# david-knigge/enf-pde

Hardware: AMD Instinct MI355X
Metric: query-points/sec (ENF fit+decode) at 64 latents x 64^2 grid (higher is better)
Workload: dtype bf16; 1 GPU; navier_stokes_64x64_z64_b16_per_gpu; decoded_states=1, latents=64, signals_per_gpu=16, inner_steps=3, sampled_points=512, num_hidden=128, num_heads=2, latent_dim=16, num_out=1, invariant=rel_pos_periodic, hparams=config_navier_stokes.yaml:23-96 with 64 latents, parallelism=dp1 (signals sharded, no data-path collective in fit/decode)

## Files before the change

enf-pde_amd/_lib.py:

```python
import ctypes
import os

_HERE = os.path.dirname(os.path.abspath(__file__))
LIB_PATH = os.environ.get("ENF_HIP_LIB") or os.path.join(_HERE, "libenf_hip.so")
TEST_LIB_PATH = os.environ.get("ENF_HIP_TEST_LIB") or os.path.join(_HERE, "libenf_hip_test.so")

ENF_NUM_TENSORS = 46
PREC = {"f32": 0, "fp32": 0, "float32": 0, "bf16": 1, "bfloat16": 1}
INVARIANT_IDS = {"rel_pos_periodic": 0, "latitude_periodic": 1, "polar_periodic": 2, "ponita": 3,
                 "abs_pos": 4, "rel_pos": 5, "norm_rel_pos": 6, "ball": 7, "ball_lat": 8, "ponita_full": 9}

EXPORTS = ["enf_abi_version", "enf_strerror", "enf_invariant_dim", "enf_invariant_pose_dim", "enf_check_desc",
           "enf_packed_weight_bytes", "enf_pack_weights", "enf_workspace_bytes", "enf_forward",
           "enf_backward_latents", "enf_backward_latents_ex", "enf_forward_stages", "enf_lt_layout", "enf_lt_layout_ext", "enf_pack_pair", "enf_pair_forward",
           "enf_pair_backward", "enf_pair_backward_ex", "enf_pair_scratch_bytes", "enf_pair_variant", "enf_pair_partition", "enf_shared_forward_parts", "enf_shared_backward_applies", "enf_backward_weights", "enf_backward_weights_scratch_bytes",
           "enf_backward_all", "enf_backward_all_scratch_bytes", "enf_fit_step", "enf_fit_inputs",
           "enf_mse_value_grad",
           "enf_workspace_bytes_ex", "enf_fit_step_ex", "enf_mse_value_grad_ex", "enf_mse_scratch_bytes", "enf_pair_backward_ex2",
           "enf_pair_backward_scratch_bytes", "enf_backward_all_scratch_bytes_ex", "enf_backward_weights_ex",
           "enf_backward_weights_scratch_bytes_ex",
           "enf_fit_step_w", "enf_mse_value_grad_w", "enf_fit_inputs_w", "enf_fit_inputs_b",
           "enf_fit_step_cw", "enf_mse_value_grad_cw", "enf_fit_inputs_cw",
           "enf_fit_step_e", "enf_eval_loss", "enf_signal_sum",
           "enf_field_grad_workspace_bytes", "enf_field_grad", "enf_query_vjp",
           "enf_ode_conv_forward", "enf_ode_conv_backward_basis", "enf_ode_conv_backward_weight", "enf_ode_conv_backward_weight_scratch_bytes", "enf_ode_poly_num_features", "enf_ode_poly_forward",
           "enf_ode_poly_backward", "enf_ode_vec_readout_forward", "enf_ode_vec_readout_backward", "enf_ode_block_supported", "enf_ode_block_scratch_bytes", "enf_ode_block_forward", "enf_ode_block_backward",
           "enf_ode_basis_supported", "enf_ode_basis_scratch_bytes", "enf_ode_basis_forward",
           "enf_ode_basis_backward", "enf_relu_mask_bytes", "enf_meta_sgd_update", "enf_table_adam_update"]
ENF_NUM_PAIR_TENSORS = 12
ENF_STAGE_PROLOGUE, ENF_STAGE_PAIR, ENF_STAGE_TAIL, ENF_STAGE_FOLD = 1, 2, 4, 8
ENF_STAGE_TAIL_SAVE = 16
ENF_STAGE_PREPARE_BWD = 32
ENF_STAGE_YBAR_HALF = 64
ENF_STAGES_FORWARD = ENF_STAGE_PROLOGUE | ENF_STAGE_PAIR | ENF_STAGE_TAIL | ENF_STAGE_FOLD
ENF_BWD_REUSE_PROLOGUE, ENF_BWD_REUSE_TAIL, ENF_BWD_REUSE_PREPARED, ENF_BWD_ONLY_PAIR = 1, 2, 4, 8
ENF_BWD_DETERMINISTIC = ENF_FIT_DETERMINISTIC = ENF_MSE_DETERMINISTIC = 16
ENF_FIT_SHARED_LATENTS = ENF_STAGE_SHARED_LATENTS = 128
ENF_BWD_QUERY_GRAD = 32
(ENF_S_EQ, ENF_S_EV, ENF_S_G1, ENF_S_NH, ENF_S_DA1, ENF_S_DA2, ENF_S_DA3, ENF_S_HEAD0) = range(8)


def num_store(H):
    return 7 + 4 * H


class EnfDesc(ctypes.Structure):
    _fields_ = [(n, ctypes.c_int32) for n in
                ("B", "N", "Z", "H", "D", "C", "O", "dx", "invariant_id", "use_window", "precision")] + \
               [("h_true", ctypes.c_int32), ("d_true", ctypes.c_int32),
                ("pair_fwd_variant", ctypes.c_int32), ("pair_bwd_variant", ctypes.c_int32), ("mask_mode", ctypes.c_int32),
                ("mask_signals", ctypes.c_int32), ("embedding", ctypes.c_int32), ("relu_masks", ctypes.c_void_p)]


VARIANT = {"auto": 0, "latent_split": 1, "z_fold": 2, "z_fold_zsplit": 3}
MASK_MODE = {"off": 0, "write": 1, "read": 2}
EMB = {"rff": 0, "ffn": 1}


class EnfSgdSegment(ctypes.Structure):
    _fields_ = [("x", ctypes.c_void_p), ("g", ctypes.c_void_p), ("lr", ctypes.c_void_p), ("out", ctypes.c_void_p),
                ("n", ctypes.c_int64), ("width", ctypes.c_int32), ("g_stride", ctypes.c_int32), ("lr_len", ctypes.c_int32),
                ("reserved", ctypes.c_int32)]


ENF_SGD_MAX_SEGMENTS = 4


ENF_ADAM_MAX_SEGMENTS = 4


class EnfAdamSegment(ctypes.Structure):
    _fields_ = [(n, ctypes.c_void_p) for n in ("x", "mu", "nu", "g", "x_out", "mu_out", "nu_out")] + \
               [("width", ctypes.c_int32), ("g_stride", ctypes.c_int32)]


class EnfFitComponent(ctypes.Structure):
    _fields_ = [("src", ctypes.c_void_p), ("dst", ctypes.c_void_p), ("width", ctypes.c_int32), ("reserved", ctypes.c_int32)]


class EnfError(RuntimeError):
    pass


_lib = None
_test_lib = None


def load():
    global _lib
    if _lib is not None:
        return _lib
    _lib = _bind(LIB_PATH, test_hooks=False)
    return _lib


def load_test():
    global _test_lib
    if _test_lib is None:
        _test_lib = _bind(TEST_LIB_PATH, test_hooks=True)
    return _test_lib


class using:

    def __init__(self, lib):
        self.lib = lib

    def __enter__(self):
        global _lib
        self.prev, _lib = _lib, self.lib
        return self.lib

    def __exit__(self, *exc):
        global _lib
        _lib = self.prev


def _bind(path, test_hooks):
    if not os.path.exists(path):
        raise EnfError(f"{path} not found: build it with `make -C enf-pde_amd/csrc` "
                       "(or python -c 'import __graft_entry__ as g; g.build()'). There is no fallback path.")
    lib = ctypes.CDLL(path)
    vp, i64, sz, ci = ctypes.c_void_p, ctypes.c_int64, ctypes.c_size_t, ctypes.c_int
    dp = ctypes.POINTER(EnfDesc)
    lib.enf_abi_version.restype = ci
    lib.enf_strerror.restype = ctypes.c_char_p
    lib.enf_strerror.argtypes = [ci]
    lib.enf_invariant_dim.argtypes = [ci, ci]
    lib.enf_invariant_pose_dim.argtypes = [ci, ci]
    lib.enf_check_desc.argtypes = [dp]
    lib.enf_packed_weight_bytes.restype = sz
    lib.enf_packed_weight_bytes.argtypes = [dp]
    lib.enf_workspace_bytes.restype = sz
    lib.enf_workspace_bytes.argtypes = [dp]
    lib.enf_pack_weights.argtypes = [dp, ctypes.POINTER(vp), vp, vp]
    lib.enf_forward.argtypes = [dp, vp, i64, vp, vp, vp, vp, vp, vp, vp, vp, sz, vp]
    lib.enf_forward_stages.argtypes = [dp, vp, i64, vp, vp, vp, vp, vp, vp, vp, vp, sz, ctypes.c_uint, vp]
    lib.enf_backward_latents.argtypes = [dp, vp, i64, vp, vp, vp, vp, vp, vp, vp, vp, vp, vp, vp, sz, vp]
    lib.enf_backward_latents_ex.argtypes = [dp, vp, i64, vp, vp, vp, vp, vp, vp, vp, vp, vp, vp, vp, sz, ctypes.c_uint, vp]
    ip = ctypes.POINTER(ci)
    lib.enf_lt_layout.argtypes = [dp, ip, ip, ip, ip, ip, ip]
    lib.enf_pack_pair.argtypes = [dp, ctypes.POINTER(vp), vp, vp]
    lib.enf_mse_value_grad.argtypes = [vp, vp, sz, ctypes.c_float, vp, vp, vp]
    lib.enf_meta_sgd_update.argtypes = [ctypes.c_int, ctypes.POINTER(EnfSgdSegment), ctypes.c_float, vp]
    lib.enf_table_adam_update.argtypes = [ctypes.c_int, ctypes.POINTER(EnfAdamSegment), i64, ctypes.c_int32, vp, ctypes.c_int32] + \
                                         [ctypes.c_float] * 6 + [vp]
    lib.enf_fit_inputs.argtypes = [ctypes.c_int, ctypes.POINTER(EnfFitComponent)] + [ctypes.c_int32] * 7 + [vp] * 7
    lib.enf_ode_conv_forward.argtypes = [ci, ci, ci, ci, vp, vp, i64, i64, vp, vp, vp, vp]
    lib.enf_ode_conv_backward_basis.argtypes = [ci, ci, ci, ci, vp, vp, vp, vp, vp]
    lib.enf_ode_conv_backward_weight_scratch_bytes.restype = sz
    lib.enf_ode_conv_backward_weight_scratch_bytes.argtypes = [ci, ci, ci, ci]
    lib.enf_ode_conv_backward_weight.argtypes = [ci, ci, ci, ci, vp, vp, vp, vp, vp, sz, vp]
    lib.enf_ode_poly_num_features.argtypes = [ci, ci]
    lib.enf_ode_poly_forward.argtypes = [i64, ci, ci, vp, vp, vp]
    lib.enf_ode_poly_backward.argtypes = [i64, ci, ci, vp, vp, vp, vp]
    lib.enf_ode_basis_supported.argtypes = [ci, ci, ci, ci, ci]
    cf = ctypes.c_float
    lib.enf_ode_vec_readout_forward.argtypes = [ci, ci, ci, ci, vp, vp, vp, vp, cf, cf, vp, vp, vp]
    lib.enf_ode_vec_readout_backward.argtypes = [ci, ci, ci, ci, vp, vp, vp, vp, cf, cf, vp, vp, vp, vp, vp, vp, vp, vp]
    lib.enf_ode_block_supported.argtypes = [ci, ci]
    lib.enf_ode_block_scratch_bytes.restype = sz
    lib.enf_ode_block_scratch_bytes.argtypes = [i64, ci, ci]
    lib.enf_ode_block_forward.argtypes = [i64, ci, ci, vp, vp, vp, vp, vp, vp, vp, ctypes.c_float, vp, vp, vp]
    lib.enf_ode_block_backward.argtypes = [i64, ci, ci, vp, vp, vp, vp, vp, vp, vp, ctypes.c_float, vp, vp, vp, sz, vp]
    lib.enf_ode_basis_scratch_bytes.restype = sz
    lib.enf_ode_basis_scratch_bytes.argtypes = [i64, ci, ci, ci, ci]
    lib.enf_ode_basis_forward.argtypes = [i64, ci, ci, ci, ci, vp, vp, vp, vp, vp, vp, vp, sz, vp]
    lib.enf_ode_basis_backward.argtypes = [i64, ci, ci, ci, ci, vp, vp, vp, vp, vp, vp, vp, vp, vp, vp, vp, vp, sz, vp]
    lib.enf_relu_mask_bytes.restype = sz
    lib.enf_relu_mask_bytes.argtypes = [dp]
    lib.enf_pair_variant.argtypes = [dp, ci]
    lib.enf_pair_partition.argtypes = [dp] + [ctypes.POINTER(ctypes.c_int32)] * 3
    lib.enf_shared_forward_parts.argtypes = [dp, ctypes.POINTER(ctypes.c_int32)]
    lib.enf_shared_backward_applies.argtypes = [dp, ctypes.c_uint]
    lib.enf_backward_weights_scratch_bytes.restype = sz
    lib.enf_backward_weights_scratch_bytes.argtypes = [dp, ci]
    lib.enf_backward_weights.argtypes = [dp, vp, i64, vp, vp, vp, vp, vp, vp, ctypes.POINTER(vp), vp, vp, sz, vp]
    lib.enf_fit_step.argtypes = [dp, vp, i64, vp, vp, vp, vp, vp, ctypes.c_float, vp, vp, vp, vp, vp, sz, vp]
    lib.enf_backward_all_scratch_bytes.restype = sz
    lib.enf_backward_all_scratch_bytes.argtypes = [dp, ci]
    lib.enf_backward_all.argtypes = [dp, vp, i64, vp, vp, vp, ctypes.POINTER(vp), vp, vp, vp, vp, vp, vp, vp, ctypes.POINTER(vp), vp,
                                     vp, sz, vp, sz, ctypes.c_uint, vp]
    lib.enf_pair_scratch_bytes.restype = sz
    lib.enf_pair_scratch_bytes.argtypes = [dp]
    lib.enf_pair_forward.argtypes = [dp, vp, i64, vp, vp, vp, vp, vp, sz, vp]
    lib.enf_pair_backward.argtypes = [dp, vp, i64, vp, vp, vp, vp, vp, vp, ctypes.POINTER(vp), vp]
    lib.enf_pair_backward_ex.argtypes = [dp, vp, i64, vp, vp, vp, vp, vp, vp, ctypes.POINTER(vp), vp, vp]
    cu = ctypes.c_uint
    lib.enf_workspace_bytes_ex.restype = sz
    lib.enf_workspace_bytes_ex.argtypes = [dp, cu]
    lib.enf_fit_step_ex.argtypes = [dp, vp, i64, vp, vp, vp, vp, vp, ctypes.c_float, vp, vp, vp, vp, vp, sz, cu, vp]
    lib.enf_mse_scratch_bytes.restype = sz
    lib.enf_mse_scratch_bytes.argtypes = [sz, cu]
    lib.enf_mse_value_grad_ex.argtypes = [vp, vp, sz, ctypes.c_float, vp, vp, vp, sz, cu, vp]
    lib.enf_fit_step_w.argtypes = [dp, vp, i64, vp, vp, vp, vp, vp, ctypes.c_float, vp, vp, vp, vp, vp, sz, vp, cu, vp]
    lib.enf_mse_value_grad_w.argtypes = [vp, vp, vp, sz, ctypes.c_int32, ctypes.c_float, vp, vp, vp, sz, cu, vp]
    lib.enf_fit_inputs_w.argtypes = [ctypes.c_int, ctypes.POINTER(EnfFitComponent)] + [ctypes.c_int32] * 7 + [vp] * 9
    lib.enf_fit_inputs_b.argtypes = [ctypes.c_int, ctypes.POINTER(EnfFitComponent)] + [ctypes.c_int32] * 7 + [vp] * 9
    lib.enf_fit_step_cw.argtypes = [dp, vp, i64, vp, vp, vp, vp, vp, ctypes.c_float, vp, vp, vp, vp, vp, sz, vp, cu, vp]
    lib.enf_mse_value_grad_cw.argtypes = [vp, vp, vp, sz, ctypes.c_float, vp, vp, vp, sz, cu, vp]
    lib.enf_fit_inputs_cw.argtypes = [ctypes.c_int, ctypes.POINTER(EnfFitComponent)] + [ctypes.c_int32] * 7 + [vp] * 8 + [ctypes.c_int32, vp]
    lib.enf_fit_step_e.argtypes = [dp, vp, i64, vp, vp, vp, vp, vp, ctypes.c_float, vp, vp, vp, vp, vp, sz, vp, vp, vp, vp, cu, vp]
    lib.enf_eval_loss.argtypes = [dp, vp, i64] + [vp] * 11 + [sz, cu, vp]
    lib.enf_signal_sum.argtypes = [vp, ctypes.c_int32, ctypes.c_int32, ctypes.c_float, vp, vp]
    lib.enf_field_grad_workspace_bytes.restype = sz
    lib.enf_field_grad_workspace_bytes.argtypes = [dp, cu]
    lib.enf_field_grad.argtypes = [dp, vp, i64] + [vp] * 7 + [sz, cu, vp]
    lib.enf_query_vjp.argtypes = [dp, vp, i64] + [vp] * 8 + [sz, cu, vp]
    lib.enf_pair_backward_scratch_bytes.restype = sz
    lib.enf_pair_backward_scratch_bytes.argtypes = [dp, cu]
    lib.enf_pair_backward_ex2.argtypes = [dp, vp, i64, vp, vp, vp, vp, vp, vp, ctypes.POINTER(vp), vp, vp, sz, cu, vp]
    lib.enf_backward_all_scratch_bytes_ex.restype = sz
    lib.enf_backward_all_scratch_bytes_ex.argtypes = [dp, ci, cu]
    lib.enf_backward_weights_scratch_bytes_ex.restype = sz
    lib.enf_backward_weights_scratch_bytes_ex.argtypes = [dp, ci, cu]
    lib.enf_backward_weights_ex.argtypes = [dp, vp, i64, vp, vp, vp, vp, vp, vp, ctypes.POINTER(vp), vp, vp, sz, cu, vp]
    if test_hooks:
        for name in ("enf_debug_gemm", "enf_debug_pack", "enf_test_read_wave_sums", "enf_test_pair_fwd_streamed"):
            getattr(lib, name).restype = ci
        lib.enf_test_pair_fwd_streamed.argtypes = [ci]
        lib.enf_debug_gemm.argtypes = [vp, vp, vp, ci, ci, ci, vp]
        lib.enf_debug_pack.argtypes = [vp, vp, ci, ci, ci, vp]
        lib.enf_test_read_wave_sums.argtypes = [vp]
    if lib.enf_abi_version() != 2:
        raise EnfError(f"{path}: ABI version mismatch")
    return lib


def check(rc):
    if rc == 0:
        return
    msg = load().enf_strerror(rc).decode()
    if rc == -2:
        raise ValueError(msg)
    if rc == -6:
        raise AssertionError(msg)
    if rc == -3:
        raise NotImplementedError(msg)
    raise EnfError(f"libenf_hip error {rc}: {msg}")


def launch(dev, fn, *args):
    import torch
    idx = dev.index if dev.index is not None else torch.cuda.current_device()
    if idx == torch.cuda.current_device():
        return check(fn(*args))
    with torch.cuda.device(idx):
        return check(fn(*args))


def ptr(t):
    return ctypes.c_void_p(t.data_ptr()) if t is not None else ctypes.c_void_p(0)


def stream(dev):
    import torch
    return ctypes.c_void_p(torch.cuda.current_stream(dev).cuda_stream)


def make_desc(B, N, Z, H, D, C, O, dx, invariant_id, use_window, precision, d_true=0, h_true=0, variants=(0, 0),
              masks=None, embedding=0):
    d = EnfDesc()
    d.B, d.N, d.Z, d.H, d.D, d.C, d.O, d.dx = int(B), int(N), int(Z), int(H), int(D), int(C), int(O), int(dx)
    d.invariant_id, d.use_window, d.precision = int(invariant_id), int(bool(use_window)), int(precision)
    d.d_true, d.h_true = int(d_true), int(h_true)
    d.pair_fwd_variant, d.pair_bwd_variant = int(variants[0]), int(variants[1])
    d.embedding = int(embedding)
    if masks is not None:
        buf, mode, signals = masks
        d.relu_masks, d.mask_mode, d.mask_signals = buf.data_ptr(), MASK_MODE[mode], int(signals)
    return d
```

enf-pde_amd/csrc/enf_api.hip:

```cpp
#include <hip/hip_runtime.h>
#include <mutex>
#include <unordered_map>
#include "enf_launch.h"

extern "C" int enf_abi_version(void) { return ENF_ABI_VERSION; }

extern "C" const char* enf_strerror(int code) {
  switch (code) {
    case ENF_OK: return "ok";
    case ENF_EINVAL: return "invalid argument (null pointer or non-positive size)";
    case ENF_EINVARIANT: return "Unknown invariant type";
    case ENF_EUNSUPPORTED: return "shape not in the compiled kernel set (num_hidden 64 or 128 after padding; num_heads 1, 2, or 4 at num_hidden 64; "
                                  "num_out <= 32; ball / ball_lat at num_hidden 64 only)";
    case ENF_EWORKSPACE: return "workspace too small";
    case ENF_ELAUNCH: return "HIP launch failed";
    case ENF_EDIM: return "coordinate / pose width inconsistent with the invariant";
    default: return "unknown error";
  }
}

extern "C" int enf_invariant_dim(int inv, int dx) {
  const int i = enf_inv_dim(inv, dx);
  return i < 0 ? ENF_EINVARIANT : i;
}
extern "C" int enf_invariant_pose_dim(int inv, int dx) {
  const int i = enf_inv_pose_dim(inv, dx);
  return i < 0 ? ENF_EINVARIANT : i;
}

extern "C" int enf_check_desc(const EnfDesc* d) {
  if (!d) return ENF_EINVAL;
  if (d->B <= 0 || d->N <= 0 || d->Z <= 0 || d->C <= 0 || d->O <= 0 || d->H <= 0 || d->D <= 0) return ENF_EINVAL;
  if (d->invariant_id < 0 || d->invariant_id >= ENF_INV_COUNT) return ENF_EINVARIANT;
  if (d->dx < 1 || d->dx > 3) return ENF_EDIM;
  const bool two_d = d->invariant_id == ENF_INV_REL_POS_PERIODIC || d->invariant_id == ENF_INV_PONITA ||
                     d->invariant_id == ENF_INV_LATITUDE_PERIODIC || d->invariant_id == ENF_INV_POLAR_PERIODIC;
  if (two_d && d->dx != 2) return ENF_EDIM;
  if (d->invariant_id == ENF_INV_PONITA_FULL && d->dx != 3) return ENF_EDIM;
  if (enf_inv_has_phase(d->invariant_id) && d->D != 64) return ENF_EUNSUPPORTED;
  if (enf_inv_has_phase(d->invariant_id) && d->dx != 3) return ENF_EDIM;
  if (!(d->D == 64 || d->D == 128)) return ENF_EUNSUPPORTED;
  if (d->d_true < 0 || d->d_true > d->D || (d->d_true & 1)) return ENF_EINVAL;
  if (!(d->H == 1 || d->H == 2 || (d->H == 4 && d->D == 64))) return ENF_EUNSUPPORTED;
  if (d->h_true < 0 || d->h_true > d->H) return ENF_EINVAL;
  if (d->O > 32) return ENF_EUNSUPPORTED;
  if (d->precision != ENF_PREC_F32 && d->precision != ENF_PREC_BF16) return ENF_EINVAL;
  if (d->pair_fwd_variant < ENF_VARIANT_AUTO || d->pair_fwd_variant > ENF_VARIANT_ZFOLD_ZSPLIT) return ENF_EINVAL;
  if (d->pair_bwd_variant < ENF_VARIANT_AUTO || d->pair_bwd_variant > ENF_VARIANT_ZFOLD) return ENF_EINVAL;
  if (d->mask_mode < ENF_MASK_OFF || d->mask_mode > ENF_MASK_READ || d->mask_signals < 0) return ENF_EINVAL;
  if (d->mask_mode != ENF_MASK_OFF && !d->relu_masks) return ENF_EINVAL;
  if (d->embedding != ENF_EMB_RFF && d->embedding != ENF_EMB_FFN) return ENF_EINVAL;
  if (d->embedding == ENF_EMB_FFN && enf_inv_has_phase(d->invariant_id)) return ENF_EUNSUPPORTED;
  return ENF_OK;
}

extern "C" size_t enf_packed_weight_bytes(const EnfDesc* d) {
  if (enf_check_desc(d) != ENF_OK) return 0;
  return enf_layout(enf_dims(d)).total;
}

extern "C" size_t enf_workspace_bytes(const EnfDesc* d) {
  if (enf_check_desc(d) != ENF_OK) return 0;
  return enf_workspace(enf_dims(d)).total;
}

extern "C" size_t enf_workspace_bytes_ex(const EnfDesc* d, unsigned flags) {
  if (enf_check_desc(d) != ENF_OK || (flags & ~(ENF_BWD_DETERMINISTIC | ENF_BWD_QUERY_GRAD | ENF_FIT_SHARED_LATENTS))) return 0;
  const EnfDims m = enf_dims(d);
  const EnfWorkspace W = enf_workspace(m);
  return (flags & ENF_BWD_DETERMINISTIC) ? enf_det_workspace(m, W).total : W.total;
}

struct SidePending { hipEvent_t join = nullptr; bool pending = false; };
struct SideStream {
  hipStream_t s = nullptr;
  hipEvent_t fork = nullptr;
  std::mutex mu;
  std::unordered_map<const void*, SidePending> ws;
  SidePending* entry(const void* workspace) {
    auto it = ws.find(workspace);
    if (it != ws.end()) return &it->second;
    if (ws.size() >= 64)
      for (auto j = ws.begin(); j != ws.end();) {
        if (!j->second.pending) { (void)hipEventDestroy(j->second.join); j = ws.erase(j); } else ++j;
      }
    SidePending e;
    if (hipEventCreateWithFlags(&e.join, hipEventDisableTiming) != hipSuccess) return nullptr;
    return &ws.emplace(workspace, e).first->second;
  }
};
static constexpr int ENF_MAX_DEVICES = 64;
static SideStream* side_stream() {
  static std::mutex table_mu;
  static SideStream* table[ENF_MAX_DEVICES] = {};
  static bool tried[ENF_MAX_DEVICES] = {};
  int dev = 0;
  if (hipGetDevice(&dev) != hipSuccess || dev < 0 || dev >= ENF_MAX_DEVICES) return nullptr;
  std::lock_guard<std::mutex> lk(table_mu);
  if (!tried[dev]) {
    tried[dev] = true;
    SideStream* t = new SideStream();
    if (hipStreamCreateWithFlags(&t->s, hipStreamNonBlocking) == hipSuccess &&
        hipEventCreateWithFlags(&t->fork, hipEventDisableTiming) == hipSuccess)
      table[dev] = t;
    else
      delete t;
  }
  return table[dev];
}

int enf_side_join_pending(hipStream_t st, const void* workspace) {
  SideStream* side = side_stream();
  if (!side) return 0;
  std::lock_guard<std::mutex> lk(side->mu);
  auto it = side->ws.find(workspace);
  if (it != side->ws.end() && it->second.pending) {
    if (hipStreamWaitEvent(st, it->second.join, 0) != hipSuccess) return ENF_ELAUNCH;
    it->second.pending = false;
  }
  return 0;
}

static int side_prepare_bwd(SideStream* side, const EnfCall& c, bool zero_dlt, int wz_signals = 0) {
  if (!side) return 0;
  EnfDims mw = c.m;
  if (wz_signals > 0) mw.B = wz_signals;
  std::lock_guard<std::mutex> lk(side->mu);
  SidePending* e = side->entry(c.ws);
  if (!e) return 0;
  if (hipEventRecord(side->fork, c.st) != hipSuccess || hipStreamWaitEvent(side->s, side->fork, 0) != hipSuccess) return ENF_ELAUNCH;
  if (int rc = enf_launch_wz(mw, c.L, c.blob, c.F(c.W.lt), nullptr, c.F(c.W.wzb), nullptr, c.ws + c.W.wzt, side->s)) return rc;
  if (zero_dlt && hipMemsetAsync(c.F(c.W.dlt), 0, enf_lt_bytes(c.m), side->s) != hipSuccess) return ENF_ELAUNCH;
  if (hipEventRecord(e->join, side->s) != hipSuccess) return ENF_ELAUNCH;
  e->pending = true;
  return 1;
}

extern "C" int enf_forward_stages(const EnfDesc* d, const float* x, int64_t x_bstride, const float* p, const float* a,
                                  const float* sigma, const void* packed, float* out, float* ybar, float* lse,
                                  void* workspace, size_t workspace_bytes, unsigned stages, void* stream) {
  EnfCall c;
  const bool shared = (stages & ENF_STAGE_SHARED_LATENTS) && d && d->B > 1;
  int rc = enf_call(c, d, x && p && a && out && !(shared && x_bstride != 0), sigma, packed, workspace, workspace_bytes, stream);
  if (rc) return rc;
  const EnfDims& m = c.m;
  const EnfWorkspace& W = c.W;
  float* yb = ybar ? ybar : c.F(W.ybar);
  const bool zf = enf_use_zfold(m);
  float* ls = lse ? lse : c.F(W.lse);
  const bool yhalf = (stages & ENF_STAGE_YBAR_HALF) && m.bf16 && !ybar && (stages & ENF_STAGE_PAIR) && (stages & ENF_STAGE_TAIL) &&
                     !(stages & ENF_STAGE_TAIL_SAVE) && enf_zfold_split(m) <= 1;
  if ((rc = enf_side_join_pending(c.st, workspace))) return rc;
  if ((stages & ENF_STAGE_PROLOGUE) && (rc = enf_launch_prologue(m, c.L, c.blob, p, a, sigma, c.F(W.lt), c.F(W.an), c.F(W.kv), c.st))) return rc;
  if ((stages & (ENF_STAGE_PAIR | ENF_STAGE_FOLD)) &&
      (rc = enf_launch_pair_fwd(m, c.L, c.blob, x, x_bstride, c.F(W.lt), yb, ls, zf ? c.ws + W.wz : nullptr, zf ? c.F(W.wzb) : nullptr,
                                zf ? c.ws + W.wzu : nullptr, enf_zfold_split(m) > 1 ? c.F(W.ysplit) : nullptr, (stages & ENF_STAGE_FOLD) != 0,
                                ((stages & ENF_STAGE_PAIR) != 0 ? 1 : 0) | (yhalf ? 2 : 0), c.st, shared ? c.F(W.dybar) : nullptr)))
    return rc;
  if ((stages & ENF_STAGE_PREPARE_BWD) && enf_use_zfold_bwd(m) && (rc = side_prepare_bwd(side_stream(), c, true)) < 0) return rc;
  const bool tsave = (stages & ENF_STAGE_TAIL_SAVE) != 0;
  if ((stages & ENF_STAGE_TAIL) &&
      (rc = enf_launch_tail(m, c.L, c.blob, yb, out, nullptr, nullptr, nullptr, tsave ? c.F(W.tail_act) : nullptr, 0, (tsave ? 1 : 0) | (yhalf ? 2 : 0), c.st)))
    return rc;
  return ENF_OK;
}

extern "C" int enf_forward(const EnfDesc* d, const float* x, int64_t x_bstride, const float* p, const float* a,
                           const float* sigma, const void* packed, float* out, float* ybar, float* lse, void* workspace,
                           size_t workspace_bytes, void* stream) {
  return enf_forward_stages(d, x, x_bstride, p, a, sigma, packed, out, ybar, lse, workspace, workspace_bytes,
                            ENF_STAGE_PROLOGUE | ENF_STAGE_FOLD | ENF_STAGE_PAIR | ENF_STAGE_TAIL, stream);
}

extern "C" int enf_backward_latents(const EnfDesc* d, const float* x, int64_t x_bstride, const float* p, const float* a,
                                    const float* sigma, const void* packed, const float* ybar, const float* lse,
                                    const float* dout, float* dp, float* da, float* dsigma, void* workspace,
                                    size_t workspace_bytes, void* stream) {
  return enf_backward_latents_ex(d, x, x_bstride, p, a, sigma, packed, ybar, lse, dout, dp, da, dsigma, workspace,
                                 workspace_bytes, 0u, stream);
}

static int pair_bwd_on_workspace(const EnfCall& c, const float* x, int64_t x_bstride, const float* lse, bool det = false) {
  const bool zb = enf_use_zfold_bwd(c.m);
  return enf_launch_pair_bwd(c.m, c.L, c.blob, x, x_bstride, c.F(c.W.lt), lse, c.F(c.W.dybar), c.F(c.W.delta), c.F(c.W.dlt), nullptr,
                             zb ? c.ws + c.W.wzt : nullptr, zb ? c.F(c.W.wzb) : nullptr, nullptr, c.st, det ? c.F(c.X.part) : nullptr);
}

extern "C" int enf_backward_latents_ex(const EnfDesc* d, const float* x, int64_t x_bstride, const float* p, const float* a,
                                       const float* sigma, const void* packed, const float* ybar, const float* lse,
                                       const float* dout, float* dp, float* da, float* dsigma, void* workspace,
                                       size_t workspace_bytes, unsigned flags, void* stream) {
  EnfCall c;
  const bool det = (flags & ENF_BWD_DETERMINISTIC) != 0;
  const bool known = !(flags & ~(ENF_BWD_REUSE_PROLOGUE | ENF_BWD_REUSE_TAIL | ENF_BWD_REUSE_PREPARED | ENF_BWD_ONLY_PAIR | ENF_BWD_DETERMINISTIC));
  int rc = enf_call(c, d, known && x && p && a && ybar && lse && dout && dp && da && dsigma, sigma, packed, workspace, workspace_bytes,
                    stream, det);
  if (rc) return rc;
  const EnfDims& m = c.m;
  const EnfWorkspace& W = c.W;
  hipStream_t st = c.st;
  const bool zb = enf_use_zfold_bwd(m);
  if (flags & ENF_BWD_ONLY_PAIR) {
    if ((rc = enf_side_join_pending(st, workspace))) return rc;
    if (!det && hipMemsetAsync(c.F(W.dlt), 0, enf_lt_bytes(m), st) != hipSuccess) return ENF_ELAUNCH;
    return pair_bwd_on_workspace(c, x, x_bstride, lse, det);
  }
  if (!(flags & ENF_BWD_REUSE_PROLOGUE) && (rc = enf_launch_prologue(m, c.L, c.blob, p, a, sigma, c.F(W.lt), c.F(W.an), c.F(W.kv), st)))
    return rc;
  SideStream* side = zb ? side_stream() : nullptr;
  bool prepared = false;
  if (zb && side && (flags & ENF_BWD_REUSE_PREPARED) && (flags & ENF_BWD_REUSE_PROLOGUE)) {
    std::lock_guard<std::mutex> lk(side->mu);
    auto it = side->ws.find(workspace);
    prepared = it != side->ws.end() && it->second.pending;
  }
  if (!prepared && (rc = enf_side_join_pending(st, workspace))) return rc;
  if (zb && !prepared) {
    if ((rc = side_prepare_bwd(side, c, false)) < 0) return rc;
    if (!rc && (rc = enf_launch_wz(m, c.L, c.blob, c.F(W.lt), nullptr, c.F(W.wzb), nullptr, c.ws + W.wzt, st))) return rc;
  }
  const bool treuse = (flags & ENF_BWD_REUSE_TAIL) && (flags & ENF_BWD_REUSE_PROLOGUE);
  if ((rc = enf_launch_tail(m, c.L, c.blob, ybar, nullptr, dout, c.F(W.dybar), c.F(W.delta), c.F(W.tail_act), 1, treuse ? 1 : 0, st))) return rc;
  if (!prepared && !det && hipMemsetAsync(c.F(W.dlt), 0, enf_lt_bytes(m), st) != hipSuccess) return ENF_ELAUNCH;
  if ((rc = enf_side_join_pending(st, workspace))) return rc;
  if ((rc = pair_bwd_on_workspace(c, x, x_bstride, lse, det))) return rc;
  return enf_launch_prologue_bwd(m, c.L, c.blob, p, sigma, c.F(W.an), c.F(W.kv), c.F(W.dlt), dp, da, dsigma, st);
}


extern "C" int enf_fit_step(const EnfDesc* d, const float* x, int64_t x_bstride, const float* p, const float* a, const float* sigma,
                            const void* packed, const float* target, float grad_scale, float* loss, float* dp, float* da,
                            float* dsigma, void* workspace, size_t workspace_bytes, void* stream) {
  return enf_fit_step_ex(d, x, x_bstride, p, a, sigma, packed, target, grad_scale, loss, dp, da, dsigma, workspace, workspace_bytes, 0u,
                         stream);
}

extern "C" int enf_fit_step_ex(const EnfDesc* d, const float* x, int64_t x_bstride, const float* p, const float* a, const float* sigma,
                               const void* packed, const float* target, float grad_scale, float* loss, float* dp, float* da,
                               float* dsigma, void* workspace, size_t workspace_bytes, unsigned flags, void* stream) {
  return enf_fit_step_w(d, x, x_bstride, p, a, sigma, packed, target, grad_scale, loss, dp, da, dsigma, workspace, workspace_bytes,
                        nullptr, flags, stream);
}

static int fit_step_sequence(const EnfDesc* d, const float* x, int64_t x_bstride, const float* p, const float* a, const float* sigma,
                             const void* packed, const float* target, float grad_scale, float* loss, float* dp, float* da,
                             float* dsigma, void* workspace, size_t workspace_bytes, const float* weight, bool per_value, unsigned flags,
                             void* stream, float* err = nullptr, float* loss_b = nullptr, bool args_ok = true) {
  EnfCall c;
  const bool det = (flags & ENF_FIT_DETERMINISTIC) != 0;
  const bool shared = (flags & ENF_FIT_SHARED_LATENTS) && d && d->B > 1;
  int rc = enf_call(c, d, !(flags & ~(ENF_FIT_DETERMINISTIC | ENF_FIT_SHARED_LATENTS)) && !(shared && x_bstride != 0) && x && p && a && target &&
                    loss && dp && da && dsigma && (!per_value || weight) && args_ok, sigma, packed, workspace, workspace_bytes, stream, det);
  if (rc) return rc;
  const EnfDims& m = c.m;
  const EnfWorkspace& W = c.W;
  hipStream_t st = c.st;
  const bool zf = enf_use_zfold(m), zb = enf_use_zfold_bwd(m);
  if ((rc = enf_side_join_pending(st, workspace))) return rc;
  if ((rc = enf_launch_prologue(m, c.L, c.blob, p, a, sigma, c.F(W.lt), c.F(W.an), c.F(W.kv), st))) return rc;
  if ((rc = enf_launch_pair_fwd(m, c.L, c.blob, x, x_bstride, c.F(W.lt), c.F(W.ybar), c.F(W.lse), zf ? c.ws + W.wz : nullptr,
                                zf ? c.F(W.wzb) : nullptr, zf ? c.ws + W.wzu : nullptr, enf_zfold_split(m) > 1 ? c.F(W.ysplit) : nullptr, 1, 1, st,
                                shared ? c.F(W.dybar) : nullptr)))
    return rc;
  const bool sbwd = enf_shared_backward_rule(m, flags, per_value, err != nullptr) == 1;
  EnfDims m1 = m;
  if (sbwd) m1.B = 1;
  if ((rc = side_prepare_bwd(zb ? side_stream() : nullptr, c, !det, sbwd ? 1 : 0)) < 0) return rc;
  if (!rc) {
    if (zb && (rc = enf_launch_wz(m1, c.L, c.blob, c.F(W.lt), nullptr, c.F(W.wzb), nullptr, c.ws + W.wzt, st))) return rc;
    if (!det && hipMemsetAsync(c.F(W.dlt), 0, enf_lt_bytes(m), st) != hipSuccess) return ENF_ELAUNCH;
  }
  if (sbwd) {
    float* dout = c.F(W.dybar) + (size_t)m.N * m.HD;
    float* out1 = dout + (size_t)m.B * m.N;
    if ((rc = enf_launch_tail(m1, c.L, c.blob, c.F(W.ybar), out1, nullptr, nullptr, nullptr, c.F(W.tail_act), 0, 1, st))) return rc;
    if ((rc = enf_launch_mse_shared(out1, target, weight, m.B, m.N, grad_scale, dout, loss, st))) return rc;
    if ((rc = enf_launch_tail_seed(m1, c.L, c.blob, c.F(W.ybar), 0, c.F(W.dybar), c.F(W.delta), c.F(W.tail_act), st))) return rc;
    if ((rc = enf_side_join_pending(st, workspace))) return rc;
    if ((rc = enf_launch_pair_bwd_shared(m, c.L, c.blob, x, c.F(W.lt), c.F(W.lse), c.F(W.dybar), c.F(W.delta), dout, c.F(W.dlt),
                                         c.ws + W.wzt, c.F(W.wzb), st)))
      return rc;
    return enf_launch_prologue_bwd(m, c.L, c.blob, p, sigma, c.F(W.an), c.F(W.kv), c.F(W.dlt), dp, da, dsigma, st);
  }
  if ((rc = enf_launch_tail_loss(m, c.L, c.blob, c.F(W.ybar), target, weight, grad_scale, loss, c.F(W.dybar), c.F(W.delta), c.F(W.tail_act), st,
                                 det ? c.F(c.X.loss) : nullptr, per_value, err)))
    return rc;
  if ((rc = enf_side_join_pending(st, workspace))) return rc;
  if ((rc = pair_bwd_on_workspace(c, x, x_bstride, c.F(W.lse), det))) return rc;
  if ((rc = enf_launch_prologue_bwd(m, c.L, c.blob, p, sigma, c.F(W.an), c.F(W.kv), c.F(W.dlt), dp, da, dsigma, st))) return rc;
  return err && loss_b ? enf_launch_signal_sum(err, m.B, m.N, 1.0f / ((float)m.N * (float)m.O), loss_b, st) : ENF_OK;
}

extern "C" int enf_fit_step_w(const EnfDesc* d, const float* x, int64_t x_bstride, const float* p, const float* a, const float* sigma,
                              const void* packed, const float* target, float grad_scale, float* loss, float* dp, float* da,
                              float* dsigma, void* workspace, size_t workspace_bytes, const float* weight, unsigned flags,
                              void* stream) {
  return fit_step_sequence(d, x, x_bstride, p, a, sigma, packed, target, grad_scale, loss, dp, da, dsigma, workspace, workspace_bytes, weight,
                           false, flags, stream);
}

extern "C" int enf_fit_step_cw(const EnfDesc* d, const float* x, int64_t x_bstride, const float* p, const float* a, const float* sigma,
                               const void* packed, const float* target, float grad_scale, float* loss, float* dp, float* da,
                               float* dsigma, void* workspace, size_t workspace_bytes, const float* cweight, unsigned flags,
                               void* stream) {
  return fit_step_sequence(d, x, x_bstride, p, a, sigma, packed, target, grad_scale, loss, dp, da, dsigma, workspace, workspace_bytes, cweight,
                           true, flags, stream);
}

extern "C" int enf_fit_step_e(const EnfDesc* d, const float* x, int64_t x_bstride, const float* p, const float* a, const float* sigma,
                              const void* packed, const float* target, float grad_scale, float* loss, float* dp, float* da,
                              float* dsigma, void* workspace, size_t workspace_bytes, const float* weight, const float* cweight,
                              float* err, float* loss_b, unsigned flags, void* stream) {
  return fit_step_sequence(d, x, x_bstride, p, a, sigma, packed, target, grad_scale, loss, dp, da, dsigma, workspace, workspace_bytes,
                           cweight ? cweight : weight, cweight != nullptr, flags, stream, err, loss_b, err && !(weight && cweight));
}

extern "C" int enf_eval_loss(const EnfDesc* d, const float* x, int64_t x_bstride, const float* p, const float* a, const float* sigma,
                             const void* packed, const float* target, const float* weight, const float* cweight, float* loss,
                             float* err, float* loss_b, void* workspace, size_t workspace_bytes, unsigned flags, void* stream) {
  EnfCall c;
  const bool det = (flags & ENF_FIT_DETERMINISTIC) != 0;
  int rc = enf_call(c, d, !(flags & ~ENF_FIT_DETERMINISTIC) && x && p && a && target && !(weight && cweight) && (loss || err || loss_b),
                    sigma, packed, workspace, workspace_bytes, stream, det);
  if (rc) return rc;
  const EnfDims& m = c.m;
  const EnfWorkspace& W = c.W;
  hipStream_t st = c.st;
  const bool zf = enf_use_zfold(m);
  if ((rc = enf_side_join_pending(st, workspace))) return rc;
  if ((rc = enf_launch_prologue(m, c.L, c.blob, p, a, sigma, c.F(W.lt), c.F(W.an), c.F(W.kv), st))) return rc;
  if ((rc = enf_launch_pair_fwd(m, c.L, c.blob, x, x_bstride, c.F(W.lt), c.F(W.ybar), c.F(W.lse), zf ? c.ws + W.wz : nullptr,
                                zf ? c.F(W.wzb) : nullptr, zf ? c.ws + W.wzu : nullptr, enf_zfold_split(m) > 1 ? c.F(W.ysplit) : nullptr, 1, 1, st)))
    return rc;
  float* e = err ? err : (loss_b ? c.F(W.dybar) : nullptr);
  if ((rc = enf_launch_tail_eval(m, c.L, c.blob, c.F(W.ybar), target, cweight ? cweight : weight, cweight != nullptr, loss, e, st,
                                 det ? c.F(c.X.loss) : nullptr)))
    return rc;
  return loss_b ? enf_launch_signal_sum(e, m.B, m.N, 1.0f / ((float)m.N * (float)m.O), loss_b, st) : ENF_OK;
}

extern "C" size_t enf_field_grad_workspace_bytes(const EnfDesc* d, unsigned flags) {
  if (enf_check_desc(d) != ENF_OK || d->mask_mode != ENF_MASK_OFF || (flags & ~ENF_BWD_DETERMINISTIC)) return 0;
  const EnfDims m = enf_dims(d);
  const EnfWorkspace W = enf_workspace(m);
  return (flags & ENF_BWD_DETERMINISTIC) ? enf_det_workspace(m, W).total + enf_det_dx_bytes(m) : W.total;
}

static int field_grad_sequence(const EnfDesc* d, const float* x, int64_t x_bstride, const float* p, const float* a, const float* sigma,
                               const void* packed, const float* dout, float* out, float* grad, bool args_ok, void* workspace,
                               size_t workspace_bytes, unsigned flags, void* stream) {
  int rc = enf_check_desc(d);
  if (rc) return rc;
  if (d->mask_mode != ENF_MASK_OFF) return ENF_EUNSUPPORTED;
  EnfCall c;
  const bool det = (flags & ENF_BWD_DETERMINISTIC) != 0;
  if ((rc = enf_call(c, d, !(flags & ~ENF_BWD_DETERMINISTIC) && x && p && a && grad && args_ok, sigma, packed, workspace, workspace_bytes,
                     stream, det)))
    return rc;
  const EnfDims& m = c.m;
  const EnfWorkspace& W = c.W;
  hipStream_t st = c.st;
  if (det && workspace_bytes < c.X.total + enf_det_dx_bytes(m)) return ENF_EWORKSPACE;
  float* part = det ? c.F(c.X.part) : nullptr;
  float* dxpart = det ? c.F(c.X.total) : nullptr;
  const bool zf = enf_use_zfold(m), zb = enf_use_zfold_bwd(m);
  const size_t per = (size_t)m.B * m.N * m.dx;
  const int passes = dout ? 1 : m.O;
  if ((rc = enf_side_join_pending(st, workspace))) return rc;
  if ((rc = enf_launch_prologue(m, c.L, c.blob, p, a, sigma, c.F(W.lt), c.F(W.an), c.F(W.kv), st))) return rc;
  if (zb && (rc = enf_launch_wz(m, c.L, c.blob, c.F(W.lt), nullptr, c.F(W.wzb), nullptr, c.ws + W.wzt, st))) return rc;
  if ((rc = enf_launch_pair_fwd(m, c.L, c.blob, x, x_bstride, c.F(W.lt), c.F(W.ybar), c.F(W.lse), zf ? c.ws + W.wz : nullptr,
                                zf ? c.F(W.wzb) : nullptr, zf ? c.ws + W.wzu : nullptr, enf_zfold_split(m) > 1 ? c.F(W.ysplit) : nullptr, 1, 1, st)))
    return rc;
  if ((rc = enf_launch_tail(m, c.L, c.blob, c.F(W.ybar), out ? out : c.F(W.dybar), nullptr, nullptr, nullptr, c.F(W.tail_act), 0, 1, st))) return rc;
  if (!det && (hipMemsetAsync(c.F(W.dlt), 0, enf_lt_bytes(m), st) != hipSuccess ||
               hipMemsetAsync(grad, 0, sizeof(float) * per * passes, st) != hipSuccess))
    return ENF_ELAUNCH;
  for (int o = 0; o < passes; ++o) {
    if (dout) rc = enf_launch_tail(m, c.L, c.blob, c.F(W.ybar), nullptr, dout, c.F(W.dybar), c.F(W.delta), c.F(W.tail_act), 1, 1, st);
    else rc = enf_launch_tail_seed(m, c.L, c.blob, c.F(W.ybar), o, c.F(W.dybar), c.F(W.delta), c.F(W.tail_act), st);
    if (rc) return rc;
    if ((rc = enf_launch_pair_bwd(m, c.L, c.blob, x, x_bstride, c.F(W.lt), c.F(W.lse), c.F(W.dybar), c.F(W.delta), c.F(W.dlt), nullptr,
                                  zb ? c.ws + W.wzt : nullptr, zb ? c.F(W.wzb) : nullptr, grad + (size_t)o * per, st, part, dxpart)))
      return rc;
  }
  return ENF_OK;
}

extern "C" int enf_field_grad(const EnfDesc* d, const float* x, int64_t x_bstride, const float* p, const float* a, const float* sigma,
                              const void* packed, float* out, float* jac, void* workspace, size_t workspace_bytes, unsigned flags,
                              void* stream) {
  return field_grad_sequence(d, x, x_bstride, p, a, sigma, packed, nullptr, out, jac, true, workspace, workspace_bytes, flags, stream);
}

extern "C" int enf_query_vjp(const EnfDesc* d, const float* x, int64_t x_bstride, const float* p, const float* a, const float* sigma,
                             const void* packed, const float* dout, float* out, float* dx, void* workspace, size_t workspace_bytes,
                             unsigned flags, void* stream) {
  return field_grad_sequence(d, x, x_bstride, p, a, sigma, packed, dout, out, dx, dout != nullptr, workspace, workspace_bytes, flags, stream);
}

extern "C" int enf_lt_layout(const EnfDesc* d, int* stride, int* off_u, int* off_v0, int* off_pose, int* off_wcoef, int* off_c) {
  int rc = enf_check_desc(d);
  if (rc) return rc;
  if (stride) *stride = enf_lt_stride(d->H, d->D);
  if (off_u) *off_u = enf_lt_off_u(d->H, d->D);
  if (off_v0) *off_v0 = enf_lt_off_v0(d->H, d->D);
  if (off_pose) *off_pose = enf_lt_off_pose(d->H, d->D);
  if (off_wcoef) *off_wcoef = enf_lt_off_wcoef(d->H, d->D);
  if (off_c) *off_c = enf_lt_off_c(d->H, d->D);
  return ENF_OK;
}

extern "C" int enf_lt_layout_ext(const EnfDesc* d, int* off_ext, int* off_phase_q, int* off_phase_v) {
  int rc = enf_check_desc(d);
  if (rc) return rc;
  if (off_ext) *off_ext = enf_lt_off_ext(d->H, d->D);
  if (off_phase_q) *off_phase_q = enf_lt_off_phq(d->H, d->D);
  if (off_phase_v) *off_phase_v = enf_lt_off_phv(d->H, d->D);
  return ENF_OK;
}

extern "C" int enf_pair_variant(const EnfDesc* d, int backward) {
  const int rc = enf_check_desc(d);
  if (rc) return rc;
  const EnfDims m = enf_dims(d);
  if (backward) return enf_use_zfold_bwd(m) ? ENF_VARIANT_ZFOLD : ENF_VARIANT_LATENT_SPLIT;
  const int sp = enf_zfold_split(m);
  return sp > 1 ? ENF_VARIANT_ZFOLD_ZSPLIT : (sp == 1 ? ENF_VARIANT_ZFOLD : ENF_VARIANT_LATENT_SPLIT);
}

extern "C" int enf_shared_forward_parts(const EnfDesc* d, int32_t* parts) {
  const int rc = enf_check_desc(d);
  if (rc) return rc;
  if (!parts) return ENF_EINVAL;
  const EnfDims m = enf_dims(d);
  const int P = enf_use_zfold(m) || (m.mask_mode != ENF_MASK_OFF && !m.ffn) ? 0 : enf_shared_fwd_parts(m);
  *parts = P ? P : 1;
  return P ? 1 : 0;
}

extern "C" int enf_shared_backward_applies(const EnfDesc* d, unsigned flags) {
  const int rc = enf_check_desc(d);
  if (rc) return rc;
  if (flags & ~(ENF_FIT_DETERMINISTIC | ENF_FIT_SHARED_LATENTS)) return ENF_EINVAL;
  return enf_shared_backward_rule(enf_dims(d), flags, false, false);
}

extern "C" int enf_pair_partition(const EnfDesc* d, int32_t* run, int32_t* workgroups, int32_t* parts) {
  const int rc = enf_check_desc(d);
  if (rc) return rc;
  if (!run || !workgroups || !parts) return ENF_EINVAL;
  const EnfDims m = enf_dims(d);
  if (enf_zfold_split(m) < 2) return 0;
  const EnfStreamK k = enf_zfold_streamk(m);
  *run = k.len; *workgroups = k.wgs; *parts = k.parts;
  return 1;
}

struct PairScratch { size_t wz, wzb, wzu, ysplit, total; };
static PairScratch pair_scratch(const EnfDims& m) {
  PairScratch s{0, 0, 0, 0, 0};
  if (!enf_use_zfold(m)) return s;
  const size_t BZ = (size_t)m.B * m.Z, BN = (size_t)m.B * m.N;
  const int split = enf_zfold_split(m);
  s.wzb = s.wz + enf_align(BZ * m.H * enf_panel_bytes(m.D, m.D, m.bf16));
  s.wzu = s.wzb + enf_align(sizeof(float) * BZ * m.HD);
  s.ysplit = s.wzu + enf_align(BZ * enf_wzu_bytes(m.H, m.D));
  s.total = s.ysplit + (split > 1 ? sizeof(float) * split * (BN * m.HD + BN * m.H * 3) : 0);
  return s;
}

extern "C" size_t enf_pair_scratch_bytes(const EnfDesc* d) {
  if (enf_check_desc(d)) return 0;
  return pair_scratch(enf_dims(d)).total;
}

extern "C" int enf_pair_forward(const EnfDesc* d, const float* x, int64_t x_bstride, const float* lt, const void* packed,
                                float* ybar, float* lse, void* scratch, size_t scratch_bytes, void* stream) {
  int rc = enf_check_desc(d);
  if (rc) return rc;
  if (!x || !lt || !packed || !ybar || !lse) return ENF_EINVAL;
  const EnfDims m = enf_dims(d);
  const PairScratch S = pair_scratch(m);
  const bool zf = S.total != 0;
  if (zf && (!scratch || scratch_bytes < S.total)) return ENF_EWORKSPACE;
  char* sc = (char*)scratch;
  return enf_launch_pair_fwd(m, enf_layout(m), (const char*)packed, x, x_bstride, lt, ybar, lse, zf ? sc + S.wz : nullptr,
                             zf ? reinterpret_cast<float*>(sc + S.wzb) : nullptr, zf ? sc + S.wzu : nullptr,
                             zf && enf_zfold_split(m) > 1 ? reinterpret_cast<float*>(sc + S.ysplit) : nullptr, 1, 1, (hipStream_t)stream);
}

extern "C" size_t enf_relu_mask_bytes(const EnfDesc* d) {
  if (enf_check_desc(d) != ENF_OK) return 0;
  const size_t signals = d->mask_signals > 0 ? d->mask_signals : d->B;
  return signals * d->Z * ((d->N + 15) / 16) * 2 * 64 * sizeof(unsigned);
}

extern "C" int enf_pair_backward(const EnfDesc* d, const float* x, int64_t x_bstride, const float* lt, const void* packed,
                                 const float* lse, const float* dybar, const float* delta, float* dlt, void* const* store,
                                 void* stream) {
  return enf_pair_backward_ex(d, x, x_bstride, lt, packed, lse, dybar, delta, dlt, store, nullptr, stream);
}

extern "C" int enf_pair_backward_ex(const EnfDesc* d, const float* x, int64_t x_bstride, const float* lt, const void* packed,
                                    const float* lse, const float* dybar, const float* delta, float* dlt, void* const* store,
                                    float* dx, void* stream) {
  return enf_pair_backward_ex2(d, x, x_bstride, lt, packed, lse, dybar, delta, dlt, store, dx, nullptr, 0, 0u, stream);
}

extern "C" size_t enf_pair_backward_scratch_bytes(const EnfDesc* d, unsigned flags) {
  if (enf_check_desc(d) != ENF_OK || (flags & ~(ENF_BWD_DETERMINISTIC | ENF_BWD_QUERY_GRAD))) return 0;
  if (!(flags & ENF_BWD_DETERMINISTIC)) return 0;
  const EnfDims m = enf_dims(d);
  return enf_det_part_bytes(m, false) + ((flags & ENF_BWD_QUERY_GRAD) ? enf_det_dx_bytes(m) : 0);
}

extern "C" int enf_pair_backward_ex2(const EnfDesc* d, const float* x, int64_t x_bstride, const float* lt, const void* packed,
                                     const float* lse, const float* dybar, const float* delta, float* dlt, void* const* store,
                                     float* dx, void* scratch, size_t scratch_bytes, unsigned flags, void* stream) {
  int rc = enf_check_desc(d);
  if (rc) return rc;
  if ((flags & ~ENF_BWD_DETERMINISTIC) || !x || !lt || !packed || !lse || !dybar || !delta || !dlt) return ENF_EINVAL;
  const bool det = (flags & ENF_BWD_DETERMINISTIC) != 0;
  if (det && !scratch) return ENF_EINVAL;
  const EnfDims m = enf_dims(d);
  if (store)
    for (int i = 0; i < ENF_NUM_STORE(m.H); ++i)
      if (!store[i]) return ENF_EINVAL;
  hipStream_t st = (hipStream_t)stream;
  if (det) {
    const size_t pb = enf_det_part_bytes(m, false);
    if (scratch_bytes < pb + (dx ? enf_det_dx_bytes(m) : 0)) return ENF_EWORKSPACE;
    return enf_launch_pair_bwd(m, enf_layout(m), (const char*)packed, x, x_bstride, lt, lse, dybar, delta, dlt, store, nullptr, nullptr, dx, st,
                               (float*)scratch, dx ? reinterpret_cast<float*>((char*)scratch + pb) : nullptr);
  }
  if (hipMemsetAsync(dlt, 0, enf_lt_bytes(m), st) != hipSuccess) return ENF_ELAUNCH;
  return enf_launch_pair_bwd(m, enf_layout(m), (const char*)packed, x, x_bstride, lt, lse, dybar, delta, dlt, store, nullptr, nullptr, dx, st);
}

extern "C" size_t enf_backward_weights_scratch_bytes(const EnfDesc* d, int chunk_signals) {
  if (enf_check_desc(d) != ENF_OK || chunk_signals < 1 || chunk_signals > d->B) return 0;
  return enf_wgrad_scratch_bytes(enf_dims(d), chunk_signals);
}

extern "C" int enf_backward_weights(const EnfDesc* d, const float* x, int64_t x_bstride, const float* lt, const void* packed,
                                    const float* lse, const float* dybar, const float* delta, float* dlt,
                                    float* const* dpair, float* dx, void* scratch, size_t scratch_bytes, void* stream) {
  return enf_backward_weights_ex(d, x, x_bstride, lt, packed, lse, dybar, delta, dlt, dpair, dx, scratch, scratch_bytes, 0u, stream);
}

static size_t wgrad_scratch_ex(const EnfDims& m, int cb, unsigned flags) {
  size_t n = enf_wgrad_scratch_bytes(m, cb);
  if (flags & ENF_BWD_DETERMINISTIC) {
    n += enf_wgrad_det_part_bytes(m, cb);
    if (flags & ENF_BWD_QUERY_GRAD) n += enf_align(sizeof(float) * (size_t)cb * m.Z * m.N * m.dx);
  }
  return n;
}
extern "C" size_t enf_backward_weights_scratch_bytes_ex(const EnfDesc* d, int chunk_signals, unsigned flags) {
  if (enf_check_desc(d) != ENF_OK || chunk_signals < 1 || chunk_signals > d->B) return 0;
  if (flags & ~(ENF_BWD_DETERMINISTIC | ENF_BWD_QUERY_GRAD)) return 0;
  return wgrad_scratch_ex(enf_dims(d), chunk_signals, flags);
}

extern "C" int enf_backward_weights_ex(const EnfDesc* d, const float* x, int64_t x_bstride, const float* lt, const void* packed,
                                       const float* lse, const float* dybar, const float* delta, float* dlt,
                                       float* const* dpair, float* dx, void* scratch, size_t scratch_bytes, unsigned flags,
                                       void* stream) {
  int rc = enf_check_desc(d);
  if (rc) return rc;
  if (d->embedding == ENF_EMB_FFN) return ENF_EUNSUPPORTED;
  if ((flags & ~ENF_BWD_DETERMINISTIC) || !x || !lt || !packed || !lse || !dybar || !delta || !dlt || !dpair || !scratch) return ENF_EINVAL;
  for (int i = 0; i < ENF_NUM_PAIR_TENSORS; ++i)
    if (i != ENF_P_COEFQ && i != ENF_P_COEFV && !dpair[i]) return ENF_EINVAL;
  const EnfDims m = enf_dims(d);
  const unsigned sflags = flags ? (ENF_BWD_DETERMINISTIC | (dx ? ENF_BWD_QUERY_GRAD : 0u)) : 0u;
  const int cb = enf_wgrad_chunk(m, scratch_bytes, [&](int n) { return wgrad_scratch_ex(m, n, sflags); });
  if (!cb) return ENF_EWORKSPACE;
  char* sc = (char*)scratch;
  float* part = sflags ? reinterpret_cast<float*>(sc + enf_wgrad_scratch_bytes(m, cb)) : nullptr;
  float* dxpart = sflags && dx ? reinterpret_cast<float*>(sc + enf_wgrad_scratch_bytes(m, cb) + enf_wgrad_det_part_bytes(m, cb)) : nullptr;
  return enf_launch_wgrad_chunks(m, enf_layout(m), (const char*)packed, cb, x, x_bstride, lt, lse, dybar, delta, dlt, dx, sc, dpair,
                                 (hipStream_t)stream, part, dxpart);
}
```

enf-pde_amd/csrc/enf_launch.h:

```cpp
#pragma once
#include <hip/hip_runtime.h>
#include <atomic>
#include "enf_layout.h"

typedef std::atomic<unsigned long long> EnfAttrBits;
inline bool enf_lds_attr(const void* kern, int bytes, EnfAttrBits& done) {
  int dev = 0;
  if (hipGetDevice(&dev) != hipSuccess) return false;
  if (dev >= 0 && dev < 64 && ((done.load(std::memory_order_acquire) >> dev) & 1ull)) return true;
  if (hipFuncSetAttribute(kern, hipFuncAttributeMaxDynamicSharedMemorySize, bytes) != hipSuccess) return false;
  if (dev >= 0 && dev < 64) done.fetch_or(1ull << dev, std::memory_order_release);
  return true;
}

inline bool enf_pair_bwd_zfold_fits(const EnfDims& m) { return (size_t)m.H * 2 * enf_panel_bytes(m.D, m.D, m.bf16) < 0x7fffffffu; }
inline int enf_pair_bwd_nsplit(const EnfDims& m, bool zfold) {
  const long long wgs = zfold ? (long long)m.B * m.Z : ((long long)m.B * m.Z + 7) / 8;
  const int ntiles = (m.N + 15) / 16;
  int ns = 1;
  while (wgs * ns < 256 && ns * 2 <= ntiles) ns *= 2;
  return ns;
}
inline int enf_pair_bwd_shared_nsplit(const EnfDims& m) {
  const int ntiles = (m.N + 15) / 16;
  if ((long long)m.Z * ((m.N + 127) / 128) <= 256) return (ntiles + 7) / 8;
  EnfDims m1 = m;
  m1.B = 1;
  return enf_pair_bwd_nsplit(m1, true);
}
inline size_t enf_det_part_bytes(const EnfDims& m, bool zfold) {
  return enf_align(sizeof(float) * (size_t)enf_pair_bwd_nsplit(m, zfold) * m.B * m.Z * enf_lt_stride(m.H, m.D));
}
inline size_t enf_det_dx_bytes(const EnfDims& m) { return enf_align(sizeof(float) * (size_t)m.B * m.Z * m.N * m.dx); }
int enf_tail_loss_parts(const EnfDims& m);
int enf_launch_loss_sum(const float* part, int n, float* loss, hipStream_t st);
struct EnfDetWorkspace { size_t part, loss, total; };
inline EnfDetWorkspace enf_det_workspace(const EnfDims& m, const EnfWorkspace& W) {
  EnfDetWorkspace X;
  X.part = W.total;
  X.loss = X.part + enf_det_part_bytes(m, enf_use_zfold_bwd(m) && enf_pair_bwd_zfold_fits(m));
  X.total = X.loss + enf_align(sizeof(float) * (size_t)enf_tail_loss_parts(m));
  return X;
}

struct EnfCall {
  EnfDims m;
  EnfLayout L;
  EnfWorkspace W;
  EnfDetWorkspace X;
  hipStream_t st;
  char* ws;
  const char* blob;
  float* F(size_t off) const { return reinterpret_cast<float*>(ws + off); }
};
inline int enf_call(EnfCall& c, const EnfDesc* d, bool pointers_ok, const float* sigma, const void* packed, void* workspace,
                    size_t workspace_bytes, void* stream, bool deterministic = false) {
  const int rc = enf_check_desc(d);
  if (rc) return rc;
  if (!pointers_ok || !packed || !workspace) return ENF_EINVAL;
  if (d->use_window && !sigma) return ENF_EINVAL;
  c.m = enf_dims(d);
  c.L = enf_layout(c.m);
  c.W = enf_workspace(c.m);
  c.X = enf_det_workspace(c.m, c.W);
  if (workspace_bytes < (deterministic ? c.X.total : c.W.total)) return ENF_EWORKSPACE;
  c.st = (hipStream_t)stream;
  c.ws = (char*)workspace;
  c.blob = (const char*)packed;
  return ENF_OK;
}

int enf_side_join_pending(hipStream_t st, const void* workspace);

int enf_launch_prologue(const EnfDims& m, const EnfLayout& L, const char* blob, const float* p, const float* a, const float* sigma,
                        float* lt, float* an, float* kv, hipStream_t st);
int enf_launch_prologue_bwd(const EnfDims& m, const EnfLayout& L, const char* blob, const float* p, const float* sigma,
                            const float* an, const float* kv, const float* dlt, float* dp, float* da, float* dsigma, hipStream_t st);
int enf_launch_prologue_bwd_wg(const EnfDims& m, const EnfLayout& L, const char* blob, const float* p, const float* sigma,
                               const float* an, const float* kv, const float* dlt, float* dp, float* da, float* dsigma, float* pg,
                               hipStream_t st);

int enf_launch_wz(const EnfDims& m, const EnfLayout& L, const char* blob, const float* lt, char* wz, float* wzb, char* wzu,
                  char* wzt, hipStream_t st);

int enf_launch_pair_fwd(const EnfDims& m, const EnfLayout& L, const char* blob, const float* x, long long x_bstride, const float* lt,
                        float* ybar, float* lse, char* wz, float* wzb, char* wzu, float* ysplit, int run_fold, int run_pair,
                        hipStream_t st, float* spart = nullptr);

int enf_launch_pair_bwd(const EnfDims& m, const EnfLayout& L, const char* blob, const float* x, long long x_bstride, const float* lt,
                        const float* lse, const float* dybar, const float* delta, float* dlt, void* const* store, const char* wzt,
                        const float* wzb, float* dxq, hipStream_t st, float* part = nullptr, float* dxpart = nullptr);

int enf_launch_pair_bwd_shared(const EnfDims& m, const EnfLayout& L, const char* blob, const float* x, const float* lt, const float* lse,
                               const float* dybar, const float* delta, const float* dout, float* dlt, const char* wzt, const float* wzb,
                               hipStream_t st);

size_t enf_xtd_part_bytes(const EnfDims& m, long long P);
int enf_launch_xtd(const EnfDims& m, void* const* store, long long P, float* const* dpair, float* part, int accumulate,
                   hipStream_t st);

size_t enf_wgrad_scratch_bytes(const EnfDims& m, int cb);
size_t enf_wgrad_det_part_bytes(const EnfDims& m, int cb);
int enf_launch_wgrad_chunks(const EnfDims& m, const EnfLayout& L, const char* blob, int cb, const float* x, long long x_bstride,
                            const float* lt, const float* lse, const float* dybar, const float* delta, float* dlt, float* dx,
                            char* scratch, float* const* dpair, hipStream_t st, float* part = nullptr, float* dxpart = nullptr);
template <class Bytes>
inline int enf_wgrad_chunk(const EnfDims& m, size_t avail, Bytes bytes) {
  const int step = m.mask_mode == ENF_MASK_READ && m.mask_B < m.B ? m.mask_B : 1;
  int cb = m.B;
  while (cb > step && bytes(cb) > avail) cb = (cb - 1) / step * step;
  return cb >= 1 && bytes(cb) <= avail ? cb : 0;
}

int enf_launch_tail(const EnfDims& m, const EnfLayout& L, const char* blob, const float* ybar, float* out, const float* dout,
                    float* dybar, float* delta, float* act, int bwd, int opt, hipStream_t st);
int enf_launch_tail_wg(const EnfDims& m, const EnfLayout& L, const char* blob, const float* ybar, float* out, const float* dout,
                       float* dybar, float* delta, float* act, float* tdel, int bwd, int opt, hipStream_t st);
int enf_launch_tail_seed(const EnfDims& m, const EnfLayout& L, const char* blob, const float* ybar, int seed, float* dybar, float* delta,
                         float* act, hipStream_t st);
int enf_launch_tail_loss(const EnfDims& m, const EnfLayout& L, const char* blob, const float* ybar, const float* target,
                         const float* weight, float gscale, float* loss, float* dybar, float* delta, float* act, hipStream_t st,
                         float* loss_part = nullptr, bool per_value = false, float* err = nullptr);
int enf_launch_tail_eval(const EnfDims& m, const EnfLayout& L, const char* blob, const float* ybar, const float* target,
                         const float* weight, bool per_value, float* loss, float* err, hipStream_t st, float* loss_part = nullptr);
int enf_launch_mse_shared(const float* out1, const float* target, const float* weight, int B, int N, float gscale, float* dout,
                          float* loss, hipStream_t st);
int enf_launch_signal_sum(const float* err, int B, int N, float scale, float* loss_b, hipStream_t st);
```

enf-pde_amd/csrc/enf_pair_bwd.hip:

```cpp
#include <hip/hip_runtime.h>
#include "enf_launch.h"
#include "enf_device.h"
#include "enf_pair_common.h"

#define K3_SCHED_FENCE() __builtin_amdgcn_sched_barrier(0)
#define K3_OPAQUE(x) asm volatile("" : "+v"(x))
#define K3_LSE(h) A.lse[qrow * H + (h)]
#define K3_DELTA(h) A.delta[qrow * H + (h)]

struct PairBwdArgs {
  const float* x; long long x_bstride;
  const float* lt; const char* blob; EnfLayout L;
  const float* lse; const float* dybar; const float* delta;
  float* dlt;
  void* store[ENF_NUM_STORE(4)];
  float inv_d;
  const char* wzt; const float* wzb;
  float* dxq;
  const unsigned* masks; int mask_B;
  int mask_b0;
  int B, N, Z, dx, inv, use_window, nsplit;
  int xcd_remap;
  float* part; float* dxpart;
  const float* dout; int SB;
};

DEV void* k3_store_ptr(const PairBwdArgs& A, int i) {
  void* p;
  const unsigned off = (unsigned)(offsetof(PairBwdArgs, store) + 8 * i);
  asm volatile("s_load_dwordx2 %0, %1, %2\n\ts_waitcnt lgkmcnt(0)" : "=s"(p) : "s"(__builtin_amdgcn_kernarg_segment_ptr()), "s"(off));
  return p;
}

#ifdef ENF_STAMPS
__device__ unsigned long long enf_stamps_bwd[8 * 4 * 24];
#define BSTAMP(k)                                                                                             \
  do {                                                                                                        \
    if (blockIdx.x == 7 && blockIdx.y == 0 && lane == 0 && ti < 4)                                            \
      enf_stamps_bwd[(wave * 4 + ti) * 24 + (k)] = __builtin_amdgcn_s_memtime();                              \
  } while (0)
extern "C" int enf_debug_read_stamps_bwd(unsigned long long* dst) {
  return hipMemcpyFromSymbol(dst, HIP_SYMBOL(enf_stamps_bwd), sizeof(enf_stamps_bwd)) == hipSuccess ? 0 : -1;
}
__device__ unsigned long long enf_stamps_bwd_wg[4 * 8 * 4];
#define WSTAMP(k)                                                                                             \
  do {                                                                                                        \
    if ((blockIdx.x & 255) == 7 && blockIdx.x < 1024 && blockIdx.y == 0 && lane == 0)                         \
      enf_stamps_bwd_wg[((blockIdx.x >> 8) * 8 + wave) * 4 + (k)] = __builtin_amdgcn_s_memtime();             \
  } while (0)
extern "C" int enf_debug_read_stamps_bwd_wg(unsigned long long* dst) {
  return hipMemcpyFromSymbol(dst, HIP_SYMBOL(enf_stamps_bwd_wg), sizeof(enf_stamps_bwd_wg)) == hipSuccess ? 0 : -1;
}
#else
#define BSTAMP(k) do {} while (0)
#define WSTAMP(k) do {} while (0)
#endif

#ifdef ENF_TEST_HOOKS
constexpr int ENF_HOOK_WGS = 64, ENF_HOOK_ROW = 16 * 64 + 16;
__device__ float enf_hook_wave_sums[ENF_HOOK_WGS * NWAVES * ENF_HOOK_ROW];
extern "C" int enf_test_read_wave_sums(float* dst) {
  return hipMemcpyFromSymbol(dst, HIP_SYMBOL(enf_hook_wave_sums), sizeof(enf_hook_wave_sums)) == hipSuccess ? 0 : -1;
}
#endif

template <bool BF16, int KB>
DEV void store_frags(void* base, size_t row, int D, const Frags<BF16, KB>& F, int quad) {
  if constexpr (BF16) {
    __bf16* p = reinterpret_cast<__bf16*>(base) + row * D;
#pragma unroll
    for (int blk = 0; blk < KB; ++blk) {
      *reinterpret_cast<bf16x8*>(p + 32 * blk + 8 * quad) = F.f[blk];
    }
  } else {
    float* p = reinterpret_cast<float*>(base) + row * D;
#pragma unroll
    for (int t = 0; t < 2 * KB; ++t) *reinterpret_cast<f32x4*>(p + 16 * t + 4 * quad) = F.f[t];
  }
}

template <int D, int H, bool BF16, bool FFN = false> struct PairBwdSmem {
  static constexpr int RING = 0;
  static constexpr int CONSTS = RING + 2 * STAGE_MAX;
  static constexpr int EW = FFN ? 4 * D : 2 * D;
  static constexpr int N_CONST = 4 * D + 2 * H * D + 2 * EW;
  static constexpr int GC = CONSTS + 4 * N_CONST;
  static constexpr int GC_BYTES = FFN ? 0 : PanelCfg<D / 64, 1, BF16>::BYTES;
  static constexpr int ZVEC = GC + 2 * GC_BYTES;
  static constexpr int LACC = ZVEC + 4 * NWAVES * 2 * H * D;
  static constexpr int EXTACC = LACC + 4 * NWAVES * 2 * H * (D / 16) * 64;
  static constexpr bool EXT_OK = D == 64;
  static constexpr int TOTAL = EXTACC + (EXT_OK ? 4 * NWAVES * 11 * 16 : 0);
  static_assert(TOTAL <= 160 * 1024, "K3 LDS budget");
};

template <int D> DEV void rff_embed_bwd(f32x4 (&dT)[D / 32], const f32x4 (&dE)[D / 16], const f32x4 (&E)[D / 16]) {
  constexpr int TT = D / 32;
#pragma unroll
  for (int m = 0; m < TT; ++m)
#pragma unroll
    for (int i = 0; i < 4; ++i) dT[m][i] = dE[m][i] * E[TT + m][i] - dE[TT + m][i] * E[m][i];
}

template <bool BF16, int KB> DEV void ffn_inv_frags(Frags<BF16, KB>& F, const float (&inv)[4], int quad) {
  f32x4 X[2 * KB];
#pragma unroll
  for (int t = 0; t < 2 * KB; ++t) X[t] = f32x4{0.f, 0.f, 0.f, 0.f};
  if (quad == 0) X[0] = f32x4{inv[0], inv[1], inv[2], inv[3]};
  make_frags<BF16, KB>(F, X);
}

template <int NT> DEV void ffn_dinv(float (&dinv)[4], const f32x4 (&dP)[NT], const float* w0, int quad) {
#pragma unroll
  for (int c = 0; c < 4; ++c)
    dinv[c] += xquad_sum(tiles_dot<NT>([&](int t) { return dP[t]; }, [&](int t) { return rowvec(w0 + c * 16 * NT, t, quad); }));
}

template <int D, bool BF16, int NEXT_BYTES>
DEV void gb_panel_flip(f32x4 (&v)[D / 16], f32x4 (&opgf)[D / 16], const Frags<BF16, D / 32>& F, Pipe& P, char* ring,
                       unsigned panel, unsigned next, const float* bias, const float* v0vec, int lane, int col, int quad) {
  using C = typename PairCfg<D, BF16>::GB;
  constexpr int KB = D / 32, MTS = C::MTS;
#pragma unroll
  for (int sp = 0; sp < C::SPP; ++sp) {
    if (sp + 1 < C::SPP) stage_issue<C::STAGE>(P.rs, panel + (sp + 1) * C::STAGE, ring + (P.cur ^ 1) * STAGE_MAX, P.wave, lane);
    else if (next != NO_STAGE) stage_issue<NEXT_BYTES>(P.rs, next, ring + (P.cur ^ 1) * STAGE_MAX, P.wave, lane);
    const char* slot = ring + P.cur * STAGE_MAX;
    f32x4 t[MTS];
    constexpr bool ASM = BF16 && GemmStageAsm<KB, MTS>::available && MTS == 8;
    if constexpr (ASM) {
      f32x4 af[4];
#pragma unroll
      for (int j = 0; j < 4; ++j) {
        const float bc = 1.0f + bias[16 * (sp * MTS + 4 * (j >> 1) + (j & 1)) + col];
        af[j] = f32x4{bc, bc, bc, bc};
      }
      GemmStageAsm<KB, MTS>::run_gb_bias(t, af, F.f, (unsigned)(uintptr_t)(lds_ptr_t)(const_cast<char*>(slot) + (lane << 4)),
                                                            (unsigned)(uintptr_t)(lds_ptr_t)(const_cast<float*>(bias) + 16 * sp * MTS + 4 * quad));
#pragma unroll
      for (int j = 0; j < 4; ++j) opgf[2 * (sp * (MTS / 4) + (j >> 1)) + (j & 1)] = af[j];
    } else {
#pragma unroll
      for (int j = 0; j < MTS; ++j) t[j] = rowvec(bias, sp * MTS + j, quad);
      gemm_stage<BF16, KB, MTS>(t, F, slot, lane);
    }
#pragma unroll
    for (int g = 0; g < MTS / 4; ++g) {
#pragma unroll
      for (int e = 0; e < 2; ++e) {
        const int tile = 2 * (sp * (MTS / 4) + g) + e;
        const f32x4 v0 = rowvec(v0vec, tile, quad);
#pragma unroll
        for (int i = 0; i < 4; ++i) v[tile][i] = fmaf(v0[i], 1.0f + t[4 * g + e][i], t[4 * g + 2 + e][i]);
        if constexpr (!ASM) {
          const float bc = 1.0f + bias[16 * (sp * MTS + 4 * g + e) + col];
          f32x4 af = {bc, bc, bc, bc};
          gemm_tile_flip<BF16, KB>(af, F, slot, 4 * g + e, lane);
          opgf[tile] = af;
        }
      }
    }
    stage_wait();
    __syncthreads();
    P.cur ^= 1;
  }
}

template <bool FAST>
DEV void pair_invariant_bwd(int inv_id, int dx, const QueryPt& q, const f32x4& pz, float wcoef, int use_window,
                            const float (&inv)[4], float win, float (&dinv)[4], float dwin, float (&dpose)[4],
                            float& dwc, float* dR = nullptr, float* dxq = nullptr, const float* ext = nullptr) {
  const float PI = 3.14159265358979323846f;
  const float dp0 = dpose[0], dp1 = dpose[1];
  switch (inv_id) {
    case ENF_INV_REL_POS_PERIODIC: {
      if (use_window) {
        dwc += dwin * (inv[0] * inv[0] + inv[1] * inv[1]);
        dinv[0] += dwin * 2.f * wcoef * inv[0];
        dinv[1] += dwin * 2.f * wcoef * inv[1];
      }
      dpose[0] += PI * (-inv[2] * dinv[0] + inv[0] * dinv[2]);
      dpose[1] += PI * (-inv[3] * dinv[1] + inv[1] * dinv[3]);
      if (dxq) { dxq[0] = -(dpose[0] - dp0); dxq[1] = -(dpose[1] - dp1); dxq[2] = 0.f; }
    } break;
    case ENF_INV_BALL:
    case ENF_INV_BALL_LAT:
    case ENF_INV_LATITUDE_PERIODIC:
    case ENF_INV_POLAR_PERIODIC: {
      const float dphi = (q.x0 - pz[0]) * 0.15915494309189535f;
      const float cd = cos_rev<FAST>(dphi), sd = sin_rev<FAST>(dphi);
      const float dot = q.sx * pz[2] * cd + q.cx * pz[3];
      float ddot = 0.f, dcd = 0.f, dsd = 0.f;
      if (inv_id == ENF_INV_LATITUDE_PERIODIC) { dpose[1] += dinv[1]; dcd += dinv[2]; dsd += dinv[3]; }
      else if (inv_id == ENF_INV_BALL_LAT) { dcd += dinv[1]; dsd += dinv[2]; }
      else if (inv_id == ENF_INV_BALL) {
        const float xr = q.x0 * 0.15915494309189535f;
        const float xh[3] = {q.sx * cos_rev<FAST>(xr), q.sx * sin_rev<FAST>(xr), q.cx};
#pragma unroll
        for (int i = 0; i < 3; ++i)
#pragma unroll
          for (int j = 0; j < 3; ++j) dR[3 * i + j] = dinv[i] * xh[j];
      }
      else ddot += dinv[0];
      if (use_window) {
        const float dc = fminf(fmaxf(dot, -1.f + 1e-6f), 1.f - 1e-6f);
        const float ang = acosf(dc);
        dwc += dwin * (-ang * ang * win);
        if (dot > -1.f + 1e-6f && dot < 1.f - 1e-6f)
          ddot += dwin * (2.f * ang * wcoef * win) * rsqrtf(1.f - dc * dc);
      }
      dcd += ddot * q.sx * pz[2];
      dpose[2] += ddot * q.sx * cd;
      dpose[3] += ddot * q.cx;
      dpose[0] += dcd * sd - dsd * cd;
      if (dxq) {
        dxq[0] = -(dcd * sd - dsd * cd);
        dxq[1] = ddot * (q.cx * pz[2] * cd - q.sx * pz[3]);
        dxq[2] = 0.f;
        if (inv_id == ENF_INV_LATITUDE_PERIODIC || inv_id == ENF_INV_BALL_LAT) dxq[1] += dinv[0];
        if (inv_id == ENF_INV_BALL_LAT) dxq[2] = dinv[3];
        if (inv_id == ENF_INV_BALL) {
          const float xr = q.x0 * 0.15915494309189535f;
          const float cp = cos_rev<FAST>(xr), sp = sin_rev<FAST>(xr);
          const float g0 = ext[0] * dinv[0] + ext[3] * dinv[1] + ext[6] * dinv[2];
          const float g1 = ext[1] * dinv[0] + ext[4] * dinv[1] + ext[7] * dinv[2];
          const float g2 = ext[2] * dinv[0] + ext[5] * dinv[1] + ext[8] * dinv[2];
          dxq[0] += q.sx * (-g0 * sp + g1 * cp);
          dxq[1] += q.cx * (g0 * cp + g1 * sp) - q.sx * g2;
          dxq[2] = dinv[3];
        }
      }
    } break;
    case ENF_INV_PONITA_FULL:
    case ENF_INV_PONITA: {
      const float r0 = q.x0 - pz[0], r1 = q.x1 - pz[1];
      float dr0 = dinv[0] * pz[2] - dinv[1] * pz[3];
      float dr1 = dinv[0] * pz[3] + dinv[1] * pz[2];
      dpose[2] += dinv[0] * r0 + dinv[1] * r1;
      dpose[3] += dinv[0] * r1 - dinv[1] * r0;
      float dth = 0.f;
      if (inv_id == ENF_INV_PONITA_FULL) {
        dpose[2] += dinv[2] * q.cx; dpose[3] += dinv[2] * q.sx;
        dth = dinv[2] * (-q.sx * pz[2] + q.cx * pz[3]);
      }
      if (use_window) {
        dwc += dwin * (-(r0 * r0 + r1 * r1));
        dr0 += dwin * (-2.f * wcoef * r0);
        dr1 += dwin * (-2.f * wcoef * r1);
      }
      dpose[0] -= dr0; dpose[1] -= dr1;
      if (dxq) { dxq[0] = dr0; dxq[1] = dr1; dxq[2] = dth; }
    } break;
    default: {
      const float r0 = q.x0 - pz[0], r1 = dx > 1 ? q.x1 - pz[1] : 0.f, r2 = dx > 2 ? q.x2 - pz[2] : 0.f;
      const float d2 = r0 * r0 + r1 * r1 + r2 * r2;
      float dr0 = 0.f, dr1 = 0.f, dr2 = 0.f;
      if (inv_id == ENF_INV_REL_POS) { dr0 = dinv[0]; dr1 = dinv[1]; dr2 = dinv[2]; }
      else if (inv_id == ENF_INV_NORM_REL_POS) {
        const float s = d2 > 0.f ? dinv[0] * rsqrtf(d2) : 0.f;
        dr0 = s * r0; dr1 = s * r1; dr2 = s * r2;
      }
      if (use_window) {
        dwc += dwin * (-d2);
        dr0 += dwin * (-2.f * wcoef * r0); dr1 += dwin * (-2.f * wcoef * r1); dr2 += dwin * (-2.f * wcoef * r2);
      }
      dpose[0] -= dr0;
      if (dx > 1) dpose[1] -= dr1;
      if (dx > 2) dpose[2] -= dr2;
      if (dxq) {
        dxq[0] = dr0; dxq[1] = dr1; dxq[2] = dr2;
        if (inv_id == ENF_INV_ABS_POS) { dxq[0] += dinv[0]; dxq[1] += dinv[1]; dxq[2] += dinv[2]; }
      }
    } break;
  }
}

template <int D, int H, bool BF16, bool STORE, bool ZF, int INV = -1, bool FFN = false, bool SHARED = false>
__global__ __launch_bounds__(NTHREADS, 2) void enf_pair_bwd_kernel(PairBwdArgs A) {
  static_assert(!(ZF && STORE), "the activation store needs the unfolded chain");
  static_assert(!SHARED || (ZF && !STORE && !FFN), "the shared-latent backward is a z-fold rff instantiation");
  static_assert(INV < 0 || INV == ENF_INV_REL_POS_PERIODIC || INV == ENF_INV_LATITUDE_PERIODIC || INV == ENF_INV_POLAR_PERIODIC ||
                INV == ENF_INV_PONITA, "specialised invariants: two coordinates, no phase");
  const int inv_id = INV >= 0 ? INV : A.inv;
  const int dx_ = INV >= 0 ? 2 : A.dx;
  using Cfg = PairCfg<D, BF16>;
  using SM = PairBwdSmem<D, H, BF16, FFN>;
  constexpr int KB = Cfg::KB, NT = Cfg::NT, TT = D / 32;
  constexpr int ST_DD = Cfg::DD::STAGE, ST_GB = Cfg::GB::STAGE, PANEL_GB = Cfg::GB::BYTES;
  using GG = PanelCfg<2 * KB, NT, BF16>;
  constexpr int ST_GG = GG::STAGE, PANEL_GG = GG::BYTES;
  constexpr int NW = NWAVES;
  constexpr bool LA = ZF && BF16 && Cfg::DD::SPP == 1;
  extern __shared__ __attribute__((aligned(16))) char smem[];
  char* ring = smem + SM::RING;
  float* cst = reinterpret_cast<float*>(smem + SM::CONSTS);
  float* c_bq1 = cst, *c_bv1 = cst + D, *c_bf = cst + 2 * D, *c_bm = cst + 3 * D, *c_bgb = cst + 4 * D;
  float* c_acq = c_bgb + 2 * H * D, *c_acv = c_acq + SM::EW;
  char* gcq = smem + SM::GC, *gcv = gcq + SM::GC_BYTES;
  const int tid = threadIdx.x, lane = tid & 63, wave = __builtin_amdgcn_readfirstlane(tid >> 6), col = lane & 15, quad = lane >> 4;
  float* zv = reinterpret_cast<float*>(smem + SM::ZVEC) + wave * 2 * H * D;
  const char* blob = A.blob;
  auto G = [&](size_t off) { return reinterpret_cast<const float*>(blob + off); };
  WSTAMP(0);

  int bz_ = ZF ? (int)blockIdx.x : blockIdx.x * NW + wave, split_ = blockIdx.y;
  if constexpr (ZF) {
    if (A.xcd_remap) {
      const unsigned k = blockIdx.x >> 3;
      split_ = (int)(k % (unsigned)A.nsplit);
      bz_ = (int)((k / (unsigned)A.nsplit) * 8u + (blockIdx.x & 7u));
    }
  }
  const int bz = bz_;
  const bool active = bz < A.B * A.Z;
  const int bzc = active ? bz : A.B * A.Z - 1;
  const int b = bzc / A.Z;
  const int split = split_;

  for (int i = tid; i < D; i += NTHREADS) { c_bq1[i] = G(A.L.bq1)[i]; c_bv1[i] = G(A.L.bv1)[i]; c_bf[i] = G(A.L.bf)[i]; c_bm[i] = G(A.L.bm)[i]; }
  if constexpr (ZF) { for (int i = tid; i < H * D; i += NTHREADS) c_bgb[i] = G(A.L.p_opbg)[i]; }
  else { for (int i = tid; i < 2 * H * D; i += NTHREADS) c_bgb[i] = G(A.L.bgb)[i]; }
  for (int i = tid; i < SM::EW; i += NTHREADS) { c_acq[i] = G(A.L.acq)[i]; c_acv[i] = G(A.L.acv)[i]; }
  for (int i = tid; i < SM::GC_BYTES / 4; i += NTHREADS) {
    reinterpret_cast<float*>(gcq)[i] = G(A.L.gcq)[i];
    reinterpret_cast<float*>(gcv)[i] = G(A.L.gcv)[i];
  }
  const int ltstride = enf_lt_stride(H, D);
  const float* ltrow = A.lt + (size_t)bzc * ltstride;
  if constexpr (ZF) {
    const float* czrow = A.wzb + (size_t)bzc * (H * D);
#pragma unroll
    for (int i = lane * 4; i < H * D; i += 256) {
      *reinterpret_cast<f32x4*>(zv + i) = *reinterpret_cast<const f32x4*>(ltrow + i);
      *reinterpret_cast<f32x4*>(zv + H * D + i) = *reinterpret_cast<const f32x4*>(czrow + i);
    }
  } else {
#pragma unroll
    for (int i = lane * 4; i < 2 * H * D; i += 256)
      *reinterpret_cast<f32x4*>(zv + i) = *reinterpret_cast<const f32x4*>(ltrow + i);
  }
  const f32x4 pz = *reinterpret_cast<const f32x4*>(ltrow + enf_lt_off_pose(H, D));
  const float wcoef = ltrow[enf_lt_off_wcoef(H, D)];
  float cz[H];
#pragma unroll
  for (int h = 0; h < H; ++h) cz[h] = ltrow[enf_lt_off_c(H, D) + h];
  const bool has_ph = INV < 0 && SM::EXT_OK && enf_inv_has_phase(inv_id);
  const float* ext = ltrow + enf_lt_off_ext(H, D);
  const float* phq = has_ph ? ltrow + enf_lt_off_phq(H, D) : nullptr;
  const float* phv = has_ph ? ltrow + enf_lt_off_phv(H, D) : nullptr;
  float* eacc = reinterpret_cast<float*>(smem + SM::EXTACC) + wave * (11 * 16) + col;
  if (has_ph) {
    if (quad == 0) { for (int k = 0; k < 9; ++k) eacc[k * 16] = 0.f; }
    else if (quad == 1) { eacc[9 * 16] = 0.f; eacc[10 * 16] = 0.f; }
  }

  const unsigned pQ1 = (unsigned)A.L.aq1, pV1 = (unsigned)A.L.av1, pF = (unsigned)A.L.af, pGB = (unsigned)A.L.agb,
                 pM = (unsigned)A.L.am, gQ1 = (unsigned)A.L.gq1, gV1 = (unsigned)A.L.gv1, gF = (unsigned)A.L.gf,
                 gGB = (unsigned)A.L.ggb, gM = (unsigned)A.L.gm;

  Pipe P;
  P.rs = make_blob_rsrc(blob, (unsigned)A.L.total);
  constexpr int PANEL_DD = Cfg::DD::BYTES;
  if constexpr (ZF) P.rs2 = make_blob_rsrc(A.wzt + (size_t)bzc * H * 2 * PANEL_DD, (unsigned)(H * 2 * PANEL_DD));
  else P.rs2 = P.rs;
  const unsigned pWG = (unsigned)A.L.awg;
  first_stage<ST_DD, NW>(P, ring, FFN ? pF : pQ1, wave, lane);
  if constexpr (LA) stage_issue_p<ST_DD, NW>(P, FFN ? STAGE_RS2 : pV1, ring + STAGE_MAX, lane);

  float* lacc = reinterpret_cast<float*>(smem + SM::LACC) + wave * (2 * H * NT * 64) + lane;
  auto lacc_flush = [&](int slot0, const float (&part)[NT]) {
    float cur[NT];
#pragma unroll
    for (int t = 0; t < NT; ++t) cur[t] = lacc[(slot0 + t) * 64];
#pragma unroll
    for (int t = 0; t < NT; ++t) lacc[(slot0 + t) * 64] = cur[t] + part[t];
  };
  auto dU_get = [&](int h, int t) { return lacc[(h * NT + t) * 64]; };
  auto dV0_get = [&](int h, int t) { return lacc[((H + h) * NT + t) * 64]; };
  float dC[H], dpose[4] = {0.f, 0.f, 0.f, 0.f}, dwc = 0.f;
#pragma unroll
  for (int h = 0; h < H; ++h) {
    dC[h] = 0.f;
    if constexpr (!SHARED) {
#pragma unroll
      for (int t = 0; t < NT; ++t) {
        lacc[(h * NT + t) * 64] = 0.f; lacc[((H + h) * NT + t) * 64] = 0.f;
      }
    }
  }

  const int ntiles = (A.N + 15) / 16;
  const int split_tiles = (ntiles - split + A.nsplit - 1) / A.nsplit;
  const int my_tiles = ZF ? (split_tiles + NW - 1) / NW : split_tiles;
  WSTAMP(1);
  for (int ti = 0; ti < my_tiles; ++ti) {
    const int tk = ZF ? ti * NW + wave : ti;
    const bool tvalid = tk < split_tiles;
    const int n0 = tvalid ? (split + tk * A.nsplit) * 16 : 0;
    const bool nvalid = tvalid && n0 + col < A.N;
    const int n = min(n0 + col, A.N - 1);
    const size_t qrow = (size_t)b * A.N + n;
    const QueryPt q = load_query(A.x + (size_t)b * A.x_bstride + (size_t)n * dx_, dx_, inv_id);
    float inv[4], win;
    pair_invariant<BF16>(inv_id, dx_, q, pz, wcoef, A.use_window, inv, win, ext);
    const size_t srow = (size_t)bzc * A.N + n;
    const bool swrite = STORE && nvalid && active;
    auto load_dout = [&](float (&ad)[4]) {
      const int sb = 16 * (int)blockIdx.z + col;
#pragma unroll
      for (int i = 0; i < 4; ++i) {
        const int nn = n0 + 4 * quad + i;
        ad[i] = SHARED && tvalid && sb < A.SB && nn < A.N ? A.dout[(size_t)sb * A.N + nn] : 0.f;
      }
    };
    auto shared_add = [&](int off, const f32x4& g, bool cols) {
      if (!(SHARED && tvalid && active && cols)) return;
#pragma unroll
      for (int j = 0; j < 4; ++j) {
        const int sb = 16 * (int)blockIdx.z + 4 * quad + j;
        if (sb < A.SB) atomicAdd(A.dlt + ((size_t)sb * A.Z + bz) * ltstride + off, g[j]);
      }
    };

    BSTAMP(0);
    float att[H], dlogit[H];
    Frags<BF16, KB> F;
    unsigned maskq = 0u, maskv = 0u;
    {
      f32x4 acc[NT];
      if constexpr (FFN) {
        ffn_pre<D>(acc, inv, c_acq, c_bq1, col, quad);
        gelu_tiles<NT>(acc);
      } else {
        rff_embed<D, BF16>(acc, inv, c_acq, lane, quad, phq);
        make_frags<BF16, KB>(F, acc);
        panel_gemm<KB, NT, BF16, ST_DD, NWAVES, INIT_BIAS, LA>(acc, F, P, ring, pQ1, LA ? pF : pV1, true, lane, c_bq1);
      }
      if constexpr (STORE && !FFN) {
        if (A.masks) {
          maskq = A.masks[relu_mask_index((b + A.mask_b0) % A.mask_B, A.Z, bzc % A.Z, (A.N + 15) / 16, n0 / 16, 0, lane)];
          maskv = A.masks[relu_mask_index((b + A.mask_b0) % A.mask_B, A.Z, bzc % A.Z, (A.N + 15) / 16, n0 / 16, 1, lane)];
          relu_apply_mask<NT>(acc, maskq);
        }
      }
      const bool masked = FFN || (STORE && A.masks != nullptr);
#pragma unroll
      for (int h = 0; h < H; ++h) {
        const float s = tiles_dot<NT>(
            [&](int t) { return masked ? acc[t] : f32x4{relu_f(acc[t][0]), relu_f(acc[t][1]), relu_f(acc[t][2]), relu_f(acc[t][3])}; },
            [&](int t) { return rowvec(zv + h * D, t, quad); });
        const float lg = xquad_sum(s) + cz[h] + win;
        att[h] = __expf(lg - K3_LSE(h));
      }
    }
    BSTAMP(1);
    unsigned relu_mask = 0u;
    Parked<BF16, NT> A3P;
    float mu1, r1;
    {
      f32x4 a3[NT], nh[NT];
      f32x4 acc[NT];
      if constexpr (FFN) {
        ffn_pre<D>(acc, inv, c_acv, c_bv1, col, quad);
        gelu_tiles<NT>(acc);
        make_frags<BF16, KB>(F, acc);
        if (swrite) {
          store_frags<BF16, KB>(k3_store_ptr(A, ENF_S_G1), srow, D, F, quad);
          Frags<BF16, KB> FI;
          ffn_inv_frags<BF16, KB>(FI, inv, quad);
          store_frags<BF16, KB>(k3_store_ptr(A, ENF_S_EV), srow, D, FI, quad);
        }
      } else {
        rff_embed<D, BF16>(acc, inv, c_acv, lane, quad, phv);
        make_frags<BF16, KB>(F, acc);
        if (swrite) store_frags<BF16, KB>(k3_store_ptr(A, ENF_S_EV), srow, D, F, quad);
        panel_gemm<KB, NT, BF16, ST_DD, NWAVES, INIT_BIAS, LA>(acc, F, P, ring, pV1, LA ? STAGE_RS2 : pF, true, lane, c_bv1);
#pragma unroll
        for (int t = 0; t < NT; ++t)
#pragma unroll
          for (int i = 0; i < 4; ++i) {
            if (STORE && A.masks) {
              acc[t][i] = (maskv >> (4 * t + i)) & 1u ? acc[t][i] : 0.f;
            } else {
              if (acc[t][i] > 0.f) relu_mask |= 1u << (4 * t + i);
              acc[t][i] = fmaxf(acc[t][i], 0.f);
            }
          }
        if (STORE && A.masks) relu_mask = maskv;
        make_frags<BF16, KB>(F, acc);
        if (swrite) store_frags<BF16, KB>(k3_store_ptr(A, ENF_S_G1), srow, D, F, quad);
      }
      if constexpr (ZF) panel_gemm<KB, NT, BF16, ST_DD, NWAVES, INIT_BIAS, LA>(a3, F, P, ring, pF, LA ? gM : STAGE_RS2, true, lane, c_bf);
      else panel_gemm<KB, NT, BF16, ST_GB, NWAVES, INIT_BIAS>(a3, F, P, ring, pF, pGB, true, lane, c_bf);
      K3_SCHED_FENCE();
#pragma unroll
      for (int t = 0; t < NT; ++t) {
        gelu_fg_tile(a3[t], nh[t]);
        asm volatile("" : "+v"(nh[t]), "+v"(a3[t]));
        K3_SCHED_FENCE();
      }
      ln_stats<NT>(nh, mu1, r1, A.inv_d);
      ln_apply<NT>(nh, mu1, r1);
      make_frags<BF16, KB>(F, nh);
      if (swrite) store_frags<BF16, KB>(k3_store_ptr(A, ENF_S_NH), srow, D, F, quad);
      A3P.park(a3);
    }
    BSTAMP(2);
    f32x4 dnh[NT];
    if constexpr (!ZF) {
#pragma unroll
      for (int t = 0; t < NT; ++t) dnh[t] = f32x4{0.f, 0.f, 0.f, 0.f};
    }

    if constexpr (ZF) {
      Frags<BF16, KB> FAh[H];
#pragma unroll
      for (int h = 0; h < H; ++h) {
        const unsigned wzf = STAGE_RS2 | (unsigned)(h * 2 * PANEL_DD);
        f32x4 a5[NT], v[NT];
        f32x4 dy[NT];
        {
          const float* dyrow = A.dybar + qrow * (H * D) + h * D + 4 * quad;
#pragma unroll
          for (int t = 0; t < NT; ++t) dy[t] = *reinterpret_cast<const f32x4*>(dyrow + 16 * t);
        }
        const float delta_h = K3_DELTA(h);
        panel_gemm<KB, NT, BF16, ST_DD, NWAVES, INIT_BIAS, LA>(a5, F, P, ring, wzf, LA ? pWG + h * PANEL_DD : gM, true, lane, zv + H * D + h * D);
        BSTAMP(4 + 6 * h);
        float mu2, r2;
        K3_SCHED_FENCE();
#pragma unroll
        for (int t = 0; t < NT; ++t) {
          gelu_fg_tile(a5[t], v[t]);
          asm volatile("" : "+v"(v[t]), "+v"(a5[t]));
          K3_SCHED_FENCE();
        }
        ln_stats<NT>(v, mu2, r2, A.inv_d);
        ln_apply<NT>(v, mu2, r2);
        float s0 = 0.f, sd = 0.f;
        tiles_sum_dot<NT>(dy, [&](int t) { return v[t]; }, sd, s0);
        const float datt = xquad_sum(s0);
        dlogit[h] = nvalid ? att[h] * (datt - delta_h) : 0.f;
        const float ah = nvalid ? att[h] : 0.f;
        const float m1 = ah * xquad_sum(sd) * A.inv_d, m2 = ah * datt * A.inv_d;
        {
          const float ahr = ah * r2, m1r = m1 * r2, nm2r = -m2 * r2;
#pragma unroll
          for (int t = 0; t < NT; ++t) {
            K3_OPAQUE(a5[t]);
#pragma unroll
            for (int i = 0; i < 4; ++i)
              dy[t][i] = fmaf(nm2r, v[t][i], fmaf(ahr, dy[t][i], -m1r)) * a5[t][i];
          }
        }
        BSTAMP(5 + 6 * h);
        Frags<BF16, KB>& FA = FAh[h];
        make_frags<BF16, KB>(FA, dy);
        f32x4 dvf[NT];
        {
          f32x4 none[1];
          const unsigned wzb0 = STAGE_RS2 | (unsigned)PANEL_DD;
          const unsigned nxt = h + 1 < H ? wzf + 2 * PANEL_DD : wzb0;
          const unsigned nxt2 = h + 1 < H ? gM : (H > 1 ? wzb0 + 2 * PANEL_DD : gF);
          panel_gemm_flip<KB, NT, BF16, ST_DD, NW, false, INIT_ZERO, LA>(
              none, FA, P, ring, gM, LA ? nxt : pWG + h * PANEL_DD, lane, [](int) { return f32x4{0.f, 0.f, 0.f, 0.f}; },
              [&](int mt, const f32x4& af) { dvf[mt] = af; });
          float part[NT];
          float ad[4];
          if constexpr (SHARED) load_dout(ad);
          panel_gemm_flip<KB, NT, BF16, ST_DD, NW, false, INIT_ACC, LA>(
              none, F, P, ring, pWG + h * PANEL_DD, LA ? nxt2 : nxt, lane,
              [&](int mt) { const float bc = c_bgb[h * D + 16 * mt + col]; return f32x4{bc, bc, bc, bc}; },
              [&](int mt, const f32x4& af) {
                if constexpr (SHARED) {
                  f32x4 g = {0.f, 0.f, 0.f, 0.f};
#pragma unroll
                  for (int i = 0; i < 4; ++i) g = __builtin_amdgcn_mfma_f32_16x16x4f32(ad[i], af[i] * dvf[mt][i], g, 0, 0, 0);
                  shared_add(enf_lt_off_v0(H, D) + h * D + 16 * mt + col, g, true);
                } else {
                  const f32x2 p2 = __builtin_elementwise_fma(hi2(af), hi2(dvf[mt]), lo2(af) * lo2(dvf[mt]));
                  part[mt] = p2[0] + p2[1];
                }
              });
          if constexpr (!SHARED) lacc_flush((H + h) * NT, part);
        }
        BSTAMP(6 + 6 * h);
      }
      {
#pragma unroll
        for (int h = 0; h < H; ++h) {
          const unsigned wzb = (STAGE_RS2 | (unsigned)(h * 2 * PANEL_DD)) + PANEL_DD;
          const unsigned after = h + 1 < H ? wzb + 2 * PANEL_DD : gF;
          const unsigned after2 = h + 2 < H ? wzb + 4 * PANEL_DD : (h + 2 == H ? gF : FFN ? (ti + 1 < my_tiles ? pF : NO_STAGE) : gV1);
          if (h == 0) panel_gemm<KB, NT, BF16, ST_DD, NWAVES, INIT_ZERO, LA>(dnh, FAh[h], P, ring, wzb, LA ? after2 : after, true, lane);
          else panel_gemm<KB, NT, BF16, ST_DD, NWAVES, INIT_ACC, LA>(dnh, FAh[h], P, ring, wzb, LA ? after2 : after, true, lane);
        }
      }
    } else
#pragma unroll
    for (int h = 0; h < H; ++h) {
      f32x4 v[NT];
      Parked<BF16, NT> OPG;
      {
        f32x4 opgf[NT];
        gb_panel_flip<D, BF16, ST_DD>(v, opgf, F, P, ring, pGB + h * PANEL_GB, pM, c_bgb + 2 * h * D, zv + H * D + h * D,
                                      lane, col, quad);
        OPG.park(opgf);
      }
      BSTAMP(3 + 6 * h);
      f32x4 a5[NT];
      {
        Frags<BF16, KB> FV;
        make_frags<BF16, KB>(FV, v);
        if (swrite) store_frags<BF16, KB>(k3_store_ptr(A, ENF_S_HEAD0 + 4 * h), srow, D, FV, quad);
        panel_gemm<KB, NT, BF16, ST_DD, NWAVES, INIT_BIAS>(a5, FV, P, ring, pM, gM, true, lane, c_bm);
      }
      BSTAMP(4 + 6 * h);
      f32x4 dy[NT];
      float mu2, r2;
      K3_SCHED_FENCE();
#pragma unroll
      for (int t = 0; t < NT; ++t) {
#pragma unroll
        for (int i = 0; i < 4; ++i) {
          float g, d;
          gelu_fg1(a5[t][i], g, d);
          v[t][i] = g;
          a5[t][i] = d;
        }
        asm volatile("" : "+v"(v[t]), "+v"(a5[t]));
        K3_SCHED_FENCE();
      }
      ln_stats<NT>(v, mu2, r2, A.inv_d);
      ln_apply<NT>(v, mu2, r2);
      {
        const float* dyrow = A.dybar + qrow * (H * D) + h * D;
#pragma unroll
        for (int t = 0; t < NT; ++t) dy[t] = *reinterpret_cast<const f32x4*>(dyrow + 16 * t + 4 * quad);
      }
      float s0, sd;
      tiles_sum_dot<NT>(dy, [&](int t) { return v[t]; }, sd, s0);
      const float datt = xquad_sum(s0);
      dlogit[h] = nvalid ? att[h] * (datt - K3_DELTA(h)) : 0.f;
      const float ah = nvalid ? att[h] : 0.f;
      const float m1 = ah * xquad_sum(sd) * A.inv_d, m2 = ah * datt * A.inv_d;
#pragma unroll
      for (int t = 0; t < NT; ++t) {
        K3_OPAQUE(a5[t]);
#pragma unroll
        for (int i = 0; i < 4; ++i)
          dy[t][i] = r2 * (fmaf(ah, dy[t][i], -m1) - v[t][i] * m2) * a5[t][i];
        K3_SCHED_FENCE();
      }
      BSTAMP(5 + 6 * h);
      {
        Frags<BF16, KB> FA;
        make_frags<BF16, KB>(FA, dy);
        if (swrite) store_frags<BF16, KB>(k3_store_ptr(A, ENF_S_HEAD0 + 4 * h + 1), srow, D, FA, quad);
        float part[NT];
        panel_gemm_flip<KB, NT, BF16, ST_GG, NW, true, INIT_ZERO>(
            v, FA, P, ring, gM, gGB + h * PANEL_GG, lane, [](int) { return f32x4{0.f, 0.f, 0.f, 0.f}; },
            [&](int mt, const f32x4& af) {
              const f32x4 og = OPG.get(mt);
              part[mt] = af[0] * og[0] + af[1] * og[1] + af[2] * og[2] + af[3] * og[3];
            });
        lacc_flush((H + h) * NT, part);
      }
      BSTAMP(6 + 6 * h);
      Frags<BF16, 2 * KB> FG;
#pragma unroll
      for (int m = 0; m < KB; ++m) {
        f32x4 dg[2];
#pragma unroll
        for (int e = 0; e < 2; ++e) {
          const f32x4 v0 = rowvec(zv + H * D + h * D, 2 * m + e, quad);
#pragma unroll
          for (int i = 0; i < 4; ++i) dg[e][i] = v[2 * m + e][i] * v0[i];
        }
        if constexpr (BF16) {
#pragma unroll
          for (int j = 0; j < 8; ++j) {
            FG.f[2 * m][j] = (__bf16)dg[j >> 2][j & 3];
            FG.f[2 * m + 1][j] = (__bf16)v[2 * m + (j >> 2)][j & 3];
          }
        } else {
          FG.f[4 * m] = dg[0]; FG.f[4 * m + 1] = dg[1];
          FG.f[4 * m + 2] = v[2 * m]; FG.f[4 * m + 3] = v[2 * m + 1];
        }
      }
      BSTAMP(7 + 6 * h);
      if (swrite) {
        Frags<BF16, KB> Fg, Fb;
#pragma unroll
        for (int m = 0; m < KB; ++m) {
          if constexpr (BF16) { Fg.f[m] = FG.f[2 * m]; Fb.f[m] = FG.f[2 * m + 1]; }
          else { Fg.f[2 * m] = FG.f[4 * m]; Fg.f[2 * m + 1] = FG.f[4 * m + 1]; Fb.f[2 * m] = FG.f[4 * m + 2]; Fb.f[2 * m + 1] = FG.f[4 * m + 3]; }
        }
        store_frags<BF16, KB>(k3_store_ptr(A, ENF_S_HEAD0 + 4 * h + 2), srow, D, Fg, quad);
        store_frags<BF16, KB>(k3_store_ptr(A, ENF_S_HEAD0 + 4 * h + 3), srow, D, Fb, quad);
      }
      if (h + 1 < H) panel_gemm<2 * KB, NT, BF16, ST_GB>(dnh, FG, P, ring, gGB + h * PANEL_GG, pGB + (h + 1) * PANEL_GB, true, lane);
      else panel_gemm<2 * KB, NT, BF16, ST_DD>(dnh, FG, P, ring, gGB + h * PANEL_GG, gF, true, lane);
    }

    BSTAMP(15);
    float dinv[4] = {0.f, 0.f, 0.f, 0.f};
    float dlat[2] = {0.f, 0.f};
    {
      float s1, s2;
      tiles_sum_dot<NT>(dnh, [&](int t) { return Parked<BF16, NT>{F}.get(t); }, s1, s2);
      const float m1 = xquad_sum(s1) * A.inv_d, m2 = xquad_sum(s2) * A.inv_d;
      const float m1r = m1 * r1, nm2r = -m2 * r1;
#pragma unroll
      for (int t = 0; t < NT; ++t) {
        const f32x4 nht = Parked<BF16, NT>{F}.get(t);
        f32x4 a3t = A3P.get(t);
        K3_OPAQUE(a3t);
#pragma unroll
        for (int i = 0; i < 4; ++i)
          dnh[t][i] = fmaf(nm2r, nht[i], fmaf(r1, dnh[t][i], -m1r)) * a3t[i];
        K3_SCHED_FENCE();
      }
      make_frags<BF16, KB>(F, dnh);
      if (swrite) store_frags<BF16, KB>(k3_store_ptr(A, ENF_S_DA3), srow, D, F, quad);
      f32x4 acc[NT];
      if constexpr (FFN) {
        const bool more = ti + 1 < my_tiles;
        panel_gemm<KB, NT, BF16, ST_DD, NWAVES, INIT_ZERO, LA>(acc, F, P, ring, gF, more ? (LA ? STAGE_RS2 : pF) : NO_STAGE, true, lane);
        f32x4 pre[NT];
        ffn_pre<D>(pre, inv, c_acv, c_bv1, col, quad);
#pragma unroll
        for (int t = 0; t < NT; ++t) {
          f32x4 g;
          gelu_fg_tile(pre[t], g);
#pragma unroll
          for (int i = 0; i < 4; ++i) acc[t][i] *= pre[t][i];
        }
        if (swrite) {
          Frags<BF16, KB> FD;
          make_frags<BF16, KB>(FD, acc);
          store_frags<BF16, KB>(k3_store_ptr(A, ENF_S_DA2), srow, D, FD, quad);
        }
        ffn_dinv<NT>(dinv, acc, c_acv, quad);
      } else {
        panel_gemm<KB, NT, BF16, ST_DD, NWAVES, INIT_ZERO, LA>(acc, F, P, ring, gF, LA ? pQ1 : gV1, true, lane);
#pragma unroll
        for (int t = 0; t < NT; ++t)
#pragma unroll
          for (int i = 0; i < 4; ++i)
            acc[t][i] = ((relu_mask >> (4 * t + i)) & 1u) ? acc[t][i] : 0.f;
        make_frags<BF16, KB>(F, acc);
        if (swrite) store_frags<BF16, KB>(k3_store_ptr(A, ENF_S_DA2), srow, D, F, quad);
        panel_gemm<KB, NT, BF16, ST_DD, NWAVES, INIT_ZERO, LA>(acc, F, P, ring, gV1, LA ? gQ1 : pQ1, true, lane);
        f32x4 Ev[NT];
        rff_embed<D, BF16>(Ev, inv, c_acv, lane, quad, phv);
        f32x4 dT[TT];
        rff_embed_bwd<D>(dT, acc, Ev);
        Frags<BF16, D / 64> FT;
        make_frags<BF16, D / 64>(FT, dT);
        f32x4 di[1] = {f32x4{0.f, 0.f, 0.f, 0.f}};
        gemm_stage<BF16, D / 64, 1>(di, FT, gcv, lane);
        if (quad == 0) { dinv[0] += di[0][0]; dinv[1] += di[0][1]; dinv[2] += di[0][2]; dinv[3] += di[0][3]; }
        else if (quad == 1) { dlat[0] += di[0][0]; dlat[1] += di[0][1]; }
      }
    }
    BSTAMP(16);
    if constexpr (FFN) {
      float dl[H][4];
#pragma unroll
      for (int h = 0; h < H; ++h)
#pragma unroll
        for (int i = 0; i < 4; ++i) dl[h][i] = __shfl(dlogit[h], (quad << 4) | (4 * quad + i), 64);
      {
        f32x4 hf[NT];
        ffn_pre_flip<D>(hf, inv, c_acq, c_bq1, col, quad);
        gelu_tiles<NT>(hf);
        float upart[H][NT];
#pragma unroll
        for (int mt = 0; mt < NT; ++mt)
#pragma unroll
          for (int h = 0; h < H; ++h) {
            const f32x2 p2 = __builtin_elementwise_fma(hi2(hf[mt]), f32x2{dl[h][2], dl[h][3]}, lo2(hf[mt]) * f32x2{dl[h][0], dl[h][1]});
            upart[h][mt] = p2[0] + p2[1];
          }
#pragma unroll
        for (int h = 0; h < H; ++h) lacc_flush(h * NT, upart[h]);
      }
      f32x4 pre[NT];
      ffn_pre<D>(pre, inv, c_acq, c_bq1, col, quad);
#pragma unroll
      for (int t = 0; t < NT; ++t) {
        f32x4 g, dh = {0.f, 0.f, 0.f, 0.f};
        gelu_fg_tile(pre[t], g);
#pragma unroll
        for (int h = 0; h < H; ++h) {
          const f32x4 u = rowvec(zv + h * D, t, quad);
#pragma unroll
          for (int i = 0; i < 4; ++i) dh[i] = fmaf(dlogit[h], u[i], dh[i]);
        }
#pragma unroll
        for (int i = 0; i < 4; ++i) pre[t][i] *= dh[i];
      }
      if (swrite) {
        Frags<BF16, KB> FS;
        make_frags<BF16, KB>(FS, pre);
        store_frags<BF16, KB>(k3_store_ptr(A, ENF_S_DA1), srow, D, FS, quad);
        ffn_inv_frags<BF16, KB>(FS, inv, quad);
        store_frags<BF16, KB>(k3_store_ptr(A, ENF_S_EQ), srow, D, FS, quad);
      }
      ffn_dinv<NT>(dinv, pre, c_acq, quad);
    } else
    {
      f32x4 E[NT];
      rff_embed<D, BF16>(E, inv, c_acq, lane, quad, phq);
      make_frags<BF16, KB>(F, E);
      if (swrite) store_frags<BF16, KB>(k3_store_ptr(A, ENF_S_EQ), srow, D, F, quad);
      f32x4 acc[NT];
      float dl[H][4];
#pragma unroll
      for (int h = 0; h < H; ++h)
#pragma unroll
        for (int i = 0; i < 4; ++i) dl[h][i] = __shfl(dlogit[h], (quad << 4) | (4 * quad + i), 64);
      const bool more = ti + 1 < my_tiles;
      float upart[H][NT];
      float adl[H][4];
      if constexpr (SHARED) {
        float ad[4];
        load_dout(ad);
#pragma unroll
        for (int h = 0; h < H; ++h)
#pragma unroll
          for (int i = 0; i < 4; ++i) adl[h][i] = ad[i] * dl[h][i];
      }
      unsigned mflip[4] = {0u, 0u, 0u, 0u};
      const bool masked = STORE && A.masks != nullptr;
      if (masked) {
#pragma unroll
        for (int i = 0; i < 4; ++i) mflip[i] = (unsigned)__shfl((int)maskq, ((col >> 2) << 4) | (4 * quad + i), 64) >> (col & 3);
      }
      panel_gemm_flip<KB, NT, BF16, ST_DD, NW, true, INIT_BIAS, LA>(
          acc, F, P, ring, pQ1, LA ? (more ? pQ1 : NO_STAGE) : gQ1, lane,
          [&](int mt) { const float bc = c_bq1[16 * mt + col]; return f32x4{bc, bc, bc, bc}; },
          [&](int mt, const f32x4& af) {
            float r0, r1, r2, r3;
            if (masked) {
              r0 = (mflip[0] >> (4 * mt)) & 1u ? af[0] : 0.f; r1 = (mflip[1] >> (4 * mt)) & 1u ? af[1] : 0.f;
              r2 = (mflip[2] >> (4 * mt)) & 1u ? af[2] : 0.f; r3 = (mflip[3] >> (4 * mt)) & 1u ? af[3] : 0.f;
            } else { r0 = relu_f(af[0]); r1 = relu_f(af[1]); r2 = relu_f(af[2]); r3 = relu_f(af[3]); }
#pragma unroll
            for (int h = 0; h < H; ++h) {
              if constexpr (SHARED) {
                f32x4 g = {0.f, 0.f, 0.f, 0.f};
                g = __builtin_amdgcn_mfma_f32_16x16x4f32(adl[h][0], r0, g, 0, 0, 0);
                g = __builtin_amdgcn_mfma_f32_16x16x4f32(adl[h][1], r1, g, 0, 0, 0);
                g = __builtin_amdgcn_mfma_f32_16x16x4f32(adl[h][2], r2, g, 0, 0, 0);
                g = __builtin_amdgcn_mfma_f32_16x16x4f32(adl[h][3], r3, g, 0, 0, 0);
                shared_add(enf_lt_off_u(H, D) + h * D + 16 * mt + col, g, true);
              } else {
                const f32x2 p2 = __builtin_elementwise_fma(f32x2{r2, r3}, f32x2{dl[h][2], dl[h][3]}, f32x2{r0, r1} * f32x2{dl[h][0], dl[h][1]});
                upart[h][mt] = p2[0] + p2[1];
              }
            }
          }, c_bq1);
      if constexpr (!SHARED) {
#pragma unroll
        for (int h = 0; h < H; ++h) {
          lacc_flush(h * NT, upart[h]);
        }
      }
#pragma unroll
      for (int t = 0; t < NT; ++t) {
        f32x4 dh = {0.f, 0.f, 0.f, 0.f};
#pragma unroll
        for (int h = 0; h < H; ++h) {
          const f32x4 u = rowvec(zv + h * D, t, quad);
#pragma unroll
          for (int i = 0; i < 4; ++i) dh[i] = fmaf(dlogit[h], u[i], dh[i]);
        }
#pragma unroll
        for (int i = 0; i < 4; ++i)
          acc[t][i] = (masked ? ((maskq >> (4 * t + i)) & 1u) != 0u : acc[t][i] > 0.f) ? dh[i] : 0.f;
      }
      Frags<BF16, KB> FA;
      make_frags<BF16, KB>(FA, acc);
      if (swrite) store_frags<BF16, KB>(k3_store_ptr(A, ENF_S_DA1), srow, D, FA, quad);
      panel_gemm<KB, NT, BF16, ST_DD, NWAVES, INIT_ZERO, LA>(acc, FA, P, ring, gQ1, more ? (LA ? pV1 : pQ1) : NO_STAGE, true, lane);
      f32x4 dT[TT];
      rff_embed_bwd<D>(dT, acc, E);
      Frags<BF16, D / 64> FT;
      make_frags<BF16, D / 64>(FT, dT);
      f32x4 di[1] = {f32x4{0.f, 0.f, 0.f, 0.f}};
      gemm_stage<BF16, D / 64, 1>(di, FT, gcq, lane);
      if (quad == 0) { dinv[0] += di[0][0]; dinv[1] += di[0][1]; dinv[2] += di[0][2]; dinv[3] += di[0][3]; }
      else if (quad == 1) { dlat[0] += di[0][0]; dlat[1] += di[0][1]; }
    }
    BSTAMP(17);
    if constexpr (SHARED) {
      float sc[H + 5];
#pragma unroll
      for (int j = 0; j < H + 5; ++j) sc[j] = 0.f;
      if (quad == 0) {
        float dwin = 0.f, tp[4] = {0.f, 0.f, 0.f, 0.f}, tw = 0.f;
#pragma unroll
        for (int h = 0; h < H; ++h) { sc[h] = dlogit[h]; dwin += dlogit[h]; }
        pair_invariant_bwd<BF16>(inv_id, dx_, q, pz, wcoef, A.use_window, inv, win, dinv, dwin, tp, tw, nullptr, nullptr);
        sc[H] = tp[0]; sc[H + 1] = tp[1]; sc[H + 2] = tp[2]; sc[H + 3] = tp[3]; sc[H + 4] = tw;
      }
      float ad[4];
      load_dout(ad);
      f32x4 g = {0.f, 0.f, 0.f, 0.f};
#pragma unroll
      for (int i = 0; i < 4; ++i) {
        float bv = 0.f;
#pragma unroll
        for (int j = 0; j < H + 5; ++j) {
          const float t = __shfl(sc[j], 4 * quad + i, 64);
          bv = col == j ? t : bv;
        }
        g = __builtin_amdgcn_mfma_f32_16x16x4f32(ad[i], bv, g, 0, 0, 0);
      }
      const int off = col < H ? enf_lt_off_c(H, D) + col : col < H + 4 ? enf_lt_off_pose(H, D) + col - H : enf_lt_off_wcoef(H, D);
      shared_add(off, g, col < H + 5);
    } else
    if (quad == 0) {
      float dwin = 0.f;
#pragma unroll
      for (int h = 0; h < H; ++h) { dC[h] += dlogit[h]; dwin += dlogit[h]; }
      float dxv[3];
      float* dxp = A.dxq ? dxv : nullptr;
      if (has_ph) {
        float dR[9] = {0.f, 0.f, 0.f, 0.f, 0.f, 0.f, 0.f, 0.f, 0.f};
        pair_invariant_bwd<BF16>(inv_id, dx_, q, pz, wcoef, A.use_window, inv, win, dinv, dwin, dpose, dwc, dR, dxp, ext);
        if (inv_id == ENF_INV_BALL) {
#pragma unroll
          for (int k = 0; k < 9; ++k) eacc[k * 16] += dR[k];
        }
      } else
      pair_invariant_bwd<BF16>(inv_id, dx_, q, pz, wcoef, A.use_window, inv, win, dinv, dwin, dpose, dwc, nullptr, dxp);
      if (A.dxq && nvalid && active) {
        if (A.dxpart) {
          float* o = A.dxpart + ((size_t)bzc * A.N + n) * dx_;
          o[0] = dxv[0];
          if (dx_ > 1) o[1] = dxv[1];
          if (dx_ > 2) o[2] = dxv[2];
        } else {
          float* o = A.dxq + ((size_t)b * A.N + n) * dx_;
          atomicAdd(o, dxv[0]);
          if (dx_ > 1) atomicAdd(o + 1, dxv[1]);
          if (dx_ > 2) atomicAdd(o + 2, dxv[2]);
        }
      }
    } else if (has_ph && quad == 1) { eacc[9 * 16] += dlat[0]; eacc[10 * 16] += dlat[1]; }
  }

#ifdef ENF_TEST_HOOKS
  if constexpr (!SHARED && 2 * H * (D / 16) <= 16) {
    const int wg = blockIdx.y * gridDim.x + blockIdx.x;
    if (wg < ENF_HOOK_WGS) {
      float* o = enf_hook_wave_sums + (size_t)(wg * NWAVES + wave) * ENF_HOOK_ROW;
      for (int k = 0; k < 2 * H * NT; ++k) o[k * 64 + lane] = lacc[k * 64];
      float q0[H + 5];
      for (int h = 0; h < H; ++h) q0[h] = dC[h];
      q0[H] = dpose[0]; q0[H + 1] = dpose[1]; q0[H + 2] = dpose[2]; q0[H + 3] = dpose[3]; q0[H + 4] = dwc;
      for (int i = 0; i < H + 5; ++i) {
        float a = quad == 0 ? q0[i] : 0.f;
        for (int off = 32; off > 0; off >>= 1) a += __shfl_xor(a, off, 64);
        if (lane == 0) o[16 * 64 + i] = a;
      }
      if (lane == 0) { o[16 * 64 + 8] = (float)bz; o[16 * 64 + 9] = (float)bzc; o[16 * 64 + 10] = (float)my_tiles; }
    }
  }
#endif
  pipe_finish(P);
  WSTAMP(2);
  if constexpr (SHARED) return;
  if (!active) return;
  const bool det = A.part != nullptr;
  float* drow = det ? A.part + ((size_t)split * ((size_t)A.B * A.Z) + bz) * ltstride : A.dlt + (size_t)bz * ltstride;
  auto put = [&](float* p, float v) { if (det) *p = v; else atomicAdd(p, v); };
  if constexpr (ZF) {
    __syncthreads();
    const float* lall = reinterpret_cast<const float*>(smem + SM::LACC) + lane;
    constexpr int NS = 2 * H * NT;
    for (int sl = wave; sl < NS; sl += NW) {
      float v = 0.f;
#pragma unroll
      for (int w = 0; w < NW; ++w) v += lall[(w * NS + sl) * 64];
      v = xquad_sum(v);
      if (quad == 0)
        put(drow + (sl < H * NT ? enf_lt_off_u(H, D) + 16 * sl : enf_lt_off_v0(H, D) + 16 * (sl - H * NT)) + col, v);
    }
  } else
#pragma unroll
  for (int h = 0; h < H; ++h)
#pragma unroll
    for (int t = 0; t < NT; ++t) {
      const float a = xquad_sum(dU_get(h, t)), c = xquad_sum(dV0_get(h, t));
      if (quad == 0) {
        put(drow + enf_lt_off_u(H, D) + h * D + 16 * t + col, a);
        put(drow + enf_lt_off_v0(H, D) + h * D + 16 * t + col, c);
      }
    }
  float sc[H + 5];
#pragma unroll
  for (int h = 0; h < H; ++h) sc[h] = dC[h];
  sc[H] = dpose[0]; sc[H + 1] = dpose[1]; sc[H + 2] = dpose[2]; sc[H + 3] = dpose[3]; sc[H + 4] = dwc;
#pragma unroll
  for (int i = 0; i < H + 5; ++i) {
    float a = quad == 0 ? sc[i] : 0.f;
#pragma unroll
    for (int o = 32; o > 0; o >>= 1) a += __shfl_xor(a, o, 64);
    sc[i] = a;
  }
  if constexpr (ZF) {
    if (det) {
      __syncthreads();
      float* fold = reinterpret_cast<float*>(smem + SM::LACC);
      float mine = 0.f;
#pragma unroll
      for (int i = 0; i < H + 5; ++i) mine = lane == i ? sc[i] : mine;
      if (has_ph) {
#pragma unroll
        for (int k = 0; k < 11; ++k) {
          float a = quad == (k < 9 ? 0 : 1) ? eacc[k * 16] : 0.f;
#pragma unroll
          for (int o = 32; o > 0; o >>= 1) a += __shfl_xor(a, o, 64);
          mine = lane == 16 + k ? a : mine;
        }
      }
      if (lane < 32) fold[wave * 32 + lane] = mine;
      __syncthreads();
      if (wave == 0 && (lane < H + 5 || (has_ph && lane >= 16 && lane < 27))) {
        float v = 0.f;
#pragma unroll
        for (int w = 0; w < NW; ++w) v += fold[w * 32 + lane];
        const int off = lane < H ? enf_lt_off_c(H, D) + lane
                        : lane < H + 4 ? enf_lt_off_pose(H, D) + lane - H
                        : lane == H + 4 ? enf_lt_off_wcoef(H, D) : enf_lt_off_ext(H, D) + lane - 16;
        drow[off] = v;
      }
      WSTAMP(3);
      return;
    }
  }
  if (lane == 0) {
#pragma unroll
    for (int h = 0; h < H; ++h) put(drow + enf_lt_off_c(H, D) + h, sc[h]);
#pragma unroll
    for (int i = 0; i < 4; ++i) put(drow + enf_lt_off_pose(H, D) + i, sc[H + i]);
    put(drow + enf_lt_off_wcoef(H, D), sc[H + 4]);
  }
  if (has_ph) {
#pragma unroll
    for (int k = 0; k < 11; ++k) {
      float a = quad == (k < 9 ? 0 : 1) ? eacc[k * 16] : 0.f;
#pragma unroll
      for (int o = 32; o > 0; o >>= 1) a += __shfl_xor(a, o, 64);
      if (lane == 0) put(drow + enf_lt_off_ext(H, D) + k, a);
    }
  }
  WSTAMP(3);
}

__global__ __launch_bounds__(256) void enf_dlt_reduce_kernel(const float* __restrict__ part, int nsplit, long long rows, int H, int D,
                                                            int ext, float* __restrict__ dlt) {
  const int stride = enf_lt_stride(H, D);
  const long long total = rows * stride, e = (long long)blockIdx.x * 256 + threadIdx.x;
  if (e >= total) return;
  const int c = (int)(e % stride), base = 2 * H * D;
  const bool written = c < base + 5 || (c >= enf_lt_off_c(H, D) && c < enf_lt_off_c(H, D) + H) ||
                       (ext && c >= enf_lt_off_ext(H, D) && c < enf_lt_off_ext(H, D) + 11);
  float s = 0.f;
  if (written) {
    s = part[e];
    for (int k = 1; k < nsplit; ++k) s += part[(size_t)k * total + e];
  }
  dlt[e] = s;
}
__global__ __launch_bounds__(256) void enf_dxq_reduce_kernel(const float* __restrict__ dxpart, int B, int Z, int N, int dx,
                                                            float* __restrict__ out) {
  const long long per = (long long)N * dx, e = (long long)blockIdx.x * 256 + threadIdx.x;
  if (e >= per * B) return;
  const long long b = e / per, r = e - b * per;
  const float* src = dxpart + (size_t)b * Z * per + r;
  float s = src[0];
  for (int z = 1; z < Z; ++z) s += src[(size_t)z * per];
  out[e] = s;
}

template <int D, int H, bool BF16, bool STORE, bool ZF, int INV = -1, bool FFN = false>
static int launch_pair_bwd(const PairBwdArgs& A, hipStream_t st) {
  using SM = PairBwdSmem<D, H, BF16, FFN>;
  auto kern = enf_pair_bwd_kernel<D, H, BF16, STORE, ZF, INV, FFN>;
  static EnfAttrBits attr_done{0};
  if (!enf_lds_attr(reinterpret_cast<const void*>(kern), SM::TOTAL, attr_done)) return ENF_ELAUNCH;
  dim3 grid(ZF ? A.B * A.Z : (A.B * A.Z + NWAVES - 1) / NWAVES, A.nsplit);
  if (ZF && A.xcd_remap) grid = dim3(A.B * A.Z * A.nsplit, 1);
  hipLaunchKernelGGL(kern, grid, dim3(NTHREADS), SM::TOTAL, st, A);
  return hipGetLastError() == hipSuccess ? 0 : ENF_ELAUNCH;
}

template <int D, int H, bool BF16, int INV = -1>
static int launch_pair_bwd_shared(const PairBwdArgs& A, hipStream_t st) {
  using SM = PairBwdSmem<D, H, BF16, false>;
  auto kern = enf_pair_bwd_kernel<D, H, BF16, false, true, INV, false, true>;
  static EnfAttrBits attr_done{0};
  if (!enf_lds_attr(reinterpret_cast<const void*>(kern), SM::TOTAL, attr_done)) return ENF_ELAUNCH;
  hipLaunchKernelGGL(kern, dim3(A.Z, A.nsplit, (A.SB + 15) / 16), dim3(NTHREADS), SM::TOTAL, st, A);
  return hipGetLastError() == hipSuccess ? 0 : ENF_ELAUNCH;
}

int enf_launch_pair_bwd_shared(const EnfDims& m, const EnfLayout& L, const char* blob, const float* x, const float* lt, const float* lse,
                               const float* dybar, const float* delta, const float* dout, float* dlt, const char* wzt, const float* wzb,
                               hipStream_t st) {
  if (!enf_pair_bwd_shared_exists(m) || !enf_pair_bwd_zfold_fits(m) || !wzt || !wzb || !dout) return ENF_EUNSUPPORTED;
  PairBwdArgs A;
  A.dxq = nullptr; A.part = nullptr; A.dxpart = nullptr; A.masks = nullptr; A.mask_B = 1; A.mask_b0 = 0;
  A.wzt = wzt; A.wzb = wzb; A.inv_d = 1.0f / (float)m.Dt;
  A.x = x; A.x_bstride = 0; A.lt = lt; A.blob = blob; A.L = L; A.lse = lse; A.dybar = dybar; A.delta = delta;
  A.dlt = dlt; A.B = 1; A.N = m.N; A.Z = m.Z; A.dx = m.dx; A.inv = m.inv; A.use_window = m.use_window;
  A.nsplit = enf_pair_bwd_shared_nsplit(m); A.xcd_remap = 0;
  A.dout = dout; A.SB = m.B;
  if (m.bf16 && m.dx == 2) {
    if (m.D == 128 && m.H == 2 && m.inv == ENF_INV_REL_POS_PERIODIC) return launch_pair_bwd_shared<128, 2, true, ENF_INV_REL_POS_PERIODIC>(A, st);
    if (m.D == 64 && m.H == 2 && m.inv == ENF_INV_PONITA) return launch_pair_bwd_shared<64, 2, true, ENF_INV_PONITA>(A, st);
  }
#define ENF_CASE(DD, HH) \
  if (m.D == DD && m.H == HH) return m.bf16 ? launch_pair_bwd_shared<DD, HH, true>(A, st) : launch_pair_bwd_shared<DD, HH, false>(A, st);
  ENF_CASE(128, 2)
  ENF_CASE(64, 2)
  ENF_CASE(128, 1)
#undef ENF_CASE
  return ENF_EUNSUPPORTED;
}


static int pair_bwd_kernel(const EnfDims& m, const EnfLayout& L, const char* blob, const float* x, long long x_bstride,
                           const float* lt, const float* lse, const float* dybar, const float* delta, float* dlt,
                           void* const* store, const char* wzt, const float* wzb, float* dxq, hipStream_t st, float* part,
                           float* dxpart, int* nsplit);

int enf_launch_pair_bwd(const EnfDims& m, const EnfLayout& L, const char* blob, const float* x, long long x_bstride,
                        const float* lt, const float* lse, const float* dybar, const float* delta, float* dlt,
                        void* const* store, const char* wzt, const float* wzb, float* dxq, hipStream_t st, float* part,
                        float* dxpart) {
  if (part && dxq && !dxpart) return ENF_EINVAL;
  int ns = 1;
  if (int rc = pair_bwd_kernel(m, L, blob, x, x_bstride, lt, lse, dybar, delta, dlt, store, wzt, wzb, dxq, st, part,
                               part ? dxpart : nullptr, &ns))
    return rc;
  if (!part) return 0;
  const long long rows = (long long)m.B * m.Z, nl = rows * enf_lt_stride(m.H, m.D);
  hipLaunchKernelGGL(enf_dlt_reduce_kernel, dim3((unsigned)((nl + 255) / 256)), dim3(256), 0, st, part, ns, rows, m.H, m.D,
                     (int)enf_inv_has_phase(m.inv), dlt);
  if (dxq) {
    const long long nx = (long long)m.B * m.N * m.dx;
    hipLaunchKernelGGL(enf_dxq_reduce_kernel, dim3((unsigned)((nx + 255) / 256)), dim3(256), 0, st, dxpart, m.B, m.Z, m.N, m.dx, dxq);
  }
  return hipGetLastError() == hipSuccess ? 0 : ENF_ELAUNCH;
}

static int pair_bwd_kernel(const EnfDims& m, const EnfLayout& L, const char* blob, const float* x, long long x_bstride,
                           const float* lt, const float* lse, const float* dybar, const float* delta, float* dlt,
                           void* const* store, const char* wzt, const float* wzb, float* dxq, hipStream_t st, float* part,
                           float* dxpart, int* nsplit) {
  PairBwdArgs A;
  A.dxq = dxq; A.part = part; A.dxpart = dxpart;
  A.dout = nullptr; A.SB = 0;
  A.masks = store && m.mask_mode == ENF_MASK_READ ? m.masks : nullptr; A.mask_B = m.mask_B; A.mask_b0 = m.mask_b0;
  const bool zf = !store && wzt && wzb && enf_pair_bwd_zfold_fits(m);
  A.wzt = wzt; A.wzb = wzb; A.inv_d = 1.0f / (float)m.Dt;
  A.x = x; A.x_bstride = x_bstride; A.lt = lt; A.blob = blob; A.L = L; A.lse = lse; A.dybar = dybar; A.delta = delta;
  A.dlt = dlt; A.B = m.B; A.N = m.N; A.Z = m.Z; A.dx = m.dx; A.inv = m.inv; A.use_window = m.use_window;
  static_assert(NWAVES == 8, "enf_pair_bwd_nsplit (enf_launch.h) counts 8 latents per latent-split workgroup");
  const int wgs = zf ? m.B * m.Z : (m.B * m.Z + NWAVES - 1) / NWAVES;
  const int ns = enf_pair_bwd_nsplit(m, zf);
  A.nsplit = ns; *nsplit = ns;
  A.xcd_remap = zf && ns > 1 && wgs % 8 == 0;
  if (store)
    for (int i = 0; i < ENF_NUM_STORE(m.H); ++i) A.store[i] = store[i];
  if (m.ffn) {
    A.masks = nullptr;
#define ENF_FFN_CASE(DD, HH)                                                                                                       \
    if (m.D == DD && m.H == HH) {                                                                                                 \
      if (store) return m.bf16 ? launch_pair_bwd<DD, HH, true, true, false, -1, true>(A, st) : launch_pair_bwd<DD, HH, false, true, false, -1, true>(A, st); \
      if (zf) return m.bf16 ? launch_pair_bwd<DD, HH, true, false, true, -1, true>(A, st) : launch_pair_bwd<DD, HH, false, false, true, -1, true>(A, st); \
      return m.bf16 ? launch_pair_bwd<DD, HH, true, false, false, -1, true>(A, st) : launch_pair_bwd<DD, HH, false, false, false, -1, true>(A, st);      \
    }
    ENF_FFN_CASE(128, 2)
    ENF_FFN_CASE(64, 2)
    ENF_FFN_CASE(128, 1)
    ENF_FFN_CASE(64, 1)
    ENF_FFN_CASE(64, 4)
#undef ENF_FFN_CASE
    return ENF_EUNSUPPORTED;
  }
#define ENF_CASE(DD, HH)                                                                   \
  if (m.D == DD && m.H == HH) {                                                            \
    if (store) return m.bf16 ? launch_pair_bwd<DD, HH, true, true, false>(A, st) : launch_pair_bwd<DD, HH, false, true, false>(A, st); \
    if (zf) return m.bf16 ? launch_pair_bwd<DD, HH, true, false, true>(A, st) : launch_pair_bwd<DD, HH, false, false, true>(A, st);    \
    return m.bf16 ? launch_pair_bwd<DD, HH, true, false, false>(A, st) : launch_pair_bwd<DD, HH, false, false, false>(A, st);         \
  }
  if (zf && m.bf16 && m.dx == 2) {
    if (m.D == 128 && m.H == 2) {
      if (m.inv == ENF_INV_REL_POS_PERIODIC) return launch_pair_bwd<128, 2, true, false, true, ENF_INV_REL_POS_PERIODIC>(A, st);
      if (m.inv == ENF_INV_LATITUDE_PERIODIC) return launch_pair_bwd<128, 2, true, false, true, ENF_INV_LATITUDE_PERIODIC>(A, st);
      if (m.inv == ENF_INV_POLAR_PERIODIC) return launch_pair_bwd<128, 2, true, false, true, ENF_INV_POLAR_PERIODIC>(A, st);
    }
    if (m.D == 64 && m.H == 2 && m.inv == ENF_INV_PONITA) return launch_pair_bwd<64, 2, true, false, true, ENF_INV_PONITA>(A, st);
  }
  if (store && m.bf16 && m.dx == 2 && m.D == 128 && m.H == 2 && m.inv == ENF_INV_REL_POS_PERIODIC)
    return launch_pair_bwd<128, 2, true, true, false, ENF_INV_REL_POS_PERIODIC>(A, st);
  ENF_CASE(128, 2)
  ENF_CASE(64, 2)
  ENF_CASE(128, 1)
  ENF_CASE(64, 1)
  ENF_CASE(64, 4)
#undef ENF_CASE
  return ENF_EUNSUPPORTED;
}
```

enf-pde_amd/csrc/enf_tail.hip:

```cpp
#include <hip/hip_runtime.h>
#include <cstdlib>
#include "enf_launch.h"
#define ENF_PIPE_ONE_RS 1
#include "enf_device.h"

struct TailArgs {
  const float* ybar; const char* blob; EnfLayout L;
  float* out;
  const float* dout;
  float* dybar; float* delta; float* act;
  const float* target; float* loss; float gscale, inv_n;
  const float* weight;
  float* err;
  float* loss_part;
  float* tdel;
  union {
    int ybar_half;
    int seed;
  };
  int NQ, O;
  float inv_hd;
};

template <int NT> DEV void load_rows(f32x4 (&X)[NT], const float* row, int quad) {
#pragma unroll
  for (int t = 0; t < NT; ++t) X[t] = *reinterpret_cast<const f32x4*>(row + 16 * t + 4 * quad);
}
template <int NT> DEV void load_rows_half(f32x4 (&X)[NT], const unsigned short* row, int quad) {
#pragma unroll
  for (int t = 0; t < NT; ++t) {
    const uint2 w = *reinterpret_cast<const uint2*>(row + 16 * t + 4 * quad);
    X[t] = f32x4{__builtin_bit_cast(float, w.x << 16), __builtin_bit_cast(float, w.x & 0xffff0000u),
                 __builtin_bit_cast(float, w.y << 16), __builtin_bit_cast(float, w.y & 0xffff0000u)};
  }
}
template <int NT> DEV void store_rows(const f32x4 (&X)[NT], float* row, int quad) {
#pragma unroll
  for (int t = 0; t < NT; ++t) *reinterpret_cast<f32x4*>(row + 16 * t + 4 * quad) = X[t];
}
template <int NT> DEV void zero_tiles(f32x4 (&X)[NT]) {
#pragma unroll
  for (int t = 0; t < NT; ++t) X[t] = f32x4{0.f, 0.f, 0.f, 0.f};
}

template <int D, int H, bool BF16> struct TailCfg {
  static constexpr int KB = D / 32, KBH = H * D / 32, NT = D / 16, NTH = H * D / 16, HD = H * D;
  static constexpr int ACT = 2 * HD + 2 * D + 2;
  static constexpr int ST_TB = PanelCfg<KBH, NTH, BF16>::STAGE;
  static constexpr int ST_O0 = PanelCfg<KBH, NT, BF16>::STAGE;
  static constexpr int ST_O2 = PanelCfg<KB, NT, BF16>::STAGE;
  static constexpr int ST_O4 = PanelCfg<KB, 2, BF16>::STAGE;
  static constexpr int ST_G4 = PanelCfg<1, NT, BF16>::STAGE;
  static constexpr int ST_G0 = PanelCfg<KB, NTH, BF16>::STAGE;
  static constexpr int SMEM = 2 * STAGE_MAX + 4 * (2 * HD + 2 * D + 32);
  static constexpr int SMEM3 = 3 * STAGE_MAX + 4 * (2 * HD + 2 * D + 32);
};

template <int BYTES> struct La2Cnt { static constexpr int K = BYTES > 0 ? (BYTES / 1024) / NWAVES : 0; };
template <int K> DEV void wait_vm() { asm volatile("s_waitcnt vmcnt(%0)" ::"n"(K) : "memory"); }
template <int BYTES> DEV void la2_issue(const Pipe& P, unsigned off, char* ring, int slot, int lane) {
  stage_issue<BYTES>(P.rs, off, ring + slot * STAGE_MAX, P.wave, lane);
}
template <int KBIN, int MTOUT, bool BF16> struct Pan {
  using C = PanelCfg<KBIN, MTOUT, BF16>;
  static constexpr int SPP = C::SPP, STAGE = C::STAGE;
};
struct NoPan { static constexpr int SPP = 0, STAGE = 0; };

template <int SP, int KBIN, int MTOUT, bool BF16, typename N1, typename N2, int INIT>
DEV void la2_step(f32x4 (&acc)[MTOUT], const Frags<BF16, KBIN>& F, Pipe& P, char* ring, unsigned panel, unsigned n1, unsigned n2,
                  int lane, const float* bias) {
  using C = PanelCfg<KBIN, MTOUT, BF16>;
  constexpr int AHEAD = SP + 2 - C::SPP;
  const int slot2 = (P.cur + 2) % 3;
  constexpr int ISSUED = AHEAD < 0 ? C::STAGE : (AHEAD < N1::SPP ? N1::STAGE : (AHEAD == N1::SPP && N1::SPP <= 1 ? N2::STAGE : 0));
  if constexpr (AHEAD < 0) la2_issue<C::STAGE>(P, panel + (SP + 2) * C::STAGE, ring, slot2, lane);
  else if constexpr (AHEAD < N1::SPP) la2_issue<N1::STAGE>(P, n1 + AHEAD * N1::STAGE, ring, slot2, lane);
  else if constexpr (AHEAD == N1::SPP && N1::SPP <= 1 && N2::STAGE > 0) la2_issue<N2::STAGE>(P, n2, ring, slot2, lane);
  gemm_stage<BF16, KBIN, C::MTS, INIT>(&acc[SP * C::MTS], F, ring + P.cur * STAGE_MAX, lane, bias + 16 * SP * C::MTS);
  wait_vm<La2Cnt<ISSUED>::K>();
  __syncthreads();
  P.cur = (P.cur + 1) % 3;
}
template <int KBIN, int MTOUT, bool BF16, typename N1, typename N2, int INIT = INIT_ACC>
DEV void panel_gemm_la2(f32x4 (&acc)[MTOUT], const Frags<BF16, KBIN>& F, Pipe& P, char* ring, unsigned panel, unsigned n1,
                        unsigned n2, int lane, const float* bias = nullptr) {
  using C = PanelCfg<KBIN, MTOUT, BF16>;
  static_assert(C::SPP <= 8, "unrolled by hand");
#define LA2_STEP(SP_) if constexpr (C::SPP > SP_) la2_step<SP_, KBIN, MTOUT, BF16, N1, N2, INIT>(acc, F, P, ring, panel, n1, n2, lane, bias);
  LA2_STEP(0) LA2_STEP(1) LA2_STEP(2) LA2_STEP(3) LA2_STEP(4) LA2_STEP(5) LA2_STEP(6) LA2_STEP(7)
#undef LA2_STEP
}
template <typename A0, typename B0>
DEV void la2_first(Pipe& P, char* ring, unsigned a, unsigned b, int wave, int lane) {
  P.cur = 0;
  P.wave = __builtin_amdgcn_readfirstlane(wave);
  P.early = false;
  la2_issue<A0::STAGE>(P, a, ring, 0, lane);
  constexpr int S1 = A0::SPP > 1 ? A0::STAGE : B0::STAGE;
  if constexpr (A0::SPP > 1) la2_issue<A0::STAGE>(P, a + A0::STAGE, ring, 1, lane);
  else if constexpr (B0::STAGE > 0) la2_issue<B0::STAGE>(P, b, ring, 1, lane);
  wait_vm<La2Cnt<S1>::K>();
  __syncthreads();
}
template <bool LA2, int KBIN, int MTOUT, bool BF16, typename N1, typename N2, int NEXT_BYTES>
DEV void tail_gemm(f32x4 (&acc)[MTOUT], const Frags<BF16, KBIN>& F, Pipe& P, char* ring, unsigned panel, unsigned n1, unsigned n2,
                   int lane) {
  if constexpr (LA2) panel_gemm_la2<KBIN, MTOUT, BF16, N1, N2>(acc, F, P, ring, panel, n1, n2, lane);
  else panel_gemm<KBIN, MTOUT, BF16, NEXT_BYTES>(acc, F, P, ring, panel, n1, true, lane);
}

template <int D, int H, bool BF16, bool SAVE, bool LA2, typename NX1, typename NX2>
DEV void tail_forward(f32x4 (&o4)[2], const float* yrow, float* act, const EnfLayout& L, const float* cst, Pipe& P,
                      char* ring, unsigned next, unsigned next2, int lane, int quad, float inv_hd, bool save_ok = true, bool y_half = false) {
  using T = TailCfg<D, H, BF16>;
  constexpr int KB = T::KB, KBH = T::KBH, NT = T::NT, NTH = T::NTH, HD = T::HD;
  using PTB = Pan<KBH, NTH, BF16>; using PO0 = Pan<KBH, NT, BF16>; using PO2 = Pan<KB, NT, BF16>; using PO4 = Pan<KB, 2, BF16>;
  constexpr int NEXT_BYTES = NX1::STAGE > 0 ? NX1::STAGE : 1024;
  const float* c_bB = cst, *c_bF1 = cst + HD, *c_bO0 = cst + 2 * HD, *c_bO2 = cst + 2 * HD + D, *c_bO4 = cst + 2 * HD + 2 * D;
  Frags<BF16, KBH> FH;
  f32x4 a[NTH];
  if (y_half) load_rows_half<NTH>(a, reinterpret_cast<const unsigned short*>(yrow), quad);
  else load_rows<NTH>(a, yrow, quad);
  make_frags<BF16, KBH>(FH, a);
#pragma unroll
  for (int t = 0; t < NTH; ++t) a[t] = rowvec(c_bB, t, quad);
  tail_gemm<LA2, KBH, NTH, BF16, PTB, PO0, T::ST_TB>(a, FH, P, ring, (unsigned)L.atb, (unsigned)L.atf1, (unsigned)L.ato0, lane);
  if (SAVE && save_ok) store_rows<NTH>(a, act, quad);
#pragma unroll
  for (int t = 0; t < NTH; ++t)
#pragma unroll
    for (int i = 0; i < 4; ++i) a[t][i] = gelu_f(a[t][i]);
  float mu, rstd;
  ln_stats<NTH>(a, mu, rstd, inv_hd);
  if (SAVE && save_ok && quad == 0) { act[T::ACT - 2] = mu; act[T::ACT - 1] = rstd; }
  ln_apply<NTH>(a, mu, rstd);
  make_frags<BF16, KBH>(FH, a);
#pragma unroll
  for (int t = 0; t < NTH; ++t) a[t] = rowvec(c_bF1, t, quad);
  tail_gemm<LA2, KBH, NTH, BF16, PO0, PO2, T::ST_O0>(a, FH, P, ring, (unsigned)L.atf1, (unsigned)L.ato0, (unsigned)L.ato2, lane);
  if (SAVE && save_ok) store_rows<NTH>(a, act + HD, quad);
#pragma unroll
  for (int t = 0; t < NTH; ++t)
#pragma unroll
    for (int i = 0; i < 4; ++i) a[t][i] = gelu_f(a[t][i]);
  make_frags<BF16, KBH>(FH, a);
  f32x4 c[NT];
#pragma unroll
  for (int t = 0; t < NT; ++t) c[t] = rowvec(c_bO0, t, quad);
  tail_gemm<LA2, KBH, NT, BF16, PO2, PO4, T::ST_O2>(c, FH, P, ring, (unsigned)L.ato0, (unsigned)L.ato2, (unsigned)L.ato4, lane);
  if (SAVE && save_ok) store_rows<NT>(c, act + 2 * HD, quad);
#pragma unroll
  for (int t = 0; t < NT; ++t)
#pragma unroll
    for (int i = 0; i < 4; ++i) c[t][i] = gelu_f(c[t][i]);
  Frags<BF16, KB> FD;
  make_frags<BF16, KB>(FD, c);
#pragma unroll
  for (int t = 0; t < NT; ++t) c[t] = rowvec(c_bO2, t, quad);
  tail_gemm<LA2, KB, NT, BF16, PO4, NX1, T::ST_O4>(c, FD, P, ring, (unsigned)L.ato2, (unsigned)L.ato4, next, lane);
  if (SAVE && save_ok) store_rows<NT>(c, act + 2 * HD + D, quad);
#pragma unroll
  for (int t = 0; t < NT; ++t)
#pragma unroll
    for (int i = 0; i < 4; ++i) c[t][i] = gelu_f(c[t][i]);
  make_frags<BF16, KB>(FD, c);
  o4[0] = rowvec(c_bO4, 0, quad);
  o4[1] = rowvec(c_bO4, 1, quad);
  tail_gemm<LA2, KB, 2, BF16, NX1, NX2, NEXT_BYTES>(o4, FD, P, ring, (unsigned)L.ato4, next, next2, lane);
}

template <int D, int H, bool BF16>
DEV void tail_consts(float* cst, const char* blob, const EnfLayout& L, int tid) {
  constexpr int HD = H * D;
  auto G = [&](size_t off) { return reinterpret_cast<const float*>(blob + off); };
  for (int i = tid; i < HD; i += NTHREADS) { cst[i] = G(L.bB)[i]; cst[HD + i] = G(L.bF1)[i]; }
  for (int i = tid; i < D; i += NTHREADS) { cst[2 * HD + i] = G(L.bO0)[i]; cst[2 * HD + D + i] = G(L.bO2)[i]; }
  for (int i = tid; i < 32; i += NTHREADS) cst[2 * HD + 2 * D + i] = G(L.bO4)[i];
}

template <bool CW>
DEV float tail_sq_err(const f32x4 (&o4)[2], f32x4 (&g0)[2], const TailArgs& A, int qi, bool qvalid, int quad, float gs) {
  float se = 0.f;
  if constexpr (CW) {
#pragma unroll
    for (int t = 0; t < 2; ++t)
#pragma unroll
      for (int i = 0; i < 4; ++i) {
        const int o = 16 * t + 4 * quad + i;
        const bool in = o < A.O && qvalid;
        const float w = in ? A.weight[(size_t)qi * A.O + o] : 0.f;
        const float dd = (in && w > 0.f) ? o4[t][i] - A.target[(size_t)qi * A.O + o] : 0.f;
        const float wd = w * dd;
        se = fmaf(wd, dd, se);
        g0[t][i] = wd * gs;
      }
  } else if (A.weight) {
    const float w = A.weight[qi];
    const bool live = qvalid && w > 0.f;
#pragma unroll
    for (int t = 0; t < 2; ++t)
#pragma unroll
      for (int i = 0; i < 4; ++i) {
        const int o = 16 * t + 4 * quad + i;
        const float dd = (o < A.O && live) ? o4[t][i] - A.target[(size_t)qi * A.O + o] : 0.f;
        const float wd = w * dd;
        se = fmaf(wd, dd, se);
        g0[t][i] = wd * gs;
      }
  } else {
#pragma unroll
    for (int t = 0; t < 2; ++t)
#pragma unroll
      for (int i = 0; i < 4; ++i) {
        const int o = 16 * t + 4 * quad + i;
        const float dd = (o < A.O && qvalid) ? o4[t][i] - A.target[(size_t)qi * A.O + o] : 0.f;
        se = fmaf(dd, dd, se);
        g0[t][i] = dd * gs;
      }
  }
  return se;
}
DEV float tail_err_reduce(float se, float* err, int q, bool qvalid, int quad, bool want_sum = true) {
  se += __shfl_xor(se, 32, 64);
  se += __shfl_xor(se, 16, 64);
  if (err && quad == 0 && qvalid) err[q] = se;
  if (want_sum) {
#pragma unroll
    for (int o = 8; o > 0; o >>= 1) se += __shfl_xor(se, o, 64);
  }
  return se;
}
DEV void tail_loss_add(float se, const TailArgs& A, int wave) {
  if (A.loss_part) A.loss_part[blockIdx.x * NWAVES + wave] = se * A.inv_n;
  else atomicAdd(A.loss, se * A.inv_n);
}

template <int D, int H, bool BF16, bool LA2, bool SAVE, int EVAL = 0>
__global__ __launch_bounds__(NTHREADS, 2) void enf_tail_fwd_kernel(TailArgs A) {
  static_assert(!(SAVE && EVAL != 0), "the evaluation tail has no backward to stash for");
  using T = TailCfg<D, H, BF16>;
  extern __shared__ __attribute__((aligned(16))) char smem[];
  char* ring = smem;
  float* cst = reinterpret_cast<float*>(smem + (LA2 ? 3 : 2) * STAGE_MAX);
  const int tid = threadIdx.x, lane = tid & 63, wave = tid >> 6, col = lane & 15, quad = lane >> 4;
  const int q0 = blockIdx.x * (16 * NWAVES) + wave * 16;
  const int qi = min(q0 + col, A.NQ - 1);
  tail_consts<D, H, BF16>(cst, A.blob, A.L, tid);
  Pipe P;
  P.rs = make_blob_rsrc(A.blob, (unsigned)A.L.total);
  P.rs2 = P.rs;
  if constexpr (LA2) {
    __syncthreads();
    la2_first<Pan<T::KBH, T::NTH, BF16>, Pan<T::KBH, T::NTH, BF16>>(P, ring, (unsigned)A.L.atb, (unsigned)A.L.atf1, wave, lane);
  } else first_stage<T::ST_TB>(P, ring, (unsigned)A.L.atb, wave, lane);
  f32x4 o4[2];
  const bool yh = !SAVE && A.ybar_half;
  const float* yrow = yh ? reinterpret_cast<const float*>(reinterpret_cast<const unsigned short*>(A.ybar) + (size_t)qi * T::HD)
                         : A.ybar + (size_t)qi * T::HD;
  tail_forward<D, H, BF16, SAVE, LA2, NoPan, NoPan>(o4, yrow, SAVE ? A.act + (size_t)qi * T::ACT : nullptr, A.L,
                                                    cst, P, ring, NO_STAGE, NO_STAGE, lane, quad, A.inv_hd, true, yh);
  if constexpr (EVAL != 0) {
    const bool qvalid = q0 + col < A.NQ;
    f32x4 g0[2];
    float se = tail_sq_err<EVAL == 2>(o4, g0, A, qi, qvalid, quad, 0.f);
    se = tail_err_reduce(se, A.err, q0 + col, qvalid, quad, A.loss != nullptr);
    if (A.loss && lane == 0) tail_loss_add(se, A, wave);
  } else if (q0 + col < A.NQ) {
#pragma unroll
    for (int t = 0; t < 2; ++t)
#pragma unroll
      for (int i = 0; i < 4; ++i) {
        const int o = 16 * t + 4 * quad + i;
        if (o < A.O) A.out[(size_t)(q0 + col) * A.O + o] = o4[t][i];
      }
  }
}

template <int D, int H, bool BF16, bool LA2, bool RECOMP, bool WG = false, bool LOSS = false, bool CW = false, bool SEED = false>
__global__ __launch_bounds__(NTHREADS, 2) void enf_tail_bwd_kernel(TailArgs A) {
  static_assert(!LOSS || RECOMP, "the fused loss needs the forward chain's outputs");
  static_assert(!CW || LOSS, "per-channel weights belong to the fused loss");
  static_assert(!SEED || (!RECOMP && !WG && !LOSS), "the seeded backward reads the stash and writes d ybar and delta only");
  using T = TailCfg<D, H, BF16>;
  constexpr int KB = T::KB, KBH = T::KBH, NT = T::NT, NTH = T::NTH, HD = T::HD;
  using PG4 = Pan<1, NT, BF16>; using PG2 = Pan<KB, NT, BF16>; using PG0 = Pan<KB, NTH, BF16>; using PGH = Pan<KBH, NTH, BF16>;
  extern __shared__ __attribute__((aligned(16))) char smem[];
  char* ring = smem;
  float* cst = reinterpret_cast<float*>(smem + (LA2 ? 3 : 2) * STAGE_MAX);
  const int tid = threadIdx.x, lane = tid & 63, wave = tid >> 6, col = lane & 15, quad = lane >> 4;
  const int q0 = blockIdx.x * (16 * NWAVES) + wave * 16;
  const bool qvalid = q0 + col < A.NQ;
  const int qi = min(q0 + col, A.NQ - 1);
  float* act = A.act + (size_t)qi * T::ACT;
  float* tdel = WG ? A.tdel + (size_t)qi * (2 * HD + 2 * D) : nullptr;
  const float* yrow = A.ybar + (size_t)qi * HD;
  tail_consts<D, H, BF16>(cst, A.blob, A.L, tid);
  Pipe P;
  P.rs = make_blob_rsrc(A.blob, (unsigned)A.L.total);
  P.rs2 = P.rs;
  f32x4 o4[2] = {f32x4{0.f, 0.f, 0.f, 0.f}, f32x4{0.f, 0.f, 0.f, 0.f}};
  if constexpr (RECOMP) {
    if constexpr (LA2) {
      __syncthreads();
      la2_first<PGH, PGH>(P, ring, (unsigned)A.L.atb, (unsigned)A.L.atf1, wave, lane);
    } else first_stage<T::ST_TB>(P, ring, (unsigned)A.L.atb, wave, lane);
    tail_forward<D, H, BF16, true, LA2, PG4, PG2>(o4, yrow, act, A.L, cst, P, ring, (unsigned)A.L.gto4, (unsigned)A.L.gto2, lane, quad,
                                                  A.inv_hd, !WG || qvalid);
  } else {
    if constexpr (LA2) {
      __syncthreads();
      la2_first<PG4, PG2>(P, ring, (unsigned)A.L.gto4, (unsigned)A.L.gto2, wave, lane);
    } else first_stage<T::ST_G4>(P, ring, (unsigned)A.L.gto4, wave, lane);
  }

  f32x4 g0[2];
  if constexpr (LOSS) {
    float se = tail_sq_err<CW>(o4, g0, A, qi, qvalid, quad, 2.0f * A.inv_n * A.gscale);
    se = tail_err_reduce(se, A.err, q0 + col, qvalid, quad);
    if (lane == 0) tail_loss_add(se, A, wave);
  } else if constexpr (SEED) {
#pragma unroll
    for (int t = 0; t < 2; ++t)
#pragma unroll
      for (int i = 0; i < 4; ++i) g0[t][i] = (16 * t + 4 * quad + i == A.seed && qvalid) ? 1.f : 0.f;
  } else {
#pragma unroll
  for (int t = 0; t < 2; ++t)
#pragma unroll
    for (int i = 0; i < 4; ++i) {
      const int o = 16 * t + 4 * quad + i;
      g0[t][i] = (o < A.O && qvalid) ? A.dout[(size_t)qi * A.O + o] : 0.f;
    }
  }
  Frags<BF16, 1> F1;
  make_frags<BF16, 1>(F1, g0);
  f32x4 c[NT];
  zero_tiles<NT>(c);
  tail_gemm<LA2, 1, NT, BF16, PG2, PG0, T::ST_O2>(c, F1, P, ring, (unsigned)A.L.gto4, (unsigned)A.L.gto2, (unsigned)A.L.gto0, lane);
  {
    f32x4 pre[NT];
    load_rows<NT>(pre, act + 2 * HD + D, quad);
#pragma unroll
    for (int t = 0; t < NT; ++t)
#pragma unroll
      for (int i = 0; i < 4; ++i) c[t][i] *= gelu_grad_f(pre[t][i]);
    if constexpr (WG) {
      if (qvalid) store_rows<NT>(c, tdel + 2 * HD + D, quad);
#pragma unroll
      for (int t = 0; t < NT; ++t)
#pragma unroll
        for (int i = 0; i < 4; ++i) pre[t][i] = gelu_f(pre[t][i]);
      if (qvalid) store_rows<NT>(pre, act + 2 * HD + D, quad);
    }
  }
  Frags<BF16, KB> FD;
  make_frags<BF16, KB>(FD, c);
  zero_tiles<NT>(c);
  tail_gemm<LA2, KB, NT, BF16, PG0, PGH, T::ST_G0>(c, FD, P, ring, (unsigned)A.L.gto2, (unsigned)A.L.gto0, (unsigned)A.L.gtf1, lane);
  {
    f32x4 pre[NT];
    load_rows<NT>(pre, act + 2 * HD, quad);
#pragma unroll
    for (int t = 0; t < NT; ++t)
#pragma unroll
      for (int i = 0; i < 4; ++i) c[t][i] *= gelu_grad_f(pre[t][i]);
    if constexpr (WG) {
      if (qvalid) store_rows<NT>(c, tdel + 2 * HD, quad);
#pragma unroll
      for (int t = 0; t < NT; ++t)
#pragma unroll
        for (int i = 0; i < 4; ++i) pre[t][i] = gelu_f(pre[t][i]);
      if (qvalid) store_rows<NT>(pre, act + 2 * HD, quad);
    }
  }
  make_frags<BF16, KB>(FD, c);
  f32x4 a[NTH];
  zero_tiles<NTH>(a);
  tail_gemm<LA2, KB, NTH, BF16, PGH, PGH, T::ST_TB>(a, FD, P, ring, (unsigned)A.L.gto0, (unsigned)A.L.gtf1, (unsigned)A.L.gtb, lane);
  {
    f32x4 pre[NTH];
    load_rows<NTH>(pre, act + HD, quad);
#pragma unroll
    for (int t = 0; t < NTH; ++t)
#pragma unroll
      for (int i = 0; i < 4; ++i) a[t][i] *= gelu_grad_f(pre[t][i]);
    if constexpr (WG) {
      if (qvalid) store_rows<NTH>(a, tdel + HD, quad);
#pragma unroll
      for (int t = 0; t < NTH; ++t)
#pragma unroll
        for (int i = 0; i < 4; ++i) pre[t][i] = gelu_f(pre[t][i]);
      if (qvalid) store_rows<NTH>(pre, act + HD, quad);
    }
  }
  Frags<BF16, KBH> FH;
  make_frags<BF16, KBH>(FH, a);
  zero_tiles<NTH>(a);
  tail_gemm<LA2, KBH, NTH, BF16, PGH, NoPan, T::ST_TB>(a, FH, P, ring, (unsigned)A.L.gtf1, (unsigned)A.L.gtb, NO_STAGE, lane);
  {
    f32x4 pre[NTH];
    load_rows<NTH>(pre, act, quad);
    const float mu = act[T::ACT - 2], rstd = act[T::ACT - 1];
    float s1 = 0.f, s2 = 0.f;
#pragma unroll
    for (int t = 0; t < NTH; ++t)
#pragma unroll
      for (int i = 0; i < 4; ++i) {
        const float nh = (gelu_f(pre[t][i]) - mu) * rstd;
        s1 += a[t][i]; s2 = fmaf(a[t][i], nh, s2);
      }
    const float m1 = xquad_sum(s1) * A.inv_hd, m2 = xquad_sum(s2) * A.inv_hd;
#pragma unroll
    for (int t = 0; t < NTH; ++t)
#pragma unroll
      for (int i = 0; i < 4; ++i) {
        const float nh = (gelu_f(pre[t][i]) - mu) * rstd;
        a[t][i] = rstd * (a[t][i] - m1 - nh * m2) * gelu_grad_f(pre[t][i]);
        if constexpr (WG) pre[t][i] = nh;
      }
    if constexpr (WG) {
      if (qvalid) store_rows<NTH>(a, tdel, quad);
      if (qvalid) store_rows<NTH>(pre, act, quad);
    }
  }
  make_frags<BF16, KBH>(FH, a);
  zero_tiles<NTH>(a);
  tail_gemm<LA2, KBH, NTH, BF16, NoPan, NoPan, 1024>(a, FH, P, ring, (unsigned)A.L.gtb, NO_STAGE, NO_STAGE, lane);
  f32x4 y[NTH];
  load_rows<NTH>(y, yrow, quad);
#pragma unroll
  for (int h = 0; h < H; ++h) {
    float s = 0.f;
#pragma unroll
    for (int t = 0; t < NT; ++t)
#pragma unroll
      for (int i = 0; i < 4; ++i) s = fmaf(a[h * NT + t][i], y[h * NT + t][i], s);
    s = xquad_sum(s);
    if (quad == 0 && qvalid) A.delta[(size_t)qi * H + h] = s;
  }
  if (qvalid) store_rows<NTH>(a, A.dybar + (size_t)qi * HD, quad);
}

template <int D, int H, bool BF16>
static int launch_tail(const TailArgs& A, bool bwd, bool opt, hipStream_t st, bool cw = false, bool eval = false, bool seeded = false) {
  const bool wg = bwd && A.tdel != nullptr;
  const bool fused_loss = bwd && A.target != nullptr;
  using T = TailCfg<D, H, BF16>;
  dim3 grid((A.NQ + 16 * NWAVES - 1) / (16 * NWAVES));
  const bool la2 = grid.x <= 256;
  static EnfAttrBits attr_done[8][2][2];
  auto go = [&](void (*kern_ptr)(TailArgs)) -> int {
    const int smem = la2 ? T::SMEM3 : T::SMEM;
    const int which = seeded ? 7 : eval ? (cw ? 6 : 5) : fused_loss ? (cw ? 4 : 3) : (wg ? 2 : bwd);
    if (!enf_lds_attr(reinterpret_cast<const void*>(kern_ptr), smem, attr_done[which][la2][opt])) return ENF_ELAUNCH;
    hipLaunchKernelGGL(kern_ptr, grid, dim3(NTHREADS), smem, st, A);
    return hipGetLastError() == hipSuccess ? 0 : ENF_ELAUNCH;
  };
  if (seeded) {
    if (!bwd || !opt || wg || fused_loss || eval || A.seed < 0 || A.seed >= A.O) return ENF_EINVAL;
    return la2 ? go(enf_tail_bwd_kernel<D, H, BF16, true, false, false, false, false, true>)
               : go(enf_tail_bwd_kernel<D, H, BF16, false, false, false, false, false, true>);
  }
  if (eval) {
    if (bwd || opt || !A.target || (cw && !A.weight)) return ENF_EINVAL;
    if (cw) return la2 ? go(enf_tail_fwd_kernel<D, H, BF16, true, false, 2>) : go(enf_tail_fwd_kernel<D, H, BF16, false, false, 2>);
    return la2 ? go(enf_tail_fwd_kernel<D, H, BF16, true, false, 1>) : go(enf_tail_fwd_kernel<D, H, BF16, false, false, 1>);
  }
  if (fused_loss) {
    if (wg || opt) return ENF_EINVAL;
    if (cw) {
      if (!A.weight) return ENF_EINVAL;
      return la2 ? go(enf_tail_bwd_kernel<D, H, BF16, true, true, false, true, true>)
                 : go(enf_tail_bwd_kernel<D, H, BF16, false, true, false, true, true>);
    }
    return la2 ? go(enf_tail_bwd_kernel<D, H, BF16, true, true, false, true>) : go(enf_tail_bwd_kernel<D, H, BF16, false, true, false, true>);
  }
  if (wg) {
    if (la2) return opt ? go(enf_tail_bwd_kernel<D, H, BF16, true, false, true>) : go(enf_tail_bwd_kernel<D, H, BF16, true, true, true>);
    return opt ? go(enf_tail_bwd_kernel<D, H, BF16, false, false, true>) : go(enf_tail_bwd_kernel<D, H, BF16, false, true, true>);
  }
  if (bwd) {
    if (la2) return opt ? go(enf_tail_bwd_kernel<D, H, BF16, true, false>) : go(enf_tail_bwd_kernel<D, H, BF16, true, true>);
    return opt ? go(enf_tail_bwd_kernel<D, H, BF16, false, false>) : go(enf_tail_bwd_kernel<D, H, BF16, false, true>);
  }
  if (la2) return opt ? go(enf_tail_fwd_kernel<D, H, BF16, true, true>) : go(enf_tail_fwd_kernel<D, H, BF16, true, false>);
  return opt ? go(enf_tail_fwd_kernel<D, H, BF16, false, true>) : go(enf_tail_fwd_kernel<D, H, BF16, false, false>);
}

int enf_launch_tail(const EnfDims& m, const EnfLayout& L, const char* blob, const float* ybar, float* out,
                    const float* dout, float* dybar, float* delta, float* act, int bwd, int opt, hipStream_t st) {
  return enf_launch_tail_wg(m, L, blob, ybar, out, dout, dybar, delta, act, nullptr, bwd, opt, st);
}
int enf_launch_tail_wg(const EnfDims& m, const EnfLayout& L, const char* blob, const float* ybar, float* out,
                       const float* dout, float* dybar, float* delta, float* act, float* tdel, int bwd, int opt, hipStream_t st) {
  if (m.OB != 1) return ENF_EUNSUPPORTED;
  TailArgs A;
  A.target = nullptr; A.weight = nullptr; A.loss = nullptr; A.gscale = 0.f; A.inv_n = 0.f; A.loss_part = nullptr; A.err = nullptr;
  A.tdel = tdel;
  A.ybar_half = (!bwd && (opt & 2) && m.bf16) ? 1 : 0;
  opt &= 1;
  A.ybar = ybar; A.blob = blob; A.L = L; A.out = out; A.dout = dout; A.dybar = dybar; A.delta = delta; A.act = act;
  A.NQ = m.B * m.N; A.O = m.O; A.inv_hd = 1.0f / (float)(m.Ht * m.Dt);
#define ENF_CASE(DD, HH)                                                                   \
  if (m.D == DD && m.H == HH) return m.bf16 ? launch_tail<DD, HH, true>(A, bwd != 0, opt != 0, st) : launch_tail<DD, HH, false>(A, bwd != 0, opt != 0, st);
  ENF_CASE(128, 2)
  ENF_CASE(64, 2)
  ENF_CASE(128, 1)
  ENF_CASE(64, 1)
  ENF_CASE(64, 4)
#undef ENF_CASE
  return ENF_EUNSUPPORTED;
}

int enf_launch_tail_seed(const EnfDims& m, const EnfLayout& L, const char* blob, const float* ybar, int seed, float* dybar, float* delta,
                         float* act, hipStream_t st) {
  if (m.OB != 1) return ENF_EUNSUPPORTED;
  TailArgs A;
  A.target = nullptr; A.weight = nullptr; A.loss = nullptr; A.gscale = 0.f; A.inv_n = 0.f; A.loss_part = nullptr; A.err = nullptr;
  A.tdel = nullptr; A.out = nullptr; A.dout = nullptr;
  A.seed = seed;
  A.ybar = ybar; A.blob = blob; A.L = L; A.dybar = dybar; A.delta = delta; A.act = act;
  A.NQ = m.B * m.N; A.O = m.O; A.inv_hd = 1.0f / (float)(m.Ht * m.Dt);
#define ENF_CASE(DD, HH)                                                                   \
  if (m.D == DD && m.H == HH)                                                              \
    return m.bf16 ? launch_tail<DD, HH, true>(A, true, true, st, false, false, true) : launch_tail<DD, HH, false>(A, true, true, st, false, false, true);
  ENF_CASE(128, 2)
  ENF_CASE(64, 2)
  ENF_CASE(128, 1)
  ENF_CASE(64, 1)
  ENF_CASE(64, 4)
#undef ENF_CASE
  return ENF_EUNSUPPORTED;
}

int enf_tail_loss_parts(const EnfDims& m) {
  return (int)(((long long)m.B * m.N + 16 * NWAVES - 1) / (16 * NWAVES)) * NWAVES;
}

static int tail_loss_kernel(const EnfDims& m, const EnfLayout& L, const char* blob, const float* ybar, const float* target,
                            const float* weight, float gscale, float* loss, float* dybar, float* delta, float* act, hipStream_t st, float* loss_part,
                            bool per_value, float* err, bool eval);

int enf_launch_tail_loss(const EnfDims& m, const EnfLayout& L, const char* blob, const float* ybar, const float* target,
                         const float* weight, float gscale, float* loss, float* dybar, float* delta, float* act, hipStream_t st, float* loss_part,
                         bool per_value, float* err) {
  if (int rc = tail_loss_kernel(m, L, blob, ybar, target, weight, gscale, loss, dybar, delta, act, st, loss_part, per_value, err, false)) return rc;
  return loss_part ? enf_launch_loss_sum(loss_part, enf_tail_loss_parts(m), loss, st) : 0;
}

int enf_launch_tail_eval(const EnfDims& m, const EnfLayout& L, const char* blob, const float* ybar, const float* target,
                         const float* weight, bool per_value, float* loss, float* err, hipStream_t st, float* loss_part) {
  if (!loss) loss_part = nullptr;
  if (int rc = tail_loss_kernel(m, L, blob, ybar, target, weight, 0.f, loss, nullptr, nullptr, nullptr, st, loss_part, per_value, err, true)) return rc;
  return loss_part ? enf_launch_loss_sum(loss_part, enf_tail_loss_parts(m), loss, st) : 0;
}

static int tail_loss_kernel(const EnfDims& m, const EnfLayout& L, const char* blob, const float* ybar, const float* target,
                            const float* weight, float gscale, float* loss, float* dybar, float* delta, float* act, hipStream_t st, float* loss_part,
                            bool per_value, float* err, bool eval) {
  if (m.OB != 1) return ENF_EUNSUPPORTED;
  TailArgs A;
  A.loss_part = loss_part; A.err = err;
  A.ybar = ybar; A.blob = blob; A.L = L; A.out = nullptr; A.dout = nullptr; A.dybar = dybar; A.delta = delta; A.act = act; A.tdel = nullptr;
  A.ybar_half = 0;
  A.target = target; A.weight = weight; A.loss = loss; A.gscale = gscale; A.inv_n = 1.0f / ((float)m.B * (float)m.N * (float)m.O);
  A.NQ = m.B * m.N; A.O = m.O; A.inv_hd = 1.0f / (float)(m.Ht * m.Dt);
#define ENF_CASE(DD, HH)                                                                   \
  if (m.D == DD && m.H == HH)                                                              \
    return m.bf16 ? launch_tail<DD, HH, true>(A, !eval, false, st, per_value, eval) : launch_tail<DD, HH, false>(A, !eval, false, st, per_value, eval);
  ENF_CASE(128, 2)
  ENF_CASE(64, 2)
  ENF_CASE(128, 1)
  ENF_CASE(64, 1)
  ENF_CASE(64, 4)
#undef ENF_CASE
  return ENF_EUNSUPPORTED;
}
```

Baseline: 31.64 million query-points/s.

## Fuse tail forward with seed backward and reduce shared dlt atomics via LDS slabs

In the shared-backward fit path, a single combined tail kernel now does both the forward output and the seeded backward, replacing the separate forward and seed launches. The shared pair-backward kernel now parks per-wave MFMA partials in LDS slabs and reduces them across waves before issuing global atomicAdds, instead of each wave doing its own atomics. It also adds tail kernel variants with fewer active waves per block. The intent is to cut one kernel launch, one re-read of ybar, and atomic contention on dlt, at the cost of more LDS, extra __syncthreads, and more template instantiations.

```diff
diff --git a/enf-pde_amd/_lib.py b/enf-pde_amd/_lib.py
--- a/enf-pde_amd/_lib.py
+++ b/enf-pde_amd/_lib.py
@@ -216,8 +216,12 @@
     lib.enf_backward_weights_scratch_bytes_ex.argtypes = [dp, ci, cu]
     lib.enf_backward_weights_ex.argtypes = [dp, vp, i64, vp, vp, vp, vp, vp, vp, ctypes.POINTER(vp), vp, vp, sz, cu, vp]
     if test_hooks:
-        for name in ("enf_debug_gemm", "enf_debug_pack", "enf_test_read_wave_sums", "enf_test_pair_fwd_streamed"):
+        for name in ("enf_debug_gemm", "enf_debug_pack", "enf_test_read_wave_sums", "enf_test_pair_fwd_streamed",
+                     "enf_test_tail_active_waves", "enf_test_tail_parts", "enf_test_tail"):
             getattr(lib, name).restype = ci
+        lib.enf_test_tail_active_waves.argtypes = [ci]
+        lib.enf_test_tail_parts.argtypes = [dp]
+        lib.enf_test_tail.argtypes = [dp, vp, ci, ci, vp, vp, vp, ci] + [vp] * 8
         lib.enf_test_pair_fwd_streamed.argtypes = [ci]
         lib.enf_debug_gemm.argtypes = [vp, vp, vp, ci, ci, ci, vp]
         lib.enf_debug_pack.argtypes = [vp, vp, ci, ci, ci, vp]
diff --git a/enf-pde_amd/csrc/enf_api.hip b/enf-pde_amd/csrc/enf_api.hip
--- a/enf-pde_amd/csrc/enf_api.hip
+++ b/enf-pde_amd/csrc/enf_api.hip
@@ -273,9 +273,8 @@
   if (sbwd) {
     float* dout = c.F(W.dybar) + (size_t)m.N * m.HD;
     float* out1 = dout + (size_t)m.B * m.N;
-    if ((rc = enf_launch_tail(m1, c.L, c.blob, c.F(W.ybar), out1, nullptr, nullptr, nullptr, c.F(W.tail_act), 0, 1, st))) return rc;
+    if ((rc = enf_launch_tail_fwd_seed(m1, c.L, c.blob, c.F(W.ybar), out1, 0, c.F(W.dybar), c.F(W.delta), c.F(W.tail_act), st))) return rc;
     if ((rc = enf_launch_mse_shared(out1, target, weight, m.B, m.N, grad_scale, dout, loss, st))) return rc;
-    if ((rc = enf_launch_tail_seed(m1, c.L, c.blob, c.F(W.ybar), 0, c.F(W.dybar), c.F(W.delta), c.F(W.tail_act), st))) return rc;
     if ((rc = enf_side_join_pending(st, workspace))) return rc;
     if ((rc = enf_launch_pair_bwd_shared(m, c.L, c.blob, x, c.F(W.lt), c.F(W.lse), c.F(W.dybar), c.F(W.delta), dout, c.F(W.dlt),
                                          c.ws + W.wzt, c.F(W.wzb), st)))
diff --git a/enf-pde_amd/csrc/enf_launch.h b/enf-pde_amd/csrc/enf_launch.h
--- a/enf-pde_amd/csrc/enf_launch.h
+++ b/enf-pde_amd/csrc/enf_launch.h
@@ -118,6 +118,8 @@
                        float* dybar, float* delta, float* act, float* tdel, int bwd, int opt, hipStream_t st);
 int enf_launch_tail_seed(const EnfDims& m, const EnfLayout& L, const char* blob, const float* ybar, int seed, float* dybar, float* delta,
                          float* act, hipStream_t st);
+int enf_launch_tail_fwd_seed(const EnfDims& m, const EnfLayout& L, const char* blob, const float* ybar, float* out, int seed, float* dybar,
+                             float* delta, float* act, hipStream_t st);
 int enf_launch_tail_loss(const EnfDims& m, const EnfLayout& L, const char* blob, const float* ybar, const float* target,
                          const float* weight, float gscale, float* loss, float* dybar, float* delta, float* act, hipStream_t st,
                          float* loss_part = nullptr, bool per_value = false, float* err = nullptr);
diff --git a/enf-pde_amd/csrc/enf_pair_bwd.hip b/enf-pde_amd/csrc/enf_pair_bwd.hip
--- a/enf-pde_amd/csrc/enf_pair_bwd.hip
+++ b/enf-pde_amd/csrc/enf_pair_bwd.hip
@@ -32,7 +32,7 @@
   return p;
 }
 
-#ifdef ENF_STAMPS
+#if defined(ENF_STAMPS) && !defined(ENF_PAIR_BWD_KERNEL_ONLY)
 __device__ unsigned long long enf_stamps_bwd[8 * 4 * 24];
 #define BSTAMP(k)                                                                                             \
   do {                                                                                                        \
@@ -414,11 +414,23 @@
       }
     };
     auto shared_add = [&](int off, const f32x4& g, bool cols) {
-      if (!(SHARED && tvalid && active && cols)) return;
+      if (!(SHARED && active && cols)) return;
 #pragma unroll
       for (int j = 0; j < 4; ++j) {
         const int sb = 16 * (int)blockIdx.z + 4 * quad + j;
         if (sb < A.SB) atomicAdd(A.dlt + ((size_t)sb * A.Z + bz) * ltstride + off, g[j]);
+      }
+    };
+    auto shared_park = [&](int s, const f32x4& g) {
+      *reinterpret_cast<f32x4*>(smem + SM::LACC + (wave * NT + s) * 1024 + lane * 16) = tvalid ? g : f32x4{0.f, 0.f, 0.f, 0.f};
+    };
+    auto shared_reduce = [&](int ns, auto&& off_of, bool cols) {
+      for (int s = wave; s < ns; s += NW) {
+        const char* t0 = smem + SM::LACC + s * 1024 + lane * 16;
+        f32x4 v = *reinterpret_cast<const f32x4*>(t0);
+#pragma unroll
+        for (int w = 1; w < NW; ++w) v += *reinterpret_cast<const f32x4*>(t0 + w * NT * 1024);
+        shared_add(off_of(s), v, cols);
       }
     };
 
@@ -576,13 +588,14 @@
                   f32x4 g = {0.f, 0.f, 0.f, 0.f};
 #pragma unroll
                   for (int i = 0; i < 4; ++i) g = __builtin_amdgcn_mfma_f32_16x16x4f32(ad[i], af[i] * dvf[mt][i], g, 0, 0, 0);
-                  shared_add(enf_lt_off_v0(H, D) + h * D + 16 * mt + col, g, true);
+                  shared_park(mt, g);
                 } else {
                   const f32x2 p2 = __builtin_elementwise_fma(hi2(af), hi2(dvf[mt]), lo2(af) * lo2(dvf[mt]));
                   part[mt] = p2[0] + p2[1];
                 }
               });
-          if constexpr (!SHARED) lacc_flush((H + h) * NT, part);
+          if constexpr (SHARED) shared_reduce(NT, [&](int s) { return enf_lt_off_v0(H, D) + h * D + 16 * s + col; }, true);
+          else lacc_flush((H + h) * NT, part);
         }
         BSTAMP(6 + 6 * h);
       }
@@ -832,6 +845,9 @@
 #pragma unroll
           for (int i = 0; i < 4; ++i) adl[h][i] = ad[i] * dl[h][i];
       }
+      constexpr int UCH = NT / H;
+      static_assert(!SHARED || NT % H == 0, "d u chunks");
+      auto u_off = [&](int c) { return [&, c](int s) { return enf_lt_off_u(H, D) + (s / UCH) * D + 16 * (c * UCH + s % UCH) + col; }; };
       unsigned mflip[4] = {0u, 0u, 0u, 0u};
       const bool masked = STORE && A.masks != nullptr;
       if (masked) {
@@ -855,14 +871,20 @@
                 g = __builtin_amdgcn_mfma_f32_16x16x4f32(adl[h][1], r1, g, 0, 0, 0);
                 g = __builtin_amdgcn_mfma_f32_16x16x4f32(adl[h][2], r2, g, 0, 0, 0);
                 g = __builtin_amdgcn_mfma_f32_16x16x4f32(adl[h][3], r3, g, 0, 0, 0);
-                shared_add(enf_lt_off_u(H, D) + h * D + 16 * mt + col, g, true);
+                shared_park(h * UCH + mt % UCH, g);
+                if (h == H - 1 && mt % UCH == UCH - 1 && mt != NT - 1) {
+                  __syncthreads();
+                  shared_reduce(NT, u_off(mt / UCH), true);
+                  __syncthreads();
+                }
               } else {
                 const f32x2 p2 = __builtin_elementwise_fma(f32x2{r2, r3}, f32x2{dl[h][2], dl[h][3]}, f32x2{r0, r1} * f32x2{dl[h][0], dl[h][1]});
                 upart[h][mt] = p2[0] + p2[1];
               }
             }
           }, c_bq1);
-      if constexpr (!SHARED) {
+      if constexpr (SHARED) shared_reduce(NT, u_off(H - 1), true);
+      else {
 #pragma unroll
         for (int h = 0; h < H; ++h) {
           lacc_flush(h * NT, upart[h]);
@@ -920,7 +942,9 @@
         g = __builtin_amdgcn_mfma_f32_16x16x4f32(ad[i], bv, g, 0, 0, 0);
       }
       const int off = col < H ? enf_lt_off_c(H, D) + col : col < H + 4 ? enf_lt_off_pose(H, D) + col - H : enf_lt_off_wcoef(H, D);
-      shared_add(off, g, col < H + 5);
+      shared_park(0, g);
+      __syncthreads();
+      shared_reduce(1, [&](int) { return off; }, col < H + 5);
     } else
     if (quad == 0) {
       float dwin = 0.f;
@@ -1062,6 +1086,7 @@
   WSTAMP(3);
 }
 
+#ifndef ENF_PAIR_BWD_KERNEL_ONLY
 __global__ __launch_bounds__(256) void enf_dlt_reduce_kernel(const float* __restrict__ part, int nsplit, long long rows, int H, int D,
                                                             int ext, float* __restrict__ dlt) {
   const int stride = enf_lt_stride(H, D);
@@ -1098,40 +1123,6 @@
   if (ZF && A.xcd_remap) grid = dim3(A.B * A.Z * A.nsplit, 1);
   hipLaunchKernelGGL(kern, grid, dim3(NTHREADS), SM::TOTAL, st, A);
   return hipGetLastError() == hipSuccess ? 0 : ENF_ELAUNCH;
-}
-
-template <int D, int H, bool BF16, int INV = -1>
-static int launch_pair_bwd_shared(const PairBwdArgs& A, hipStream_t st) {
-  using SM = PairBwdSmem<D, H, BF16, false>;
-  auto kern = enf_pair_bwd_kernel<D, H, BF16, false, true, INV, false, true>;
-  static EnfAttrBits attr_done{0};
-  if (!enf_lds_attr(reinterpret_cast<const void*>(kern), SM::TOTAL, attr_done)) return ENF_ELAUNCH;
-  hipLaunchKernelGGL(kern, dim3(A.Z, A.nsplit, (A.SB + 15) / 16), dim3(NTHREADS), SM::TOTAL, st, A);
-  return hipGetLastError() == hipSuccess ? 0 : ENF_ELAUNCH;
-}
-
-int enf_launch_pair_bwd_shared(const EnfDims& m, const EnfLayout& L, const char* blob, const float* x, const float* lt, const float* lse,
-                               const float* dybar, const float* delta, const float* dout, float* dlt, const char* wzt, const float* wzb,
-                               hipStream_t st) {
-  if (!enf_pair_bwd_shared_exists(m) || !enf_pair_bwd_zfold_fits(m) || !wzt || !wzb || !dout) return ENF_EUNSUPPORTED;
-  PairBwdArgs A;
-  A.dxq = nullptr; A.part = nullptr; A.dxpart = nullptr; A.masks = nullptr; A.mask_B = 1; A.mask_b0 = 0;
-  A.wzt = wzt; A.wzb = wzb; A.inv_d = 1.0f / (float)m.Dt;
-  A.x = x; A.x_bstride = 0; A.lt = lt; A.blob = blob; A.L = L; A.lse = lse; A.dybar = dybar; A.delta = delta;
-  A.dlt = dlt; A.B = 1; A.N = m.N; A.Z = m.Z; A.dx = m.dx; A.inv = m.inv; A.use_window = m.use_window;
-  A.nsplit = enf_pair_bwd_shared_nsplit(m); A.xcd_remap = 0;
-  A.dout = dout; A.SB = m.B;
-  if (m.bf16 && m.dx == 2) {
-    if (m.D == 128 && m.H == 2 && m.inv == ENF_INV_REL_POS_PERIODIC) return launch_pair_bwd_shared<128, 2, true, ENF_INV_REL_POS_PERIODIC>(A, st);
-    if (m.D == 64 && m.H == 2 && m.inv == ENF_INV_PONITA) return launch_pair_bwd_shared<64, 2, true, ENF_INV_PONITA>(A, st);
-  }
-#define ENF_CASE(DD, HH) \
-  if (m.D == DD && m.H == HH) return m.bf16 ? launch_pair_bwd_shared<DD, HH, true>(A, st) : launch_pair_bwd_shared<DD, HH, false>(A, st);
-  ENF_CASE(128, 2)
-  ENF_CASE(64, 2)
-  ENF_CASE(128, 1)
-#undef ENF_CASE
-  return ENF_EUNSUPPORTED;
 }
 
 
@@ -1219,3 +1210,4 @@
 #undef ENF_CASE
   return ENF_EUNSUPPORTED;
 }
+#endif
diff --git a/enf-pde_amd/csrc/enf_pair_bwd_shared.hip b/enf-pde_amd/csrc/enf_pair_bwd_shared.hip
--- /dev/null
+++ b/enf-pde_amd/csrc/enf_pair_bwd_shared.hip
@@ -0,0 +1,39 @@
+#define ENF_PAIR_BWD_KERNEL_ONLY 1
+#include "enf_pair_bwd.hip"
+
+template <int D, int H, bool BF16, int INV = -1>
+static int launch_pair_bwd_shared(const PairBwdArgs& A, hipStream_t st) {
+  using SM = PairBwdSmem<D, H, BF16, false>;
+  auto kern = enf_pair_bwd_kernel<D, H, BF16, false, true, INV, false, true>;
+  static EnfAttrBits attr_done{0};
+  constexpr int SLABS = SM::LACC + NWAVES * (D / 16) * 1024, TOTAL = SLABS > SM::TOTAL ? SLABS : SM::TOTAL;
+  static_assert(SLABS <= SM::EXTACC || !SM::EXT_OK, "the slabs end before the ext sums");
+  static_assert(TOTAL <= 160 * 1024, "K3 LDS budget");
+  if (!enf_lds_attr(reinterpret_cast<const void*>(kern), TOTAL, attr_done)) return ENF_ELAUNCH;
+  hipLaunchKernelGGL(kern, dim3(A.Z, A.nsplit, (A.SB + 15) / 16), dim3(NTHREADS), TOTAL, st, A);
+  return hipGetLastError() == hipSuccess ? 0 : ENF_ELAUNCH;
+}
+
+int enf_launch_pair_bwd_shared(const EnfDims& m, const EnfLayout& L, const char* blob, const float* x, const float* lt, const float* lse,
+                               const float* dybar, const float* delta, const float* dout, float* dlt, const char* wzt, const float* wzb,
+                               hipStream_t st) {
+  if (!enf_pair_bwd_shared_exists(m) || !enf_pair_bwd_zfold_fits(m) || !wzt || !wzb || !dout) return ENF_EUNSUPPORTED;
+  PairBwdArgs A;
+  A.dxq = nullptr; A.part = nullptr; A.dxpart = nullptr; A.masks = nullptr; A.mask_B = 1; A.mask_b0 = 0;
+  A.wzt = wzt; A.wzb = wzb; A.inv_d = 1.0f / (float)m.Dt;
+  A.x = x; A.x_bstride = 0; A.lt = lt; A.blob = blob; A.L = L; A.lse = lse; A.dybar = dybar; A.delta = delta;
+  A.dlt = dlt; A.B = 1; A.N = m.N; A.Z = m.Z; A.dx = m.dx; A.inv = m.inv; A.use_window = m.use_window;
+  A.nsplit = enf_pair_bwd_shared_nsplit(m); A.xcd_remap = 0;
+  A.dout = dout; A.SB = m.B;
+  if (m.bf16 && m.dx == 2) {
+    if (m.D == 128 && m.H == 2 && m.inv == ENF_INV_REL_POS_PERIODIC) return launch_pair_bwd_shared<128, 2, true, ENF_INV_REL_POS_PERIODIC>(A, st);
+    if (m.D == 64 && m.H == 2 && m.inv == ENF_INV_PONITA) return launch_pair_bwd_shared<64, 2, true, ENF_INV_PONITA>(A, st);
+  }
+#define ENF_CASE(DD, HH) \
+  if (m.D == DD && m.H == HH) return m.bf16 ? launch_pair_bwd_shared<DD, HH, true>(A, st) : launch_pair_bwd_shared<DD, HH, false>(A, st);
+  ENF_CASE(128, 2)
+  ENF_CASE(64, 2)
+  ENF_CASE(128, 1)
+#undef ENF_CASE
+  return ENF_EUNSUPPORTED;
+}
diff --git a/enf-pde_amd/csrc/enf_tail.hip b/enf-pde_amd/csrc/enf_tail.hip
--- a/enf-pde_amd/csrc/enf_tail.hip
+++ b/enf-pde_amd/csrc/enf_tail.hip
@@ -1,5 +1,6 @@
 #include <hip/hip_runtime.h>
 #include <cstdlib>
+#include <type_traits>
 #include "enf_launch.h"
 #define ENF_PIPE_ONE_RS 1
 #include "enf_device.h"
@@ -67,7 +68,7 @@
 };
 struct NoPan { static constexpr int SPP = 0, STAGE = 0; };
 
-template <int SP, int KBIN, int MTOUT, bool BF16, typename N1, typename N2, int INIT>
+template <int SP, int KBIN, int MTOUT, bool BF16, typename N1, typename N2, int INIT, bool ACTIVE>
 DEV void la2_step(f32x4 (&acc)[MTOUT], const Frags<BF16, KBIN>& F, Pipe& P, char* ring, unsigned panel, unsigned n1, unsigned n2,
                   int lane, const float* bias) {
   using C = PanelCfg<KBIN, MTOUT, BF16>;
@@ -77,17 +78,17 @@
   if constexpr (AHEAD < 0) la2_issue<C::STAGE>(P, panel + (SP + 2) * C::STAGE, ring, slot2, lane);
   else if constexpr (AHEAD < N1::SPP) la2_issue<N1::STAGE>(P, n1 + AHEAD * N1::STAGE, ring, slot2, lane);
   else if constexpr (AHEAD == N1::SPP && N1::SPP <= 1 && N2::STAGE > 0) la2_issue<N2::STAGE>(P, n2, ring, slot2, lane);
-  gemm_stage<BF16, KBIN, C::MTS, INIT>(&acc[SP * C::MTS], F, ring + P.cur * STAGE_MAX, lane, bias + 16 * SP * C::MTS);
+  if constexpr (ACTIVE) gemm_stage<BF16, KBIN, C::MTS, INIT>(&acc[SP * C::MTS], F, ring + P.cur * STAGE_MAX, lane, bias + 16 * SP * C::MTS);
   wait_vm<La2Cnt<ISSUED>::K>();
   __syncthreads();
   P.cur = (P.cur + 1) % 3;
 }
-template <int KBIN, int MTOUT, bool BF16, typename N1, typename N2, int INIT = INIT_ACC>
+template <int KBIN, int MTOUT, bool BF16, typename N1, typename N2, bool ACTIVE = true, int INIT = INIT_ACC>
 DEV void panel_gemm_la2(f32x4 (&acc)[MTOUT], const Frags<BF16, KBIN>& F, Pipe& P, char* ring, unsigned panel, unsigned n1,
                         unsigned n2, int lane, const float* bias = nullptr) {
   using C = PanelCfg<KBIN, MTOUT, BF16>;
   static_assert(C::SPP <= 8, "unrolled by hand");
-#define LA2_STEP(SP_) if constexpr (C::SPP > SP_) la2_step<SP_, KBIN, MTOUT, BF16, N1, N2, INIT>(acc, F, P, ring, panel, n1, n2, lane, bias);
+#define LA2_STEP(SP_) if constexpr (C::SPP > SP_) la2_step<SP_, KBIN, MTOUT, BF16, N1, N2, INIT, ACTIVE>(acc, F, P, ring, panel, n1, n2, lane, bias);
   LA2_STEP(0) LA2_STEP(1) LA2_STEP(2) LA2_STEP(3) LA2_STEP(4) LA2_STEP(5) LA2_STEP(6) LA2_STEP(7)
 #undef LA2_STEP
 }
@@ -103,11 +104,11 @@
   wait_vm<La2Cnt<S1>::K>();
   __syncthreads();
 }
-template <bool LA2, int KBIN, int MTOUT, bool BF16, typename N1, typename N2, int NEXT_BYTES>
+template <bool LA2, int KBIN, int MTOUT, bool BF16, typename N1, typename N2, int NEXT_BYTES, bool ACTIVE = true>
 DEV void tail_gemm(f32x4 (&acc)[MTOUT], const Frags<BF16, KBIN>& F, Pipe& P, char* ring, unsigned panel, unsigned n1, unsigned n2,
                    int lane) {
-  if constexpr (LA2) panel_gemm_la2<KBIN, MTOUT, BF16, N1, N2>(acc, F, P, ring, panel, n1, n2, lane);
-  else panel_gemm<KBIN, MTOUT, BF16, NEXT_BYTES>(acc, F, P, ring, panel, n1, true, lane);
+  if constexpr (LA2) panel_gemm_la2<KBIN, MTOUT, BF16, N1, N2, ACTIVE>(acc, F, P, ring, panel, n1, n2, lane);
+  else panel_gemm<KBIN, MTOUT, BF16, NEXT_BYTES>(acc, F, P, ring, panel, n1, ACTIVE, lane);
 }
 
 template <int D, int H, bool BF16, bool SAVE, bool LA2, typename NX1, typename NX2>
@@ -179,6 +180,41 @@
   for (int i = tid; i < 32; i += NTHREADS) cst[2 * HD + 2 * D + i] = G(L.bO4)[i];
 }
 
+template <int D, int H, bool BF16, bool FWD, bool BWD>
+DEV void tail_cadence(const TailArgs& A, char* smem) {
+  using T = TailCfg<D, H, BF16>;
+  constexpr int KB = T::KB, KBH = T::KBH, NT = T::NT, NTH = T::NTH;
+  using PTB = Pan<KBH, NTH, BF16>; using PO0 = Pan<KBH, NT, BF16>; using PO2 = Pan<KB, NT, BF16>; using PO4 = Pan<KB, 2, BF16>;
+  using PG4 = Pan<1, NT, BF16>; using PG2 = Pan<KB, NT, BF16>; using PG0 = Pan<KB, NTH, BF16>; using PGH = Pan<KBH, NTH, BF16>;
+  using NX1 = std::conditional_t<BWD, PG4, NoPan>; using NX2 = std::conditional_t<BWD, PG2, NoPan>;
+  char* ring = smem;
+  const int tid = threadIdx.x, lane = tid & 63, wave = tid >> 6;
+  const EnfLayout& L = A.L;
+  tail_consts<D, H, BF16>(reinterpret_cast<float*>(smem + 3 * STAGE_MAX), A.blob, L, tid);
+  Pipe P;
+  P.rs = make_blob_rsrc(A.blob, (unsigned)L.total);
+  P.rs2 = P.rs;
+  __syncthreads();
+  f32x4 a[NTH], c[NT], o4[2];
+  Frags<BF16, KBH> FH; Frags<BF16, KB> FD; Frags<BF16, 1> F1;
+  const unsigned next = BWD ? (unsigned)L.gto4 : NO_STAGE, next2 = BWD ? (unsigned)L.gto2 : NO_STAGE;
+  if constexpr (FWD) {
+    la2_first<PTB, PTB>(P, ring, (unsigned)L.atb, (unsigned)L.atf1, wave, lane);
+    tail_gemm<true, KBH, NTH, BF16, PTB, PO0, T::ST_TB, false>(a, FH, P, ring, (unsigned)L.atb, (unsigned)L.atf1, (unsigned)L.ato0, lane);
+    tail_gemm<true, KBH, NTH, BF16, PO0, PO2, T::ST_O0, false>(a, FH, P, ring, (unsigned)L.atf1, (unsigned)L.ato0, (unsigned)L.ato2, lane);
+    tail_gemm<true, KBH, NT, BF16, PO2, PO4, T::ST_O2, false>(c, FH, P, ring, (unsigned)L.ato0, (unsigned)L.ato2, (unsigned)L.ato4, lane);
+    tail_gemm<true, KB, NT, BF16, PO4, NX1, T::ST_O4, false>(c, FD, P, ring, (unsigned)L.ato2, (unsigned)L.ato4, next, lane);
+    tail_gemm<true, KB, 2, BF16, NX1, NX2, 1024, false>(o4, FD, P, ring, (unsigned)L.ato4, next, next2, lane);
+  } else la2_first<PG4, PG2>(P, ring, (unsigned)L.gto4, (unsigned)L.gto2, wave, lane);
+  if constexpr (BWD) {
+    tail_gemm<true, 1, NT, BF16, PG2, PG0, T::ST_O2, false>(c, F1, P, ring, (unsigned)L.gto4, (unsigned)L.gto2, (unsigned)L.gto0, lane);
+    tail_gemm<true, KB, NT, BF16, PG0, PGH, T::ST_G0, false>(c, FD, P, ring, (unsigned)L.gto2, (unsigned)L.gto0, (unsigned)L.gtf1, lane);
+    tail_gemm<true, KB, NTH, BF16, PGH, PGH, T::ST_TB, false>(a, FD, P, ring, (unsigned)L.gto0, (unsigned)L.gtf1, (unsigned)L.gtb, lane);
+    tail_gemm<true, KBH, NTH, BF16, PGH, NoPan, T::ST_TB, false>(a, FH, P, ring, (unsigned)L.gtf1, (unsigned)L.gtb, NO_STAGE, lane);
+    tail_gemm<true, KBH, NTH, BF16, NoPan, NoPan, 1024, false>(a, FH, P, ring, (unsigned)L.gtb, NO_STAGE, NO_STAGE, lane);
+  }
+}
+
 template <bool CW>
 DEV float tail_sq_err(const f32x4 (&o4)[2], f32x4 (&g0)[2], const TailArgs& A, int qi, bool qvalid, int quad, float gs) {
   float se = 0.f;
@@ -231,20 +267,24 @@
   }
   return se;
 }
-DEV void tail_loss_add(float se, const TailArgs& A, int wave) {
-  if (A.loss_part) A.loss_part[blockIdx.x * NWAVES + wave] = se * A.inv_n;
+DEV void tail_loss_add(float se, const TailArgs& A, int qtile) {
+  if (A.loss_part) A.loss_part[qtile] = se * A.inv_n;
   else atomicAdd(A.loss, se * A.inv_n);
 }
 
-template <int D, int H, bool BF16, bool LA2, bool SAVE, int EVAL = 0>
+template <int D, int H, bool BF16, bool LA2, bool SAVE, int EVAL = 0, int AW = NWAVES>
 __global__ __launch_bounds__(NTHREADS, 2) void enf_tail_fwd_kernel(TailArgs A) {
   static_assert(!(SAVE && EVAL != 0), "the evaluation tail has no backward to stash for");
+  static_assert(AW == NWAVES || (LA2 && (AW == 4 || AW == 2 || AW == 1)), "fewer active waves: small grids, the 3-slot ring");
   using T = TailCfg<D, H, BF16>;
   extern __shared__ __attribute__((aligned(16))) char smem[];
   char* ring = smem;
   float* cst = reinterpret_cast<float*>(smem + (LA2 ? 3 : 2) * STAGE_MAX);
   const int tid = threadIdx.x, lane = tid & 63, wave = tid >> 6, col = lane & 15, quad = lane >> 4;
-  const int q0 = blockIdx.x * (16 * NWAVES) + wave * 16;
+  if constexpr (AW < NWAVES) {
+    if (__builtin_amdgcn_readfirstlane(wave) >= AW) { tail_cadence<D, H, BF16, true, false>(A, smem); return; }
+  }
+  const int q0 = blockIdx.x * (16 * AW) + wave * 16;
   const int qi = min(q0 + col, A.NQ - 1);
   tail_consts<D, H, BF16>(cst, A.blob, A.L, tid);
   Pipe P;
@@ -265,7 +305,7 @@
     f32x4 g0[2];
     float se = tail_sq_err<EVAL == 2>(o4, g0, A, qi, qvalid, quad, 0.f);
     se = tail_err_reduce(se, A.err, q0 + col, qvalid, quad, A.loss != nullptr);
-    if (A.loss && lane == 0) tail_loss_add(se, A, wave);
+    if (A.loss && lane == 0) tail_loss_add(se, A, blockIdx.x * AW + wave);
   } else if (q0 + col < A.NQ) {
 #pragma unroll
     for (int t = 0; t < 2; ++t)
@@ -277,11 +317,13 @@
   }
 }
 
-template <int D, int H, bool BF16, bool LA2, bool RECOMP, bool WG = false, bool LOSS = false, bool CW = false, bool SEED = false>
+template <int D, int H, bool BF16, bool LA2, bool RECOMP, bool WG = false, bool LOSS = false, bool CW = false, bool SEED = false,
+          int AW = NWAVES>
 __global__ __launch_bounds__(NTHREADS, 2) void enf_tail_bwd_kernel(TailArgs A) {
   static_assert(!LOSS || RECOMP, "the fused loss needs the forward chain's outputs");
   static_assert(!CW || LOSS, "per-channel weights belong to the fused loss");
-  static_assert(!SEED || (!RECOMP && !WG && !LOSS), "the seeded backward reads the stash and writes d ybar and delta only");
+  static_assert(!SEED || (!WG && !LOSS), "the seeded backward writes d ybar and delta (and, with the forward chain, out) only");
+  static_assert(AW == NWAVES || (LA2 && !WG && (AW == 4 || AW == 2 || AW == 1)), "fewer active waves: small grids, the 3-slot ring");
   using T = TailCfg<D, H, BF16>;
   constexpr int KB = T::KB, KBH = T::KBH, NT = T::NT, NTH = T::NTH, HD = T::HD;
   using PG4 = Pan<1, NT, BF16>; using PG2 = Pan<KB, NT, BF16>; using PG0 = Pan<KB, NTH, BF16>; using PGH = Pan<KBH, NTH, BF16>;
@@ -289,7 +331,10 @@
   char* ring = smem;
   float* cst = reinterpret_cast<float*>(smem + (LA2 ? 3 : 2) * STAGE_MAX);
   const int tid = threadIdx.x, lane = tid & 63, wave = tid >> 6, col = lane & 15, quad = lane >> 4;
-  const int q0 = blockIdx.x * (16 * NWAVES) + wave * 16;
+  if constexpr (AW < NWAVES) {
+    if (__builtin_amdgcn_readfirstlane(wave) >= AW) { tail_cadence<D, H, BF16, RECOMP, true>(A, smem); return; }
+  }
+  const int q0 = blockIdx.x * (16 * AW) + wave * 16;
   const bool qvalid = q0 + col < A.NQ;
   const int qi = min(q0 + col, A.NQ - 1);
   float* act = A.act + (size_t)qi * T::ACT;
@@ -307,6 +352,17 @@
     } else first_stage<T::ST_TB>(P, ring, (unsigned)A.L.atb, wave, lane);
     tail_forward<D, H, BF16, true, LA2, PG4, PG2>(o4, yrow, act, A.L, cst, P, ring, (unsigned)A.L.gto4, (unsigned)A.L.gto2, lane, quad,
                                                   A.inv_hd, !WG || qvalid);
+    if constexpr (SEED) {
+      if (qvalid && A.out) {
+#pragma unroll
+        for (int t = 0; t < 2; ++t)
+#pragma unroll
+          for (int i = 0; i < 4; ++i) {
+            const int o = 16 * t + 4 * quad + i;
+            if (o < A.O) A.out[(size_t)(q0 + col) * A.O + o] = o4[t][i];
+          }
+      }
+    }
   } else {
     if constexpr (LA2) {
       __syncthreads();
@@ -318,7 +374,7 @@
   if constexpr (LOSS) {
     float se = tail_sq_err<CW>(o4, g0, A, qi, qvalid, quad, 2.0f * A.inv_n * A.gscale);
     se = tail_err_reduce(se, A.err, q0 + col, qvalid, quad);
-    if (lane == 0) tail_loss_add(se, A, wave);
+    if (lane == 0) tail_loss_add(se, A, blockIdx.x * AW + wave);
   } else if constexpr (SEED) {
 #pragma unroll
     for (int t = 0; t < 2; ++t)
@@ -442,38 +498,86 @@
   if (qvalid) store_rows<NTH>(a, A.dybar + (size_t)qi * HD, quad);
 }
 
+static int tail_active_waves(int nq) {
+  const int tiles = (nq + 15) / 16;
+  for (int aw = NWAVES; aw > 1; aw >>= 1)
+    if ((tiles + aw - 1) / aw >= 256) return aw;
+  return 1;
+}
+#ifdef ENF_TEST_HOOKS
+static int g_test_tail_aw = 0;
+extern "C" int enf_test_tail_active_waves(int aw) {
+  const int was = g_test_tail_aw;
+  g_test_tail_aw = (aw == 1 || aw == 2 || aw == 4 || aw == NWAVES) ? aw : 0;
+  return was;
+}
+constexpr bool TAIL_LOSS_AW_ALL = true;
+#else
+constexpr bool TAIL_LOSS_AW_ALL = false;
+#endif
+
 template <int D, int H, bool BF16>
 static int launch_tail(const TailArgs& A, bool bwd, bool opt, hipStream_t st, bool cw = false, bool eval = false, bool seeded = false) {
   const bool wg = bwd && A.tdel != nullptr;
   const bool fused_loss = bwd && A.target != nullptr;
   using T = TailCfg<D, H, BF16>;
-  dim3 grid((A.NQ + 16 * NWAVES - 1) / (16 * NWAVES));
-  const bool la2 = grid.x <= 256;
-  static EnfAttrBits attr_done[8][2][2];
+  int aw = NWAVES;
+  if ((!bwd || seeded) && !A.loss_part) aw = tail_active_waves(A.NQ);
+#ifdef ENF_TEST_HOOKS
+  if (g_test_tail_aw && !wg && !A.loss_part && (!bwd || seeded || fused_loss)) aw = g_test_tail_aw;
+#endif
+  dim3 grid((A.NQ + 16 * aw - 1) / (16 * aw));
+  const bool la2 = grid.x <= 256 || aw < NWAVES;
+  const int awi = aw == NWAVES ? 0 : aw == 4 ? 1 : aw == 2 ? 2 : 3;
+  static EnfAttrBits attr_done[8][2][2][4];
   auto go = [&](void (*kern_ptr)(TailArgs)) -> int {
     const int smem = la2 ? T::SMEM3 : T::SMEM;
     const int which = seeded ? 7 : eval ? (cw ? 6 : 5) : fused_loss ? (cw ? 4 : 3) : (wg ? 2 : bwd);
-    if (!enf_lds_attr(reinterpret_cast<const void*>(kern_ptr), smem, attr_done[which][la2][opt])) return ENF_ELAUNCH;
+    if (!enf_lds_attr(reinterpret_cast<const void*>(kern_ptr), smem, attr_done[which][la2][opt][awi])) return ENF_ELAUNCH;
     hipLaunchKernelGGL(kern_ptr, grid, dim3(NTHREADS), smem, st, A);
     return hipGetLastError() == hipSuccess ? 0 : ENF_ELAUNCH;
   };
+#define ENF_TAIL_AW(K)                 \
+  if (aw == 4) return go(K(4));        \
+  if (aw == 2) return go(K(2));        \
+  if (aw == 1) return go(K(1));
+#define ENF_K_SEED_STASH(AW_) enf_tail_bwd_kernel<D, H, BF16, true, false, false, false, false, true, AW_>
+#define ENF_K_SEED_FWD(AW_) enf_tail_bwd_kernel<D, H, BF16, true, true, false, false, false, true, AW_>
+#define ENF_K_LOSS(AW_) enf_tail_bwd_kernel<D, H, BF16, true, true, false, true, false, false, AW_>
+#define ENF_K_LOSS_CW(AW_) enf_tail_bwd_kernel<D, H, BF16, true, true, false, true, true, false, AW_>
+#define ENF_K_EVAL(AW_) enf_tail_fwd_kernel<D, H, BF16, true, false, 1, AW_>
+#define ENF_K_EVAL_CW(AW_) enf_tail_fwd_kernel<D, H, BF16, true, false, 2, AW_>
+#define ENF_K_FWD(AW_) enf_tail_fwd_kernel<D, H, BF16, true, false, 0, AW_>
+#define ENF_K_FWD_SAVE(AW_) enf_tail_fwd_kernel<D, H, BF16, true, true, 0, AW_>
   if (seeded) {
-    if (!bwd || !opt || wg || fused_loss || eval || A.seed < 0 || A.seed >= A.O) return ENF_EINVAL;
-    return la2 ? go(enf_tail_bwd_kernel<D, H, BF16, true, false, false, false, false, true>)
-               : go(enf_tail_bwd_kernel<D, H, BF16, false, false, false, false, false, true>);
+    if (!bwd || wg || fused_loss || eval || A.seed < 0 || A.seed >= A.O) return ENF_EINVAL;
+    if (opt) {
+      ENF_TAIL_AW(ENF_K_SEED_STASH)
+      return la2 ? go(enf_tail_bwd_kernel<D, H, BF16, true, false, false, false, false, true>)
+                 : go(enf_tail_bwd_kernel<D, H, BF16, false, false, false, false, false, true>);
+    }
+    ENF_TAIL_AW(ENF_K_SEED_FWD)
+    return la2 ? go(enf_tail_bwd_kernel<D, H, BF16, true, true, false, false, false, true>)
+               : go(enf_tail_bwd_kernel<D, H, BF16, false, true, false, false, false, true>);
   }
   if (eval) {
     if (bwd || opt || !A.target || (cw && !A.weight)) return ENF_EINVAL;
-    if (cw) return la2 ? go(enf_tail_fwd_kernel<D, H, BF16, true, false, 2>) : go(enf_tail_fwd_kernel<D, H, BF16, false, false, 2>);
+    if (cw) {
+      ENF_TAIL_AW(ENF_K_EVAL_CW)
+      return la2 ? go(enf_tail_fwd_kernel<D, H, BF16, true, false, 2>) : go(enf_tail_fwd_kernel<D, H, BF16, false, false, 2>);
+    }
+    ENF_TAIL_AW(ENF_K_EVAL)
     return la2 ? go(enf_tail_fwd_kernel<D, H, BF16, true, false, 1>) : go(enf_tail_fwd_kernel<D, H, BF16, false, false, 1>);
   }
   if (fused_loss) {
     if (wg || opt) return ENF_EINVAL;
     if (cw) {
       if (!A.weight) return ENF_EINVAL;
+      if constexpr (TAIL_LOSS_AW_ALL) { ENF_TAIL_AW(ENF_K_LOSS_CW) }
       return la2 ? go(enf_tail_bwd_kernel<D, H, BF16, true, true, false, true, true>)
                  : go(enf_tail_bwd_kernel<D, H, BF16, false, true, false, true, true>);
     }
+    if constexpr (TAIL_LOSS_AW_ALL) { ENF_TAIL_AW(ENF_K_LOSS) }
     return la2 ? go(enf_tail_bwd_kernel<D, H, BF16, true, true, false, true>) : go(enf_tail_bwd_kernel<D, H, BF16, false, true, false, true>);
   }
   if (wg) {
@@ -484,8 +588,21 @@
     if (la2) return opt ? go(enf_tail_bwd_kernel<D, H, BF16, true, false>) : go(enf_tail_bwd_kernel<D, H, BF16, true, true>);
     return opt ? go(enf_tail_bwd_kernel<D, H, BF16, false, false>) : go(enf_tail_bwd_kernel<D, H, BF16, false, true>);
   }
-  if (la2) return opt ? go(enf_tail_fwd_kernel<D, H, BF16, true, true>) : go(enf_tail_fwd_kernel<D, H, BF16, true, false>);
-  return opt ? go(enf_tail_fwd_kernel<D, H, BF16, false, true>) : go(enf_tail_fwd_kernel<D, H, BF16, false, false>);
+  if (opt) {
+    ENF_TAIL_AW(ENF_K_FWD_SAVE)
+    return la2 ? go(enf_tail_fwd_kernel<D, H, BF16, true, true>) : go(enf_tail_fwd_kernel<D, H, BF16, false, true>);
+  }
+  ENF_TAIL_AW(ENF_K_FWD)
+  return la2 ? go(enf_tail_fwd_kernel<D, H, BF16, true, false>) : go(enf_tail_fwd_kernel<D, H, BF16, false, false>);
+#undef ENF_TAIL_AW
+#undef ENF_K_SEED_STASH
+#undef ENF_K_SEED_FWD
+#undef ENF_K_LOSS
+#undef ENF_K_LOSS_CW
+#undef ENF_K_EVAL
+#undef ENF_K_EVAL_CW
+#undef ENF_K_FWD
+#undef ENF_K_FWD_SAVE
 }
 
 int enf_launch_tail(const EnfDims& m, const EnfLayout& L, const char* blob, const float* ybar, float* out,
@@ -513,18 +630,18 @@
   return ENF_EUNSUPPORTED;
 }
 
-int enf_launch_tail_seed(const EnfDims& m, const EnfLayout& L, const char* blob, const float* ybar, int seed, float* dybar, float* delta,
-                         float* act, hipStream_t st) {
+static int tail_seed_kernel(const EnfDims& m, const EnfLayout& L, const char* blob, const float* ybar, float* out, int seed, float* dybar,
+                            float* delta, float* act, bool stashed, hipStream_t st) {
   if (m.OB != 1) return ENF_EUNSUPPORTED;
   TailArgs A;
   A.target = nullptr; A.weight = nullptr; A.loss = nullptr; A.gscale = 0.f; A.inv_n = 0.f; A.loss_part = nullptr; A.err = nullptr;
-  A.tdel = nullptr; A.out = nullptr; A.dout = nullptr;
+  A.tdel = nullptr; A.out = out; A.dout = nullptr;
   A.seed = seed;
   A.ybar = ybar; A.blob = blob; A.L = L; A.dybar = dybar; A.delta = delta; A.act = act;
   A.NQ = m.B * m.N; A.O = m.O; A.inv_hd = 1.0f / (float)(m.Ht * m.Dt);
 #define ENF_CASE(DD, HH)                                                                   \
   if (m.D == DD && m.H == HH)                                                              \
-    return m.bf16 ? launch_tail<DD, HH, true>(A, true, true, st, false, false, true) : launch_tail<DD, HH, false>(A, true, true, st, false, false, true);
+    return m.bf16 ? launch_tail<DD, HH, true>(A, true, stashed, st, false, false, true) : launch_tail<DD, HH, false>(A, true, stashed, st, false, false, true);
   ENF_CASE(128, 2)
   ENF_CASE(64, 2)
   ENF_CASE(128, 1)
@@ -532,6 +649,15 @@
   ENF_CASE(64, 4)
 #undef ENF_CASE
   return ENF_EUNSUPPORTED;
+}
+
+int enf_launch_tail_seed(const EnfDims& m, const EnfLayout& L, const char* blob, const float* ybar, int seed, float* dybar, float* delta,
+                         float* act, hipStream_t st) {
+  return tail_seed_kernel(m, L, blob, ybar, nullptr, seed, dybar, delta, act, true, st);
+}
+int enf_launch_tail_fwd_seed(const EnfDims& m, const EnfLayout& L, const char* blob, const float* ybar, float* out, int seed, float* dybar,
+                             float* delta, float* act, hipStream_t st) {
+  return tail_seed_kernel(m, L, blob, ybar, out, seed, dybar, delta, act, false, st);
 }
 
 int enf_tail_loss_parts(const EnfDims& m) {
@@ -577,3 +703,25 @@
 #undef ENF_CASE
   return ENF_EUNSUPPORTED;
 }
+
+#ifdef ENF_TEST_HOOKS
+extern "C" int enf_test_tail_parts(const EnfDesc* d) { return enf_check_desc(d) ? -1 : enf_tail_loss_parts(enf_dims(d)); }
+extern "C" int enf_test_tail(const EnfDesc* d, const void* packed, int form, int seed, const float* ybar, const float* target,
+                             const float* weight, int per_value, float* out, float* act, float* dybar, float* delta, float* err, float* loss,
+                             float* loss_part, void* stream) {
+  if (int rc = enf_check_desc(d)) return rc;
+  const EnfDims m = enf_dims(d);
+  const EnfLayout L = enf_layout(m);
+  const char* blob = (const char*)packed;
+  hipStream_t st = (hipStream_t)stream;
+  switch (form) {
+    case 0: return enf_launch_tail(m, L, blob, ybar, out, nullptr, nullptr, nullptr, nullptr, 0, 0, st);
+    case 1: return enf_launch_tail(m, L, blob, ybar, out, nullptr, nullptr, nullptr, act, 0, 1, st);
+    case 2: return enf_launch_tail_eval(m, L, blob, ybar, target, weight, per_value != 0, loss, err, st, loss_part);
+    case 3: return enf_launch_tail_seed(m, L, blob, ybar, seed, dybar, delta, act, st);
+    case 4: return enf_launch_tail_fwd_seed(m, L, blob, ybar, out, seed, dybar, delta, act, st);
+    case 5: return enf_launch_tail_loss(m, L, blob, ybar, target, weight, 1.0f, loss, dybar, delta, act, st, loss_part, per_value != 0, err);
+  }
+  return ENF_EINVAL;
+}
+#endif
```

Result: faster. 32.50 million query-points/s, median of 6 (+2.7%).
